# numtel/ntru-circom

Measured on NVIDIA B200. Metric: ciphertexts/sec (encrypt+decrypt) N=509 q=2048, higher is better.
Workload: dtype int8 x int8 -> int32

## Files before the change

### include/ntru_b200.h

```cpp
#ifndef NTRU_B200_H
#define NTRU_B200_H

#include <stddef.h>
#include <stdint.h>

#ifdef __cplusplus
extern "C" {
#endif

typedef struct ntru_ctx ntru_ctx;

enum {
  NTRU_OK = 0,
  NTRU_E_PARAM = -1,
  NTRU_E_LENGTH = -2,
  NTRU_E_NOKEY = -3,
  NTRU_E_CUDA = -4,
  NTRU_E_NCCL = -5,
  NTRU_E_NOMEM = -6,
  NTRU_E_UNSUPPORTED = -7
};

enum {
  NTRU_OPT_PATH = 1,
  NTRU_OPT_CHUNK_ROWS = 2,
  NTRU_OPT_TIMING = 3,
  NTRU_OPT_DR = 5,
  NTRU_OPT_DEC1_FORM = 6,
  NTRU_OPT_SCHEDULE = 7,
  NTRU_OPT_EPILOGUE = 8,
  NTRU_OPT_IMMA_FORM = 9
};

enum {
  NTRU_K_ENC_TENSOR = 0,
  NTRU_K_DEC1_TENSOR = 1,
  NTRU_K_DEC2_TENSOR = 2,
  NTRU_K_ENC_CORE = 3,
  NTRU_K_DEC_CORE = 4,
  NTRU_K_SUM = 5,
  NTRU_K_OTHER = 6,
  NTRU_K_ENC_IMMA = 7,
  NTRU_K_DEC_IMMA = 8,
  NTRU_K_MULDIV = 9,
  NTRU_K_PACK = 10,
  NTRU_K_COUNT = 11
};

int ntru_create(ntru_ctx **ctx, int N, int p, int q, int device);
void ntru_destroy(ntru_ctx *ctx);
const char *ntru_last_error(const ntru_ctx *ctx);
const char *ntru_strerror(int code);
int ntru_set_option(ntru_ctx *ctx, int key, long value);
int ntru_get_params(const ntru_ctx *ctx, int *N, int *p, int *q);
int ntru_pitch(const ntru_ctx *ctx);
uint64_t ntru_launch_count(const ntru_ctx *ctx);
int ntru_last_path(const ntru_ctx *ctx);
int ntru_timing_read(ntru_ctx *ctx, int kind, double *total_ms, uint64_t *launches);
int ntru_timing_reset(ntru_ctx *ctx);

int ntru_set_public_key(ntru_ctx *ctx, const uint16_t *h);
int ntru_set_private_key(ntru_ctx *ctx, const int8_t *f, const uint8_t *fp);

int ntru_encrypt_batch(ntru_ctx *ctx, size_t B, const uint8_t *r, const uint8_t *m,
                       uint16_t *value, uint16_t *quotientE, uint16_t *remainderE, uint8_t *r_out);
int ntru_encrypt_batch_wide(ntru_ctx *ctx, size_t B, const uint8_t *r, const uint16_t *m,
                            uint16_t *value, uint16_t *quotientE, uint16_t *remainderE, uint8_t *r_out);
int ntru_encrypt_batch_keys(ntru_ctx *ctx, size_t B, const uint16_t *h, const uint8_t *r, const uint8_t *m,
                            uint16_t *value, uint16_t *quotientE, uint16_t *remainderE, uint8_t *r_out);

#define NTRU_RNG_KEY_BYTES 32
int ntru_set_rng_key(ntru_ctx *ctx, const uint8_t key[NTRU_RNG_KEY_BYTES], uint64_t first_row);
uint64_t ntru_rng_next_row(const ntru_ctx *ctx);

int ntru_decrypt_batch(ntru_ctx *ctx, size_t B, const uint16_t *e, uint8_t *value,
                       uint16_t *quotient1, uint16_t *remainder1, uint8_t *quotient2, uint8_t *remainder2);
int ntru_decrypt_batch_keys(ntru_ctx *ctx, size_t B, const int8_t *f, const uint8_t *fp, const uint16_t *e,
                            uint8_t *value, uint16_t *quotient1, uint16_t *remainder1,
                            uint8_t *quotient2, uint8_t *remainder2);

int ntru_verify_keys_batch(ntru_ctx *ctx, size_t B, const int8_t *f, const uint16_t *fq, const uint8_t *fp, const int8_t *g,
                           uint16_t *quotient_fq, uint16_t *remainder_fq, uint8_t *quotient_fp, uint8_t *remainder_fp,
                           uint16_t *quotient_h, uint16_t *remainder_h);
int ntru_muldiv_dev(ntru_ctx *ctx, size_t B, const int8_t *x, const void *y, int mod_p, void *quotient, void *remainder);

int ntru_keygen_batch(ntru_ctx *ctx, size_t B, const int8_t *f, const int8_t *g, uint16_t *fq, uint8_t *fp, uint16_t *h,
                      uint8_t *valid);

int ntru_pack_geometry(uint32_t max_val, int data_len, int *max_input_bits, int *inputs_per_output, int *arr_len,
                       int *output_size);
int ntru_pack_output_dev(ntru_ctx *ctx, size_t B, const void *data, int elem_bytes, int data_len, size_t pitch,
                         uint32_t max_val, void *out);
int ntru_unpack_input_dev(ntru_ctx *ctx, size_t B, const void *data, int n_elems, uint32_t max_val, int packed_bits,
                          void *out, int elem_bytes, size_t pitch);

int ntru_pack_output(ntru_ctx *ctx, size_t B, const void *data, int elem_bytes, int data_len, uint32_t max_val, void *out);
int ntru_unpack_input(ntru_ctx *ctx, size_t B, const void *data, int n_elems, uint32_t max_val, int packed_bits, void *out,
                      int elem_bytes);

int ntru_packed_elems(const ntru_ctx *ctx, int mod_q, int width);
int ntru_encrypt_batch_packed(ntru_ctx *ctx, size_t B, const void *r, const void *m, void *value, void *quotientE,
                              void *remainderE, void *r_out);
int ntru_decrypt_batch_packed(ntru_ctx *ctx, size_t B, const void *e, void *value, void *quotient1, void *remainder1,
                              void *quotient2, void *remainder2);

int ntru_sum(ntru_ctx *ctx, size_t B, const uint16_t *e, uint16_t *out);
int ntru_sum_allreduce(ntru_ctx *ctx, size_t B, const uint16_t *e, uint16_t *out);

int ntru_encrypt_dev(ntru_ctx *ctx, size_t B, const uint16_t *h_rows, const uint8_t *r, const uint8_t *m,
                     uint16_t *value, uint16_t *quotientE, uint16_t *remainderE);
int ntru_decrypt_dev(ntru_ctx *ctx, size_t B, const int8_t *f_rows, const uint8_t *fp_rows, const uint16_t *e,
                     uint8_t *value, uint16_t *quotient1, uint16_t *remainder1,
                     uint8_t *quotient2, uint8_t *remainder2);
int ntru_sum_partial_dev(ntru_ctx *ctx, size_t B, const uint16_t *e, uint32_t *partial);
int ntru_sum_finalize_dev(ntru_ctx *ctx, const uint32_t *partial, uint16_t *out);
int ntru_sample_r_dev(ntru_ctx *ctx, size_t B, int dr, uint64_t row0, uint8_t *r);

#define NTRU_XCHG_HANDLE_BYTES 64
int ntru_xchg_create(ntru_ctx *ctx, int world, int rank, unsigned char handle_out[NTRU_XCHG_HANDLE_BYTES]);
int ntru_xchg_connect(ntru_ctx *ctx, const unsigned char *handles);
int ntru_sum_allreduce_dev(ntru_ctx *ctx, size_t B, const uint16_t *e, uint16_t *out);
int ntru_xchg_destroy(ntru_ctx *ctx);

void *ntru_stream(ntru_ctx *ctx);
int ntru_set_stream(ntru_ctx *ctx, void *stream);
int ntru_sync(ntru_ctx *ctx);

void *ntru_host_alloc(size_t bytes);
void ntru_host_free(void *p);

#ifdef __cplusplus
}
#endif
#endif
```

### ntru-circom_b200/_lib.py

```python
from __future__ import annotations

import ctypes
import os
from ctypes import POINTER, c_char_p, c_int, c_int8, c_long, c_size_t, c_uint8, c_uint16, c_uint32, c_uint64, c_void_p

_HERE = os.path.dirname(os.path.abspath(__file__))
LIB_PATH = os.environ.get("NTRU_B200_LIB") or os.path.join(_HERE, "libntru_b200.so")

NTRU_OK = 0
NTRU_E_PARAM, NTRU_E_LENGTH, NTRU_E_NOKEY, NTRU_E_CUDA = -1, -2, -3, -4
NTRU_E_NCCL, NTRU_E_NOMEM, NTRU_E_UNSUPPORTED = -5, -6, -7
NTRU_OPT_PATH, NTRU_OPT_CHUNK_ROWS, NTRU_OPT_TIMING, NTRU_OPT_DR, NTRU_OPT_DEC1_FORM, NTRU_OPT_SCHEDULE, NTRU_OPT_EPILOGUE = 1, 2, 3, 5, 6, 7, 8
NTRU_OPT_IMMA_FORM = 9
KERNEL_KINDS = ["enc_tensor", "dec1_tensor", "dec2_tensor", "enc_core", "dec_core", "sum", "other", "enc_imma", "dec_imma",
                "muldiv", "pack"]
PATH_AUTO, PATH_CUDA_CORE, PATH_TENSOR, PATH_IMMA = 0, 1, 2, 3

_P = c_void_p
SYMBOLS = {
    "ntru_create": (c_int, [POINTER(c_void_p), c_int, c_int, c_int, c_int]),
    "ntru_destroy": (None, [_P]),
    "ntru_last_error": (c_char_p, [_P]),
    "ntru_strerror": (c_char_p, [c_int]),
    "ntru_set_option": (c_int, [_P, c_int, c_long]),
    "ntru_pitch": (c_int, [_P]),
    "ntru_launch_count": (c_uint64, [_P]),
    "ntru_last_path": (c_int, [_P]),
    "ntru_timing_read": (c_int, [_P, c_int, POINTER(ctypes.c_double), POINTER(c_uint64)]),
    "ntru_timing_reset": (c_int, [_P]),
    "ntru_set_public_key": (c_int, [_P, _P]),
    "ntru_set_private_key": (c_int, [_P, _P, _P]),
    "ntru_encrypt_batch": (c_int, [_P, c_size_t, _P, _P, _P, _P, _P, _P]),
    "ntru_encrypt_batch_wide": (c_int, [_P, c_size_t, _P, _P, _P, _P, _P, _P]),
    "ntru_encrypt_batch_keys": (c_int, [_P, c_size_t, _P, _P, _P, _P, _P, _P, _P]),
    "ntru_set_rng_key": (c_int, [_P, _P, c_uint64]),
    "ntru_rng_next_row": (c_uint64, [_P]),
    "ntru_decrypt_batch": (c_int, [_P, c_size_t, _P, _P, _P, _P, _P, _P]),
    "ntru_decrypt_batch_keys": (c_int, [_P, c_size_t, _P, _P, _P, _P, _P, _P, _P, _P]),
    "ntru_packed_elems": (c_int, [_P, c_int, c_int]),
    "ntru_encrypt_batch_packed": (c_int, [_P, c_size_t, _P, _P, _P, _P, _P, _P]),
    "ntru_decrypt_batch_packed": (c_int, [_P, c_size_t, _P, _P, _P, _P, _P, _P]),
    "ntru_sum": (c_int, [_P, c_size_t, _P, _P]),
    "ntru_sum_allreduce": (c_int, [_P, c_size_t, _P, _P]),
    "ntru_pack_output": (c_int, [_P, c_size_t, _P, c_int, c_int, ctypes.c_uint32, _P]),
    "ntru_unpack_input": (c_int, [_P, c_size_t, _P, c_int, ctypes.c_uint32, c_int, _P, c_int]),
    "ntru_get_params": (c_int, [_P, POINTER(c_int), POINTER(c_int), POINTER(c_int)]),
    "ntru_keygen_batch": (c_int, [_P, c_size_t, _P, _P, _P, _P, _P, _P]),
    "ntru_pack_geometry": (c_int, [ctypes.c_uint32, c_int, POINTER(c_int), POINTER(c_int), POINTER(c_int), POINTER(c_int)]),
    "ntru_pack_output_dev": (c_int, [_P, c_size_t, _P, c_int, c_int, c_size_t, ctypes.c_uint32, _P]),
    "ntru_unpack_input_dev": (c_int, [_P, c_size_t, _P, c_int, ctypes.c_uint32, c_int, _P, c_int, c_size_t]),
    "ntru_verify_keys_batch": (c_int, [_P, c_size_t, _P, _P, _P, _P, _P, _P, _P, _P, _P, _P]),
    "ntru_muldiv_dev": (c_int, [_P, c_size_t, _P, _P, c_int, _P, _P]),
    "ntru_encrypt_dev": (c_int, [_P, c_size_t, _P, _P, _P, _P, _P, _P]),
    "ntru_decrypt_dev": (c_int, [_P, c_size_t, _P, _P, _P, _P, _P, _P, _P, _P]),
    "ntru_sum_partial_dev": (c_int, [_P, c_size_t, _P, _P]),
    "ntru_sum_finalize_dev": (c_int, [_P, _P, _P]),
    "ntru_sample_r_dev": (c_int, [_P, c_size_t, c_int, c_uint64, _P]),
    "ntru_xchg_create": (c_int, [_P, c_int, c_int, _P]),
    "ntru_xchg_connect": (c_int, [_P, _P]),
    "ntru_sum_allreduce_dev": (c_int, [_P, c_size_t, _P, _P]),
    "ntru_xchg_destroy": (c_int, [_P]),
    "ntru_stream": (c_void_p, [_P]),
    "ntru_set_stream": (c_int, [_P, _P]),
    "ntru_sync": (c_int, [_P]),
    "ntru_host_alloc": (c_void_p, [c_size_t]),
    "ntru_host_free": (None, [_P]),
}

_lib = None


class NtruError(RuntimeError):
    def __init__(self, code: int, msg: str):
        super().__init__(f"libntru_b200: {msg} (code {code})")
        self.code = code


def load() -> ctypes.CDLL:
    global _lib
    if _lib is not None:
        return _lib
    if not os.path.exists(LIB_PATH):
        from . import build as _build
        _build.build()
    lib = ctypes.CDLL(LIB_PATH)
    for name, (res, args) in SYMBOLS.items():
        fn = getattr(lib, name)
        fn.restype = res
        fn.argtypes = args
    _lib = lib
    return lib
```

### ntru-circom_b200/csrc/api.cu

```cuda

#include <cuda_runtime.h>
#include <stdint.h>
#include <stdio.h>
#include <stdlib.h>
#include <string.h>

#include <sys/random.h>

#include <new>
#include <string>

#include "ntru_internal.cuh"

namespace ntru {

int fail(ntru_ctx *ctx, int code, const std::string &msg) {
  if (ctx) ctx->err = msg;
  return code;
}

int cuda_fail(ntru_ctx *ctx, cudaError_t e, const char *what) {
  if (ctx) ctx->err = std::string("CUDA error: ") + cudaGetErrorString(e) + " in " + what;
  return NTRU_E_CUDA;
}

static cudaEvent_t pool_get(ntru_ctx *ctx) {
  if (!ctx->event_pool.empty()) {
    cudaEvent_t e = ctx->event_pool.back();
    ctx->event_pool.pop_back();
    return e;
  }
  cudaEvent_t e = nullptr;
  cudaEventCreate(&e);
  return e;
}

LaunchTimer::LaunchTimer(ntru_ctx *c, int k) : ctx(c), kind(k) {
  ctx->launches++;
  if (!ctx->timing) return;
  a = pool_get(ctx);
  b = pool_get(ctx);
  cudaEventRecord(a, ctx->stream);
}

LaunchTimer::~LaunchTimer() {
  if (!a) return;
  cudaEventRecord(b, ctx->stream);
  ctx->timed.push_back({kind, a, b});
}

namespace {

struct HostArr {
  const void *in = nullptr;
  void *out = nullptr;
  size_t elem = 1;
  size_t width = 0;
  bool used = false;
  int fe_bits = 0, fe_n = 0, fe_elems = 0;
  size_t host_row_bytes() const { return fe_bits ? (size_t)fe_elems * 32 : width * elem; }
};

constexpr int kMaxArr = 10;

template <class Launch>
int run_pipeline(ntru_ctx *ctx, size_t B, HostArr (&arr)[kMaxArr], Launch launch) {
  const size_t chunk = ctx->chunk_rows;
  const size_t P = (size_t)ctx->P;
  const size_t rows_alloc = B < chunk ? B : chunk;
  for (int s = 0; s < kNumSlots; ++s)
    for (int a = 0; a < kMaxArr; ++a)
      if (arr[a].used) {
        NTRU_CUDA(ctx, ctx->slot_bufs[s][a].reserve(rows_alloc * P * arr[a].elem));
        NTRU_CUDA(ctx, ctx->slot_packed[s][a].reserve(rows_alloc * arr[a].host_row_bytes()));
      }
  size_t ci = 0;
  for (size_t row0 = 0; row0 < B; row0 += chunk, ++ci) {
    const size_t rows = (B - row0) < chunk ? (B - row0) : chunk;
    const int s = (int)(ci % kNumSlots);
    void *dev[kMaxArr];
    for (int a = 0; a < kMaxArr; ++a) dev[a] = arr[a].used ? ctx->slot_bufs[s][a].ptr : nullptr;
    if (ci >= (size_t)kNumSlots) NTRU_CUDA(ctx, cudaStreamWaitEvent(ctx->s_in, ctx->ev_comp[s], 0));
    for (int a = 0; a < kMaxArr; ++a) {
      if (!arr[a].used || !arr[a].in) continue;
      const size_t wb = arr[a].host_row_bytes();
      NTRU_CUDA(ctx, cudaMemcpyAsync(ctx->slot_packed[s][a].ptr, (const char *)arr[a].in + row0 * wb, rows * wb,
                                     cudaMemcpyHostToDevice, ctx->s_in));
    }
    NTRU_CUDA(ctx, cudaEventRecord(ctx->ev_in[s], ctx->s_in));
    NTRU_CUDA(ctx, cudaStreamWaitEvent(ctx->stream, ctx->ev_in[s], 0));
    if (ci >= (size_t)kNumSlots) NTRU_CUDA(ctx, cudaStreamWaitEvent(ctx->stream, ctx->ev_out[s], 0));
    for (int a = 0; a < kMaxArr; ++a) {
      if (!arr[a].used || !arr[a].in) continue;
      int rc = arr[a].fe_bits
                   ? launch_wire_unpack(ctx, rows, (const uint32_t *)ctx->slot_packed[s][a].ptr, arr[a].fe_elems, arr[a].fe_bits,
                                        arr[a].fe_n, (int)arr[a].width, dev[a], (int)arr[a].elem)
                   : launch_repitch(ctx, ctx->slot_packed[s][a].ptr, dev[a], rows, (int)arr[a].width, (int)arr[a].elem, true);
      if (rc != NTRU_OK) return rc;
    }
    int rc = launch(rows, dev);
    if (rc != NTRU_OK) return rc;
    for (int a = 0; a < kMaxArr; ++a) {
      if (!arr[a].used || !arr[a].out) continue;
      rc = arr[a].fe_bits
               ? launch_pack_fields(ctx, rows, dev[a], (int)arr[a].elem, (int)arr[a].width, (size_t)ctx->P, arr[a].fe_bits, arr[a].fe_n,
                                    arr[a].fe_elems, (uint32_t *)ctx->slot_packed[s][a].ptr)
               : launch_repitch(ctx, dev[a], ctx->slot_packed[s][a].ptr, rows, (int)arr[a].width, (int)arr[a].elem, false);
      if (rc != NTRU_OK) return rc;
    }
    NTRU_CUDA(ctx, cudaEventRecord(ctx->ev_comp[s], ctx->stream));
    NTRU_CUDA(ctx, cudaStreamWaitEvent(ctx->s_out, ctx->ev_comp[s], 0));
    for (int a = 0; a < kMaxArr; ++a) {
      if (!arr[a].used || !arr[a].out) continue;
      const size_t wb = arr[a].host_row_bytes();
      NTRU_CUDA(ctx, cudaMemcpyAsync((char *)arr[a].out + row0 * wb, ctx->slot_packed[s][a].ptr, rows * wb,
                                     cudaMemcpyDeviceToHost, ctx->s_out));
    }
    NTRU_CUDA(ctx, cudaEventRecord(ctx->ev_out[s], ctx->s_out));
  }
  NTRU_CUDA(ctx, cudaStreamSynchronize(ctx->s_out));
  NTRU_CUDA(ctx, cudaStreamSynchronize(ctx->stream));
  return NTRU_OK;
}

void set_in(HostArr &a, const void *p, size_t elem, size_t width) {
  a.in = p; a.elem = elem; a.width = width; a.used = p != nullptr;
}
void set_out(HostArr &a, void *p, size_t elem, size_t width) {
  a.out = p; a.elem = elem; a.width = width; a.used = p != nullptr;
}

int bit_length(uint32_t v) {
  int b = 0;
  while (v) { ++b; v >>= 1; }
  return b;
}
void set_fe(HostArr &a, uint32_t max_val) {
  if (!a.used) return;
  a.fe_bits = bit_length(max_val);
  a.fe_n = 252 / a.fe_bits;
  int outs = ((int)a.width + a.fe_n - 1) / a.fe_n;
  a.fe_elems = outs < 3 ? 3 : outs;
}

int packed_elems(uint32_t max_val, int width) {
  const int n = 252 / bit_length(max_val);
  const int outs = (width + n - 1) / n;
  return outs < 3 ? 3 : outs;
}

constexpr size_t kSmallBatchRows = 4096;

bool want_tensor(ntru_ctx *ctx, bool same_key, bool ready, size_t B, int *rc) {
  *rc = NTRU_OK;
  if (ctx->opt_path == 1 || ctx->opt_path == 3) return false;
  if (ctx->opt_path == 0 && B < kSmallBatchRows && ctx->tensor_ok && imma_supported(ctx)) return false;
  const bool ok = same_key && ctx->tensor_ok && ready;
  if (ctx->opt_path == 2 && !ok) {
    *rc = fail(ctx, NTRU_E_UNSUPPORTED, "tensor schedule forced but not available for this call");
    return false;
  }
  return ok;
}

bool want_imma(ntru_ctx *ctx, bool wide_message, int *rc) {
  *rc = NTRU_OK;
  if (ctx->opt_path == 1) return false;
  const bool ok = ctx->tensor_ok && imma_supported(ctx) && !wide_message;
  if (ctx->opt_path == 3 && !ok) {
    *rc = fail(ctx, NTRU_E_UNSUPPORTED, "register-fragment schedule forced but not available for this call");
    return false;
  }
  return ok;
}

int encrypt_dispatch(ntru_ctx *ctx, size_t B, const uint16_t *h_rows, const uint8_t *r, const void *m, int m_wide,
                     uint16_t *value, uint16_t *quo, uint16_t *rem) {
  int rc;
  const bool same_key = h_rows == nullptr;
  if (same_key && !ctx->has_pub) return fail(ctx, NTRU_E_NOKEY, "public key h is not set");
  if (want_tensor(ctx, same_key && !m_wide, ctx->km_h.ready, B, &rc)) {
    ctx->last_path = 2;
    return umma_encrypt(ctx, B, r, (const uint8_t *)m, value, quo, rem);
  }
  if (rc != NTRU_OK) return rc;
  if (want_imma(ctx, m_wide != 0, &rc)) {
    ctx->last_path = 3;
    return launch_encrypt_imma(ctx, B, same_key ? (const uint16_t *)ctx->d_h.ptr : h_rows, same_key ? 0 : (size_t)ctx->P, r,
                               (const uint8_t *)m, value, quo, rem);
  }
  if (rc != NTRU_OK) return rc;
  ctx->last_path = 1;
  return launch_encrypt_generic(ctx, B, same_key ? (const uint16_t *)ctx->d_h.ptr : h_rows,
                                same_key ? 0 : (size_t)ctx->P, r, m, m_wide, value, quo, rem);
}

int decrypt_dispatch(ntru_ctx *ctx, size_t B, const int8_t *f_rows, const uint8_t *fp_rows, const uint16_t *e,
                     uint8_t *value, uint16_t *q1, uint16_t *r1, uint8_t *q2, uint8_t *r2) {
  int rc;
  const bool same_key = f_rows == nullptr && fp_rows == nullptr;
  if ((f_rows == nullptr) != (fp_rows == nullptr)) return fail(ctx, NTRU_E_PARAM, "f_rows and fp_rows must be given together");
  if (same_key && !ctx->has_priv) return fail(ctx, NTRU_E_NOKEY, "private key f/fp is not set");
  if (want_tensor(ctx, same_key, ctx->km_f.ready && ctx->km_fp.ready, B, &rc)) {
    ctx->last_path = 2;
    return umma_decrypt(ctx, B, e, value, q1, r1, q2, r2);
  }
  if (rc != NTRU_OK) return rc;
  if (want_imma(ctx, false, &rc)) {
    ctx->last_path = 3;
    return launch_decrypt_imma(ctx, B, same_key ? (const int8_t *)ctx->d_f.ptr : f_rows,
                               same_key ? (const uint8_t *)ctx->d_fp.ptr : fp_rows, same_key ? 0 : (size_t)ctx->P, e, value, q1,
                               r1, q2, r2);
  }
  if (rc != NTRU_OK) return rc;
  ctx->last_path = 1;
  return launch_decrypt_generic(ctx, B, same_key ? (const int8_t *)ctx->d_f.ptr : f_rows,
                                same_key ? (const uint8_t *)ctx->d_fp.ptr : fp_rows,
                                same_key ? 0 : (size_t)ctx->P, e, value, q1, r1, q2, r2);
}

int check(ntru_ctx *ctx) {
  if (!ctx) return NTRU_E_PARAM;
  cudaError_t e = cudaSetDevice(ctx->device);
  if (e != cudaSuccess) return cuda_fail(ctx, e, "cudaSetDevice");
  return NTRU_OK;
}

}
}

using namespace ntru;

extern "C" {

const char *ntru_strerror(int code) {
  switch (code) {
    case NTRU_OK: return "ok";
    case NTRU_E_PARAM: return "bad parameter";
    case NTRU_E_LENGTH: return "bad length";
    case NTRU_E_NOKEY: return "key not set";
    case NTRU_E_CUDA: return "CUDA error";
    case NTRU_E_NCCL: return "NCCL error";
    case NTRU_E_NOMEM: return "out of memory";
    case NTRU_E_UNSUPPORTED: return "unsupported";
    default: return "unknown error";
  }
}

const char *ntru_last_error(const ntru_ctx *ctx) { return ctx ? ctx->err.c_str() : "null context"; }

int ntru_create(ntru_ctx **out, int N, int p, int q, int device) {
  if (!out) return NTRU_E_PARAM;
  *out = nullptr;
  if (p != 3) return NTRU_E_PARAM;
  if (N < 8 || N > kMaxN) return NTRU_E_PARAM;
  if (q < 4 || q > 8192 || (q & (q - 1)) != 0) return NTRU_E_PARAM;
  if ((long long)N * 2 * (q - 1) >= (1ll << 24)) return NTRU_E_PARAM;
  int ndev = 0;
  cudaError_t e = cudaGetDeviceCount(&ndev);
  if (e != cudaSuccess || ndev == 0 || device < 0 || device >= ndev) return NTRU_E_CUDA;
  if (cudaSetDevice(device) != cudaSuccess) return NTRU_E_CUDA;
  ntru_ctx *ctx = new (std::nothrow) ntru_ctx();
  if (!ctx) return NTRU_E_NOMEM;
  ctx->N = N; ctx->p = p; ctx->q = q; ctx->device = device;
  ctx->logq = 0;
  while ((1 << ctx->logq) < q) ctx->logq++;
  ctx->P = ((N + 1 + 15) / 16) * 16;
  cudaDeviceProp prop;
  if (cudaGetDeviceProperties(&prop, device) == cudaSuccess) ctx->sm_count = prop.multiProcessorCount;
  bool ok = cudaStreamCreateWithFlags(&ctx->stream, cudaStreamNonBlocking) == cudaSuccess;
  ctx->own_stream = ok;
  ok = ok && cudaStreamCreateWithFlags(&ctx->s_in, cudaStreamNonBlocking) == cudaSuccess;
  ok = ok && cudaStreamCreateWithFlags(&ctx->s_out, cudaStreamNonBlocking) == cudaSuccess;
  for (int s = 0; ok && s < kNumSlots; ++s) {
    ok = ok && cudaEventCreateWithFlags(&ctx->ev_in[s], cudaEventDisableTiming) == cudaSuccess;
    ok = ok && cudaEventCreateWithFlags(&ctx->ev_comp[s], cudaEventDisableTiming) == cudaSuccess;
    ok = ok && cudaEventCreateWithFlags(&ctx->ev_out[s], cudaEventDisableTiming) == cudaSuccess;
  }
  ok = ok && ctx->d_h.reserve((size_t)ctx->P * 2) == cudaSuccess;
  ok = ok && ctx->d_f.reserve((size_t)ctx->P) == cudaSuccess;
  ok = ok && ctx->d_fp.reserve((size_t)ctx->P) == cudaSuccess;
  ok = ok && ctx->d_partial.reserve((size_t)ctx->P * 4) == cudaSuccess;
  if (!ok) {
    ntru_destroy(ctx);
    return NTRU_E_CUDA;
  }
  {
    size_t got = 0;
    unsigned char *kb = reinterpret_cast<unsigned char *>(ctx->rng_key);
    while (got < sizeof ctx->rng_key) {
      ssize_t n = getrandom(kb + got, sizeof ctx->rng_key - got, 0);
      if (n <= 0) break;
      got += (size_t)n;
    }
    if (got < sizeof ctx->rng_key) {
      FILE *fh = fopen("/dev/urandom", "rb");
      if (fh) {
        got += fread(kb + got, 1, sizeof ctx->rng_key - got, fh);
        fclose(fh);
      }
    }
    ctx->rng_keyed = got == sizeof ctx->rng_key;
  }
  umma_init(ctx);
  *out = ctx;
  return NTRU_OK;
}

static int xchg_release(ntru_ctx *ctx);
static int xchg_check(ntru_ctx *ctx);

void ntru_destroy(ntru_ctx *ctx) {
  if (!ctx) return;
  cudaSetDevice(ctx->device);
  cudaDeviceSynchronize();
  for (int s = 0; s < kNumSlots; ++s) {
    if (ctx->ev_in[s]) cudaEventDestroy(ctx->ev_in[s]);
    if (ctx->ev_comp[s]) cudaEventDestroy(ctx->ev_comp[s]);
    if (ctx->ev_out[s]) cudaEventDestroy(ctx->ev_out[s]);
    for (auto &b : ctx->slot_bufs[s]) b.release();
    for (auto &b : ctx->slot_packed[s]) b.release();
  }
  xchg_release(ctx);
  ctx->d_h.release(); ctx->d_f.release(); ctx->d_fp.release(); ctx->d_b.release(); ctx->d_partial.release(); ctx->d_sum_scratch.release();
  ctx->km_h.mat.release(); ctx->km_f.mat.release(); ctx->km_fp.mat.release();
  for (auto &t : ctx->timed) {
    cudaEventDestroy(t.a);
    cudaEventDestroy(t.b);
  }
  for (auto e : ctx->event_pool) cudaEventDestroy(e);
  if (ctx->own_stream && ctx->stream) cudaStreamDestroy(ctx->stream);
  if (ctx->s_in) cudaStreamDestroy(ctx->s_in);
  if (ctx->s_out) cudaStreamDestroy(ctx->s_out);
  delete ctx;
}

int ntru_set_option(ntru_ctx *ctx, int key, long value) {
  if (!ctx) return NTRU_E_PARAM;
  switch (key) {
    case NTRU_OPT_PATH:
      if (value < 0 || value > 3) return fail(ctx, NTRU_E_PARAM, "NTRU_OPT_PATH must be 0, 1, 2 or 3");
      ctx->opt_path = (int)value;
      return NTRU_OK;
    case NTRU_OPT_CHUNK_ROWS:
      if (value < 128) return fail(ctx, NTRU_E_PARAM, "NTRU_OPT_CHUNK_ROWS must be >= 128");
      ctx->chunk_rows = (size_t)value;
      return NTRU_OK;
    case NTRU_OPT_TIMING:
      ctx->timing = value != 0;
      return NTRU_OK;
    case NTRU_OPT_SCHEDULE:
      if (value < 0 || value > 1) return fail(ctx, NTRU_E_PARAM, "NTRU_OPT_SCHEDULE must be 0 or 1");
      ctx->opt_lohi = (int)value;
      return NTRU_OK;
    case NTRU_OPT_EPILOGUE:
      if (value < 0 || value > 2) return fail(ctx, NTRU_E_PARAM, "NTRU_OPT_EPILOGUE must be 0, 1 or 2");
      ctx->opt_epilogue = (int)value;
      if (ctx->tensor_ok) {
        if (ctx->has_pub) { int rc = umma_prepare_public(ctx); if (rc) return rc; }
        if (ctx->has_priv) { int rc = umma_prepare_private(ctx); if (rc) return rc; }
      }
      return NTRU_OK;
    case NTRU_OPT_IMMA_FORM:
      if (value < 0 || value > 1) return fail(ctx, NTRU_E_PARAM, "NTRU_OPT_IMMA_FORM must be 0 or 1");
      ctx->opt_imma_form = (int)value;
      return NTRU_OK;
    case NTRU_OPT_DEC1_FORM:
      if (value < 0 || value > 2) return fail(ctx, NTRU_E_PARAM, "NTRU_OPT_DEC1_FORM must be 0, 1 or 2");
      ctx->opt_dec1_form = (int)value;
      if (ctx->has_priv && ctx->tensor_ok) return umma_prepare_private(ctx);
      return NTRU_OK;
    case NTRU_OPT_DR:
      if (value < 0 || 2 * value > ctx->N) return fail(ctx, NTRU_E_PARAM, "The total of 1s and -1s cannot exceed the array length.");
      ctx->opt_dr = (int)value;
      return NTRU_OK;
    default:
      return fail(ctx, NTRU_E_PARAM, "unknown option");
  }
}

int ntru_pitch(const ntru_ctx *ctx) { return ctx ? ctx->P : 0; }
uint64_t ntru_launch_count(const ntru_ctx *ctx) { return ctx ? ctx->launches : 0; }
int ntru_last_path(const ntru_ctx *ctx) { return ctx ? ctx->last_path : 0; }

int ntru_timing_reset(ntru_ctx *ctx) {
  int rc = check(ctx);
  if (rc) return rc;
  NTRU_CUDA(ctx, cudaStreamSynchronize(ctx->stream));
  for (auto &t : ctx->timed) {
    ctx->event_pool.push_back(t.a);
    ctx->event_pool.push_back(t.b);
  }
  ctx->timed.clear();
  return NTRU_OK;
}

int ntru_timing_read(ntru_ctx *ctx, int kind, double *total_ms, uint64_t *launches) {
  int rc = check(ctx);
  if (rc) return rc;
  if (kind < 0 || kind >= NTRU_K_COUNT || !total_ms || !launches) return fail(ctx, NTRU_E_PARAM, "bad timing query");
  NTRU_CUDA(ctx, cudaStreamSynchronize(ctx->stream));
  double sum = 0;
  uint64_t n = 0;
  for (auto &t : ctx->timed) {
    if (t.kind != kind) continue;
    float ms = 0;
    NTRU_CUDA(ctx, cudaEventElapsedTime(&ms, t.a, t.b));
    sum += ms;
    ++n;
  }
  *total_ms = sum;
  *launches = n;
  return NTRU_OK;
}

int ntru_set_public_key(ntru_ctx *ctx, const uint16_t *h) {
  int rc = check(ctx);
  if (rc) return rc;
  if (!h) return fail(ctx, NTRU_E_PARAM, "h is NULL");
  uint16_t tmp[kMaxN + 32];
  memset(tmp, 0, sizeof tmp);
  for (int i = 0; i < ctx->N; ++i) {
    if (h[i] >= ctx->q) return fail(ctx, NTRU_E_PARAM, "h coefficient outside [0,q)");
    tmp[i] = h[i];
  }
  NTRU_CUDA(ctx, cudaMemcpy(ctx->d_h.ptr, tmp, (size_t)ctx->P * 2, cudaMemcpyHostToDevice));
  ctx->has_pub = true;
  ctx->km_h.ready = false;
  if (ctx->tensor_ok) {
    rc = umma_prepare_public(ctx);
    if (rc) return rc;
  }
  return NTRU_OK;
}

int ntru_set_private_key(ntru_ctx *ctx, const int8_t *f, const uint8_t *fp) {
  int rc = check(ctx);
  if (rc) return rc;
  if (!f || !fp) return fail(ctx, NTRU_E_PARAM, "f or fp is NULL");
  int8_t tf[kMaxN + 32];
  uint8_t tp[kMaxN + 32];
  memset(tf, 0, sizeof tf);
  memset(tp, 0, sizeof tp);
  for (int i = 0; i < ctx->N; ++i) {
    if (f[i] < -1 || f[i] > 1) return fail(ctx, NTRU_E_PARAM, "f coefficient outside {-1,0,1}");
    if (fp[i] >= ctx->p) return fail(ctx, NTRU_E_PARAM, "fp coefficient outside [0,p)");
    tf[i] = f[i];
    tp[i] = fp[i];
  }
  NTRU_CUDA(ctx, cudaMemcpy(ctx->d_f.ptr, tf, (size_t)ctx->P, cudaMemcpyHostToDevice));
  NTRU_CUDA(ctx, cudaMemcpy(ctx->d_fp.ptr, tp, (size_t)ctx->P, cudaMemcpyHostToDevice));
  ctx->has_priv = true;
  ctx->km_f.ready = ctx->km_fp.ready = false;
  if (ctx->tensor_ok) {
    rc = umma_prepare_private(ctx);
    if (rc) return rc;
  }
  return NTRU_OK;
}


static int encrypt_host(ntru_ctx *ctx, size_t B, const uint16_t *h, const uint8_t *r, const void *m, int m_wide,
                        uint16_t *value, uint16_t *quo, uint16_t *rem, uint8_t *r_out, bool fe = false) {
  int rc = check(ctx);
  if (rc) return rc;
  if (!m) return fail(ctx, NTRU_E_PARAM, "m is required");
  if (!r) {
    if (ctx->opt_dr < 0) return fail(ctx, NTRU_E_PARAM, "r is NULL and NTRU_OPT_DR (the dr of the constructor options) is not set");
    if (!ctx->rng_keyed) return fail(ctx, NTRU_E_UNSUPPORTED, "r is NULL and the device generator has no key (no OS entropy; call ntru_set_rng_key)");
  }
  if (B == 0) return NTRU_OK;
  const size_t N = (size_t)ctx->N;
  HostArr arr[kMaxArr];
  set_in(arr[0], h, 2, N);
  if (r) {
    set_in(arr[1], r, 1, N);
    if (r_out && r_out != r)
      memcpy(r_out, r, fe ? B * (size_t)packed_elems(ctx->p - 1, (int)N) * 32 : B * N);
  } else {
    set_out(arr[1], r_out, 1, N);
    arr[1].used = true;
  }
  set_in(arr[2], m, m_wide ? 2 : 1, N);
  set_out(arr[3], value, 2, N);
  set_out(arr[4], quo, 2, N + 1);
  set_out(arr[5], rem, 2, N + 1);
  if (fe) {
    set_fe(arr[1], (uint32_t)ctx->p - 1); set_fe(arr[2], (uint32_t)ctx->p - 1);
    for (int a = 3; a <= 5; ++a) set_fe(arr[a], (uint32_t)ctx->q - 1);
  }
  uint64_t next_row = ctx->rng_row;
  if (!r) ctx->rng_row += B;
  return run_pipeline(ctx, B, arr, [&](size_t rows, void **dev) {
    if (!r) {
      int rs = launch_sample_r(ctx, rows, ctx->opt_dr, next_row, (uint8_t *)dev[1]);
      if (rs) return rs;
      next_row += rows;
    }
    return encrypt_dispatch(ctx, rows, (const uint16_t *)dev[0], (const uint8_t *)dev[1], dev[2], m_wide,
                            (uint16_t *)dev[3], (uint16_t *)dev[4], (uint16_t *)dev[5]);
  });
}

int ntru_encrypt_batch(ntru_ctx *ctx, size_t B, const uint8_t *r, const uint8_t *m, uint16_t *value,
                       uint16_t *quotientE, uint16_t *remainderE, uint8_t *r_out) {
  return encrypt_host(ctx, B, nullptr, r, m, 0, value, quotientE, remainderE, r_out);
}

int ntru_encrypt_batch_wide(ntru_ctx *ctx, size_t B, const uint8_t *r, const uint16_t *m, uint16_t *value,
                            uint16_t *quotientE, uint16_t *remainderE, uint8_t *r_out) {
  return encrypt_host(ctx, B, nullptr, r, m, 1, value, quotientE, remainderE, r_out);
}

int ntru_encrypt_batch_keys(ntru_ctx *ctx, size_t B, const uint16_t *h, const uint8_t *r, const uint8_t *m,
                            uint16_t *value, uint16_t *quotientE, uint16_t *remainderE, uint8_t *r_out) {
  if (!h) return fail(ctx, NTRU_E_PARAM, "h is NULL");
  return encrypt_host(ctx, B, h, r, m, 0, value, quotientE, remainderE, r_out);
}

static int decrypt_host(ntru_ctx *ctx, size_t B, const int8_t *f, const uint8_t *fp, const uint16_t *e,
                        uint8_t *value, uint16_t *q1, uint16_t *r1, uint8_t *q2, uint8_t *r2, bool fe = false) {
  int rc = check(ctx);
  if (rc) return rc;
  if (!e) return fail(ctx, NTRU_E_PARAM, "e is required");
  if (B == 0) return NTRU_OK;
  const size_t N = (size_t)ctx->N;
  HostArr arr[kMaxArr];
  set_in(arr[0], f, 1, N);
  set_in(arr[1], fp, 1, N);
  set_in(arr[2], e, 2, N);
  set_out(arr[3], value, 1, N);
  set_out(arr[4], q1, 2, N + 1);
  set_out(arr[5], r1, 2, N + 1);
  set_out(arr[6], q2, 1, N + 1);
  set_out(arr[7], r2, 1, N + 1);
  if (fe) {
    set_fe(arr[2], (uint32_t)ctx->q - 1); set_fe(arr[4], (uint32_t)ctx->q - 1); set_fe(arr[5], (uint32_t)ctx->q - 1);
    set_fe(arr[3], (uint32_t)ctx->p - 1); set_fe(arr[6], (uint32_t)ctx->p - 1); set_fe(arr[7], (uint32_t)ctx->p - 1);
  }
  return run_pipeline(ctx, B, arr, [&](size_t rows, void **dev) {
    return decrypt_dispatch(ctx, rows, (const int8_t *)dev[0], (const uint8_t *)dev[1], (const uint16_t *)dev[2],
                            (uint8_t *)dev[3], (uint16_t *)dev[4], (uint16_t *)dev[5], (uint8_t *)dev[6],
                            (uint8_t *)dev[7]);
  });
}

int ntru_decrypt_batch(ntru_ctx *ctx, size_t B, const uint16_t *e, uint8_t *value, uint16_t *quotient1,
                       uint16_t *remainder1, uint8_t *quotient2, uint8_t *remainder2) {
  return decrypt_host(ctx, B, nullptr, nullptr, e, value, quotient1, remainder1, quotient2, remainder2);
}

int ntru_decrypt_batch_keys(ntru_ctx *ctx, size_t B, const int8_t *f, const uint8_t *fp, const uint16_t *e,
                            uint8_t *value, uint16_t *quotient1, uint16_t *remainder1, uint8_t *quotient2,
                            uint8_t *remainder2) {
  if (!f || !fp) return fail(ctx, NTRU_E_PARAM, "f or fp is NULL");
  return decrypt_host(ctx, B, f, fp, e, value, quotient1, remainder1, quotient2, remainder2);
}

int ntru_packed_elems(const ntru_ctx *ctx, int mod_q, int width) {
  if (!ctx || width < 0) return 0;
  return packed_elems(mod_q ? (uint32_t)ctx->q - 1 : (uint32_t)ctx->p - 1, width);
}

int ntru_encrypt_batch_packed(ntru_ctx *ctx, size_t B, const void *r, const void *m, void *value, void *quotientE,
                              void *remainderE, void *r_out) {
  return encrypt_host(ctx, B, nullptr, (const uint8_t *)r, m, 0, (uint16_t *)value, (uint16_t *)quotientE, (uint16_t *)remainderE,
                      (uint8_t *)r_out, true);
}

int ntru_decrypt_batch_packed(ntru_ctx *ctx, size_t B, const void *e, void *value, void *quotient1, void *remainder1,
                              void *quotient2, void *remainder2) {
  return decrypt_host(ctx, B, nullptr, nullptr, (const uint16_t *)e, (uint8_t *)value, (uint16_t *)quotient1, (uint16_t *)remainder1,
                      (uint8_t *)quotient2, (uint8_t *)remainder2, true);
}

__global__ void k_scale_u16(const uint16_t *__restrict__ src, uint16_t *__restrict__ dst, size_t n, uint32_t mul) {
  for (size_t i = (size_t)blockIdx.x * blockDim.x + threadIdx.x; i < n; i += (size_t)gridDim.x * blockDim.x)
    dst[i] = (uint16_t)(src[i] * mul);
}

int ntru_muldiv_dev(ntru_ctx *ctx, size_t B, const int8_t *x, const void *y, int mod_p, void *quotient, void *remainder) {
  int rc = check(ctx);
  if (rc) return rc;
  if (B > 0 && (!x || !y)) return fail(ctx, NTRU_E_PARAM, "x and y are required");
  if (!ctx->tensor_ok) return fail(ctx, NTRU_E_UNSUPPORTED, "multiply + divide needs the sm_100 tensor path");
  return launch_muldiv_imma(ctx, B, x, y, mod_p, quotient, remainder);
}

int ntru_verify_keys_batch(ntru_ctx *ctx, size_t B, const int8_t *f, const uint16_t *fq, const uint8_t *fp, const int8_t *g,
                           uint16_t *quotient_fq, uint16_t *remainder_fq, uint8_t *quotient_fp, uint8_t *remainder_fp,
                           uint16_t *quotient_h, uint16_t *remainder_h) {
  int rc = check(ctx);
  if (rc) return rc;
  if (!f || !fq || !fp || !g) return fail(ctx, NTRU_E_PARAM, "f, fq, fp and g are required");
  if (!ctx->tensor_ok) return fail(ctx, NTRU_E_UNSUPPORTED, "verify_keys needs the sm_100 tensor path");
  if (B == 0) return NTRU_OK;
  const size_t N = (size_t)ctx->N;
  HostArr arr[kMaxArr];
  set_in(arr[0], f, 1, N);
  set_in(arr[1], fq, 2, N);
  set_in(arr[2], fp, 1, N);
  set_in(arr[3], g, 1, N);
  set_out(arr[4], quotient_fq, 2, N + 1);
  set_out(arr[5], remainder_fq, 2, N + 1);
  set_out(arr[6], quotient_fp, 1, N + 1);
  set_out(arr[7], remainder_fp, 1, N + 1);
  set_out(arr[8], quotient_h, 2, N + 1);
  set_out(arr[9], remainder_h, 2, N + 1);
  return run_pipeline(ctx, B, arr, [&](size_t rows, void **dev) {
    int r2 = NTRU_OK;
    if (dev[4] || dev[5]) r2 = launch_muldiv_imma(ctx, rows, (const int8_t *)dev[0], dev[1], 0, dev[4], dev[5]);
    if (r2) return r2;
    if (dev[6] || dev[7]) r2 = launch_muldiv_imma(ctx, rows, (const int8_t *)dev[0], dev[2], 1, dev[6], dev[7]);
    if (r2) return r2;
    if (dev[8] || dev[9]) {
      NTRU_CUDA(ctx, ctx->d_b.reserve(rows * (size_t)ctx->P * 2));
      {
        LaunchTimer timer(ctx, NTRU_K_OTHER);
        k_scale_u16<<<ctx->sm_count * 4, 256, 0, ctx->stream>>>((const uint16_t *)dev[1], (uint16_t *)ctx->d_b.ptr,
                                                               rows * (size_t)ctx->P, (uint32_t)ctx->p);
      }
      NTRU_CUDA(ctx, cudaGetLastError());
      r2 = launch_muldiv_imma(ctx, rows, (const int8_t *)dev[3], ctx->d_b.ptr, 0, dev[8], dev[9]);
    }
    return r2;
  });
}

int ntru_keygen_batch(ntru_ctx *ctx, size_t B, const int8_t *f, const int8_t *g, uint16_t *fq, uint8_t *fp, uint16_t *h,
                      uint8_t *valid) {
  int rc = check(ctx);
  if (rc) return rc;
  if (B > 0 && (!f || !g || !fq || !fp || !h || !valid)) return fail(ctx, NTRU_E_PARAM, "f, g, fq, fp, h and valid are required");
  return keygen_batch(ctx, B, f, g, fq, fp, h, valid);
}


int ntru_pack_geometry(uint32_t max_val, int data_len, int *max_input_bits, int *inputs_per_output, int *arr_len,
                       int *output_size) {
  if (max_val == 0 || data_len < 0) return NTRU_E_PARAM;
  const int bits = bit_length(max_val);
  const int n = 252 / bits;
  int arr = ((data_len + n - 1) / n) * n;
  if (arr < 3 * n) arr = 3 * n;
  int outs = (arr + n - 1) / n;
  if (outs < 3) outs = 3;
  if (max_input_bits) *max_input_bits = bits;
  if (inputs_per_output) *inputs_per_output = n;
  if (arr_len) *arr_len = arr;
  if (output_size) *output_size = outs;
  return NTRU_OK;
}

int ntru_pack_output_dev(ntru_ctx *ctx, size_t B, const void *data, int elem_bytes, int data_len, size_t pitch,
                         uint32_t max_val, void *out) {
  int rc = check(ctx);
  if (rc) return rc;
  int bits, n, arr, outs;
  if (ntru_pack_geometry(max_val, data_len, &bits, &n, &arr, &outs) != NTRU_OK || (elem_bytes != 1 && elem_bytes != 2))
    return fail(ctx, NTRU_E_PARAM, "bad maxVal / dataLen / element size");
  if (bits > 8 * elem_bytes + 16) return fail(ctx, NTRU_E_PARAM, "maxVal does not fit the element type");
  if (B > 0 && (!data || !out)) return fail(ctx, NTRU_E_PARAM, "data and out are required");
  return launch_pack_fields(ctx, B, data, elem_bytes, data_len, pitch, bits, n, outs, (uint32_t *)out);
}

int ntru_unpack_input_dev(ntru_ctx *ctx, size_t B, const void *data, int n_elems, uint32_t max_val, int packed_bits,
                          void *out, int elem_bytes, size_t pitch) {
  int rc = check(ctx);
  if (rc) return rc;
  if (max_val == 0 || n_elems < 0 || packed_bits < 1 || packed_bits > 256 || (elem_bytes != 1 && elem_bytes != 2))
    return fail(ctx, NTRU_E_PARAM, "bad maxVal / packedBits / element size");
  const int bits = bit_length(max_val);
  const int n = packed_bits / bits;
  if (n < 1) return fail(ctx, NTRU_E_PARAM, "packedBits is smaller than one coefficient");
  if (bits > 8 * elem_bytes) return fail(ctx, NTRU_E_PARAM, "maxVal does not fit the element type");
  if (B > 0 && (!data || !out)) return fail(ctx, NTRU_E_PARAM, "data and out are required");
  return launch_unpack_fields(ctx, B, (const uint32_t *)data, n_elems, bits, n, pitch, out, elem_bytes);
}

int ntru_sum(ntru_ctx *ctx, size_t B, const uint16_t *e, uint16_t *out) {
  int rc = check(ctx);
  if (rc) return rc;
  if (!e || !out) return fail(ctx, NTRU_E_PARAM, "e and out are required");
  NTRU_CUDA(ctx, cudaMemsetAsync(ctx->d_partial.ptr, 0, (size_t)ctx->P * 4, ctx->stream));
  if (B > 0) {
    HostArr arr[kMaxArr];
    set_in(arr[0], e, 2, (size_t)ctx->N);
    rc = run_pipeline(ctx, B, arr, [&](size_t rows, void **dev) {
      return launch_sum_partial(ctx, rows, (const uint16_t *)dev[0], (uint32_t *)ctx->d_partial.ptr);
    });
    if (rc) return rc;
  }
  NTRU_CUDA(ctx, ctx->slot_bufs[0][9].reserve((size_t)ctx->P * 2));
  rc = launch_sum_finalize(ctx, (const uint32_t *)ctx->d_partial.ptr, (uint16_t *)ctx->slot_bufs[0][9].ptr);
  if (rc) return rc;
  NTRU_CUDA(ctx, cudaMemcpyAsync(out, ctx->slot_bufs[0][9].ptr, (size_t)ctx->N * 2, cudaMemcpyDeviceToHost,
                                 ctx->stream));
  NTRU_CUDA(ctx, cudaStreamSynchronize(ctx->stream));
  return NTRU_OK;
}


int ntru_encrypt_dev(ntru_ctx *ctx, size_t B, const uint16_t *h_rows, const uint8_t *r, const uint8_t *m,
                     uint16_t *value, uint16_t *quotientE, uint16_t *remainderE) {
  int rc = check(ctx);
  if (rc) return rc;
  if (!r || !m) return fail(ctx, NTRU_E_PARAM, "r and m are required");
  return encrypt_dispatch(ctx, B, h_rows, r, m, 0, value, quotientE, remainderE);
}

int ntru_decrypt_dev(ntru_ctx *ctx, size_t B, const int8_t *f_rows, const uint8_t *fp_rows, const uint16_t *e,
                     uint8_t *value, uint16_t *quotient1, uint16_t *remainder1, uint8_t *quotient2,
                     uint8_t *remainder2) {
  int rc = check(ctx);
  if (rc) return rc;
  if (!e) return fail(ctx, NTRU_E_PARAM, "e is required");
  return decrypt_dispatch(ctx, B, f_rows, fp_rows, e, value, quotient1, remainder1, quotient2, remainder2);
}

int ntru_sum_partial_dev(ntru_ctx *ctx, size_t B, const uint16_t *e, uint32_t *partial) {
  int rc = check(ctx);
  if (rc) return rc;
  if (!e || !partial) return fail(ctx, NTRU_E_PARAM, "e and partial are required");
  return launch_sum_partial(ctx, B, e, partial);
}

int ntru_sum_finalize_dev(ntru_ctx *ctx, const uint32_t *partial, uint16_t *out) {
  int rc = check(ctx);
  if (rc) return rc;
  if (!partial || !out) return fail(ctx, NTRU_E_PARAM, "partial and out are required");
  return launch_sum_finalize(ctx, partial, out);
}

static int xchg_release(ntru_ctx *ctx) {
  for (int r = 0; r < ntru_ctx::kMaxRanks; ++r) {
    if (ctx->peer_opened[r] && ctx->peer_window[r]) cudaIpcCloseMemHandle(ctx->peer_window[r]);
    ctx->peer_opened[r] = false;
    ctx->peer_window[r] = nullptr;
  }
  ctx->d_window.release();
  ctx->xchg_connected = false;
  ctx->xchg_world = 1;
  ctx->xchg_rank = 0;
  ctx->xchg_epoch = 0;
  return NTRU_OK;
}

static int xchg_alloc(ntru_ctx *ctx, int world, int rank) {
  xchg_release(ctx);
  const size_t bytes = xchg_window_bytes(ctx, world);
  NTRU_CUDA(ctx, ctx->d_window.reserve(bytes));
  NTRU_CUDA(ctx, cudaMemset(ctx->d_window.ptr, 0, bytes));
  ctx->xchg_world = world;
  ctx->xchg_rank = rank;
  ctx->peer_window[rank] = ctx->d_window.ptr;
  return NTRU_OK;
}

int ntru_xchg_create(ntru_ctx *ctx, int world, int rank, unsigned char handle_out[NTRU_XCHG_HANDLE_BYTES]) {
  int rc = check(ctx);
  if (rc) return rc;
  if (world < 1 || world > ntru_ctx::kMaxRanks || rank < 0 || rank >= world || !handle_out)
    return fail(ctx, NTRU_E_PARAM, "bad world / rank / handle buffer");
  static_assert(sizeof(cudaIpcMemHandle_t) == NTRU_XCHG_HANDLE_BYTES, "IPC handle size");
  rc = xchg_alloc(ctx, world, rank);
  if (rc) return rc;
  cudaIpcMemHandle_t h;
  NTRU_CUDA(ctx, cudaIpcGetMemHandle(&h, ctx->d_window.ptr));
  memcpy(handle_out, &h, sizeof h);
  ctx->xchg_connected = world == 1;
  return NTRU_OK;
}

int ntru_xchg_connect(ntru_ctx *ctx, const unsigned char *handles) {
  int rc = check(ctx);
  if (rc) return rc;
  if (!handles) return fail(ctx, NTRU_E_PARAM, "handles is NULL");
  if (!ctx->d_window.ptr) return fail(ctx, NTRU_E_PARAM, "ntru_xchg_create has not been called");
  for (int r = 0; r < ctx->xchg_world; ++r) {
    if (r == ctx->xchg_rank) continue;
    cudaIpcMemHandle_t h;
    memcpy(&h, handles + (size_t)r * NTRU_XCHG_HANDLE_BYTES, sizeof h);
    void *p = nullptr;
    NTRU_CUDA(ctx, cudaIpcOpenMemHandle(&p, h, cudaIpcMemLazyEnablePeerAccess));
    ctx->peer_window[r] = p;
    ctx->peer_opened[r] = true;
  }
  ctx->xchg_connected = true;
  return NTRU_OK;
}

int ntru_sum_allreduce_dev(ntru_ctx *ctx, size_t B, const uint16_t *e, uint16_t *out) {
  int rc = check(ctx);
  if (rc) return rc;
  if ((B > 0 && !e) || !out) return fail(ctx, NTRU_E_PARAM, "e and out are required");
  if (!ctx->d_window.ptr) {
    rc = xchg_alloc(ctx, 1, 0);
    if (rc) return rc;
    ctx->xchg_connected = true;
  }
  if (!ctx->xchg_connected) return fail(ctx, NTRU_E_PARAM, "ntru_xchg_connect has not been called");
  return launch_sum_allreduce(ctx, B, e, out);
}

int ntru_sum_allreduce(ntru_ctx *ctx, size_t B, const uint16_t *e, uint16_t *out) {
  int rc = check(ctx);
  if (rc) return rc;
  if ((B > 0 && !e) || !out) return fail(ctx, NTRU_E_PARAM, "e and out are required");
  if (!ctx->d_window.ptr) {
    rc = xchg_alloc(ctx, 1, 0);
    if (rc) return rc;
    ctx->xchg_connected = true;
  }
  if (!ctx->xchg_connected) return fail(ctx, NTRU_E_PARAM, "ntru_xchg_connect has not been called");
  NTRU_CUDA(ctx, cudaMemsetAsync(ctx->d_partial.ptr, 0, (size_t)ctx->P * 4, ctx->stream));
  if (B > 0) {
    HostArr arr[kMaxArr];
    set_in(arr[0], e, 2, (size_t)ctx->N);
    rc = run_pipeline(ctx, B, arr, [&](size_t rows, void **dev) {
      return launch_sum_partial(ctx, rows, (const uint16_t *)dev[0], (uint32_t *)ctx->d_partial.ptr);
    });
    if (rc) return rc;
  }
  NTRU_CUDA(ctx, ctx->slot_bufs[0][9].reserve((size_t)ctx->P * 2));
  rc = launch_xchg_partial(ctx, (uint32_t *)ctx->d_partial.ptr, (uint16_t *)ctx->slot_bufs[0][9].ptr);
  if (rc) return rc;
  NTRU_CUDA(ctx, cudaMemcpyAsync(out, ctx->slot_bufs[0][9].ptr, (size_t)ctx->N * 2, cudaMemcpyDeviceToHost, ctx->stream));
  NTRU_CUDA(ctx, cudaStreamSynchronize(ctx->stream));
  return xchg_check(ctx);
}

int ntru_pack_output(ntru_ctx *ctx, size_t B, const void *data, int elem_bytes, int data_len, uint32_t max_val, void *out) {
  int rc = check(ctx);
  if (rc) return rc;
  int bits, n, arr, outs;
  if (ntru_pack_geometry(max_val, data_len, &bits, &n, &arr, &outs) != NTRU_OK || (elem_bytes != 1 && elem_bytes != 2))
    return fail(ctx, NTRU_E_PARAM, "bad maxVal / dataLen / element size");
  if (B == 0) return NTRU_OK;
  if (!data || !out) return fail(ctx, NTRU_E_PARAM, "data and out are required");
  const size_t in_bytes = B * (size_t)data_len * elem_bytes, out_bytes = B * (size_t)outs * 32;
  NTRU_CUDA(ctx, ctx->slot_packed[0][8].reserve(in_bytes));
  NTRU_CUDA(ctx, ctx->slot_packed[0][9].reserve(out_bytes));
  NTRU_CUDA(ctx, cudaMemcpyAsync(ctx->slot_packed[0][8].ptr, data, in_bytes, cudaMemcpyHostToDevice, ctx->stream));
  rc = ntru_pack_output_dev(ctx, B, ctx->slot_packed[0][8].ptr, elem_bytes, data_len, (size_t)data_len, max_val, ctx->slot_packed[0][9].ptr);
  if (rc) return rc;
  NTRU_CUDA(ctx, cudaMemcpyAsync(out, ctx->slot_packed[0][9].ptr, out_bytes, cudaMemcpyDeviceToHost, ctx->stream));
  NTRU_CUDA(ctx, cudaStreamSynchronize(ctx->stream));
  return NTRU_OK;
}

int ntru_unpack_input(ntru_ctx *ctx, size_t B, const void *data, int n_elems, uint32_t max_val, int packed_bits, void *out,
                      int elem_bytes) {
  int rc = check(ctx);
  if (rc) return rc;
  if (max_val == 0 || n_elems < 0 || packed_bits < 1 || packed_bits > 256 || (elem_bytes != 1 && elem_bytes != 2))
    return fail(ctx, NTRU_E_PARAM, "bad maxVal / packedBits / element size");
  const int bits = bit_length(max_val);
  const int n = packed_bits / bits;
  if (n < 1) return fail(ctx, NTRU_E_PARAM, "packedBits is smaller than one coefficient");
  if (B == 0 || n_elems == 0) return NTRU_OK;
  if (!data || !out) return fail(ctx, NTRU_E_PARAM, "data and out are required");
  const size_t width = (size_t)n * n_elems;
  const size_t in_bytes = B * (size_t)n_elems * 32, out_bytes = B * width * elem_bytes;
  NTRU_CUDA(ctx, ctx->slot_packed[0][8].reserve(in_bytes));
  NTRU_CUDA(ctx, ctx->slot_packed[0][9].reserve(out_bytes));
  NTRU_CUDA(ctx, cudaMemcpyAsync(ctx->slot_packed[0][8].ptr, data, in_bytes, cudaMemcpyHostToDevice, ctx->stream));
  rc = ntru_unpack_input_dev(ctx, B, ctx->slot_packed[0][8].ptr, n_elems, max_val, packed_bits, ctx->slot_packed[0][9].ptr, elem_bytes, width);
  if (rc) return rc;
  NTRU_CUDA(ctx, cudaMemcpyAsync(out, ctx->slot_packed[0][9].ptr, out_bytes, cudaMemcpyDeviceToHost, ctx->stream));
  NTRU_CUDA(ctx, cudaStreamSynchronize(ctx->stream));
  return NTRU_OK;
}

int ntru_get_params(const ntru_ctx *ctx, int *N, int *p, int *q) {
  if (!ctx) return NTRU_E_PARAM;
  if (N) *N = ctx->N;
  if (p) *p = ctx->p;
  if (q) *q = ctx->q;
  return NTRU_OK;
}

int ntru_sample_r_dev(ntru_ctx *ctx, size_t B, int dr, uint64_t row0, uint8_t *r) {
  int rc = check(ctx);
  if (rc) return rc;
  if (!r) return fail(ctx, NTRU_E_PARAM, "r is NULL");
  if (dr < 0 || 2 * dr > ctx->N) return fail(ctx, NTRU_E_PARAM, "The total of 1s and -1s cannot exceed the array length.");
  if (!ctx->rng_keyed) return fail(ctx, NTRU_E_UNSUPPORTED, "the device generator has no key (no OS entropy; call ntru_set_rng_key)");
  return launch_sample_r(ctx, B, dr, row0, r);
}

int ntru_set_rng_key(ntru_ctx *ctx, const uint8_t key[NTRU_RNG_KEY_BYTES], uint64_t first_row) {
  if (!ctx || !key) return NTRU_E_PARAM;
  for (int i = 0; i < 8; ++i)
    ctx->rng_key[i] = (uint32_t)key[4 * i] | ((uint32_t)key[4 * i + 1] << 8) | ((uint32_t)key[4 * i + 2] << 16) |
                      ((uint32_t)key[4 * i + 3] << 24);
  ctx->rng_row = first_row;
  ctx->rng_keyed = true;
  return NTRU_OK;
}

uint64_t ntru_rng_next_row(const ntru_ctx *ctx) { return ctx ? ctx->rng_row : 0; }

void *ntru_stream(ntru_ctx *ctx) { return ctx ? (void *)ctx->stream : nullptr; }

int ntru_set_stream(ntru_ctx *ctx, void *stream) {
  if (!ctx) return NTRU_E_PARAM;
  if (ctx->own_stream && ctx->stream) {
    cudaStreamSynchronize(ctx->stream);
    cudaStreamDestroy(ctx->stream);
  }
  ctx->stream = (cudaStream_t)stream;
  ctx->own_stream = false;
  return NTRU_OK;
}

static int xchg_check(ntru_ctx *ctx) {
  if (!ctx->d_window.ptr) return NTRU_OK;
  uint32_t err = 0;
  const uint32_t *word = (const uint32_t *)ctx->d_window.ptr + (size_t)2 * ctx->xchg_world * ctx->P + ctx->xchg_world;
  NTRU_CUDA(ctx, cudaMemcpy(&err, word, sizeof err, cudaMemcpyDeviceToHost));
  if (err) return fail(ctx, NTRU_E_CUDA, "cross-GPU sum: a peer rank did not arrive within the timeout; the result is invalid");
  return NTRU_OK;
}

int ntru_sync(ntru_ctx *ctx) {
  int rc = check(ctx);
  if (rc) return rc;
  NTRU_CUDA(ctx, cudaStreamSynchronize(ctx->stream));
  return xchg_check(ctx);
}

int ntru_xchg_destroy(ntru_ctx *ctx) {
  int rc = check(ctx);
  if (rc) return rc;
  NTRU_CUDA(ctx, cudaStreamSynchronize(ctx->stream));
  rc = xchg_check(ctx);
  xchg_release(ctx);
  return rc;
}

void *ntru_host_alloc(size_t bytes) {
  void *p = nullptr;
  if (cudaMallocHost(&p, bytes) != cudaSuccess) return nullptr;
  return p;
}

void ntru_host_free(void *p) {
  if (p) cudaFreeHost(p);
}

}
```

### ntru-circom_b200/csrc/ntru_internal.cuh

```cuda
#pragma once

#include <cuda_runtime.h>
#include <stdint.h>

#include <string>
#include <vector>

#include "../../include/ntru_b200.h"

namespace ntru {

constexpr int kMaxN = 1024;
constexpr int kNumSlots = 2;

struct DevBuf {
  void *ptr = nullptr;
  size_t bytes = 0;
  cudaError_t reserve(size_t need) {
    if (need <= bytes) return cudaSuccess;
    if (ptr) cudaFree(ptr);
    ptr = nullptr;
    bytes = 0;
    cudaError_t e = cudaMalloc(&ptr, need);
    if (e == cudaSuccess) bytes = need;
    return e;
  }
  void release() {
    if (ptr) cudaFree(ptr);
    ptr = nullptr;
    bytes = 0;
  }
};

constexpr int kMaxChunks = 8;

struct KeyMatrix {
  DevBuf mat;
  alignas(64) unsigned char tmap_half[2][128];
  bool ready = false;
  bool f16 = false;
  int limbs = 0, nlimbs = 0, klen = 0, nchunks = 0;
  int col0[kMaxChunks + 1] = {};
  int w[2] = {0, 0};
};

}

struct ntru_ctx {
  int N = 0, p = 0, q = 0, logq = 0, device = 0;
  int P = 0;
  cudaStream_t stream = nullptr;
  bool own_stream = false;
  cudaStream_t s_in = nullptr, s_out = nullptr;
  cudaEvent_t ev_in[ntru::kNumSlots] = {}, ev_comp[ntru::kNumSlots] = {}, ev_out[ntru::kNumSlots] = {};
  bool has_pub = false, has_priv = false;
  ntru::DevBuf d_h, d_f, d_fp;
  ntru::KeyMatrix km_h, km_f, km_fp;
  ntru::DevBuf d_b;
  ntru::DevBuf slot_bufs[ntru::kNumSlots][10];
  ntru::DevBuf slot_packed[ntru::kNumSlots][10];
  ntru::DevBuf d_partial;
  ntru::DevBuf d_sum_scratch;
  static constexpr int kMaxRanks = 16;
  int xchg_world = 1, xchg_rank = 0;
  bool xchg_connected = false;
  ntru::DevBuf d_window;
  void *peer_window[kMaxRanks] = {};
  bool peer_opened[kMaxRanks] = {};
  uint32_t xchg_epoch = 0;
  size_t chunk_rows = 32768;
  int opt_path = 0;
  int opt_imma_form = 0;
  int opt_epilogue = 0;
  int opt_lohi = 0;
  int opt_dec1_form = 0;
  int umma_attr_set = 0;
  bool sampler_attr_set = false;
  uint32_t rng_key[8] = {};
  bool rng_keyed = false;
  uint64_t rng_row = 0;
  int opt_dr = -1;
  struct ImmaCfg { const void *fn; size_t smem; int per_sm; };
  std::vector<ImmaCfg> imma_cfg;
  struct TmapKey {
    const void *base; uint64_t inner, rows, stride; uint32_t box_inner, box_rows; int elem, swz;
    bool operator==(const TmapKey &o) const {
      return base == o.base && inner == o.inner && rows == o.rows && stride == o.stride && box_inner == o.box_inner &&
             box_rows == o.box_rows && elem == o.elem && swz == o.swz;
    }
  };
  struct TmapEntry { TmapKey key; alignas(64) unsigned char map[128]; };
  std::vector<TmapEntry> tmap_cache;
  size_t tmap_next = 0;
  static constexpr size_t kTmapCacheMax = 64;
  int last_path = 0;
  int sm_count = 148;
  bool tensor_ok = false;
  uint64_t launches = 0;
  std::string err;
  bool timing = false;
  struct TimedLaunch { int kind; cudaEvent_t a, b; };
  std::vector<TimedLaunch> timed;
  std::vector<cudaEvent_t> event_pool;
};

namespace ntru {

int fail(ntru_ctx *ctx, int code, const std::string &msg);
int cuda_fail(ntru_ctx *ctx, cudaError_t e, const char *what);

struct LaunchTimer {
  ntru_ctx *ctx;
  cudaEvent_t a = nullptr, b = nullptr;
  int kind;
  LaunchTimer(ntru_ctx *c, int k);
  ~LaunchTimer();
};

#define NTRU_CUDA(ctx, expr)                                        \
  do {                                                              \
    cudaError_t _e = (expr);                                        \
    if (_e != cudaSuccess) return ntru::cuda_fail(ctx, _e, #expr);  \
  } while (0)

int launch_encrypt_generic(ntru_ctx *ctx, size_t B, const uint16_t *h, size_t h_stride, const uint8_t *r,
                           const void *m, int m_wide, uint16_t *value, uint16_t *quo, uint16_t *rem);
int launch_decrypt_generic(ntru_ctx *ctx, size_t B, const int8_t *f, const uint8_t *fp, size_t key_stride,
                           const uint16_t *e, uint8_t *value, uint16_t *q1, uint16_t *r1, uint8_t *q2,
                           uint8_t *r2);
int launch_sum_partial(ntru_ctx *ctx, size_t B, const uint16_t *e, uint32_t *partial);
int launch_sum_finalize(ntru_ctx *ctx, const uint32_t *partial, uint16_t *out);
size_t xchg_window_bytes(const ntru_ctx *ctx, int world);
int launch_sum_allreduce(ntru_ctx *ctx, size_t B, const uint16_t *e, uint16_t *out);
int launch_xchg_partial(ntru_ctx *ctx, uint32_t *partial, uint16_t *out);
int launch_sample_r(ntru_ctx *ctx, size_t B, int dr, uint64_t row0, uint8_t *r);
int launch_wire_unpack(ntru_ctx *ctx, size_t B, const uint32_t *data, int in_elems, int bits, int n, int width, void *out,
                       int elem_bytes);
int launch_pack_fields(ntru_ctx *ctx, size_t B, const void *data, int elem_bytes, int data_len, size_t pitch, int bits, int n,
                       int out_elems, uint32_t *out);
int launch_unpack_fields(ntru_ctx *ctx, size_t B, const uint32_t *data, int in_elems, int bits, int n, size_t pitch, void *out,
                         int elem_bytes);
int launch_repitch(ntru_ctx *ctx, const void *src, void *dst, size_t rows, int width, int elem, bool to_pitched);

bool imma_supported(const ntru_ctx *ctx);
int launch_encrypt_imma(ntru_ctx *ctx, size_t B, const uint16_t *h, size_t h_stride, const uint8_t *r, const uint8_t *m,
                        uint16_t *value, uint16_t *quo, uint16_t *rem);
int launch_decrypt_imma(ntru_ctx *ctx, size_t B, const int8_t *f, const uint8_t *fp, size_t key_stride, const uint16_t *e,
                        uint8_t *value, uint16_t *q1, uint16_t *r1, uint8_t *q2, uint8_t *r2);

int launch_muldiv_imma(ntru_ctx *ctx, size_t B, const int8_t *x, const void *y, int mod_p, void *quo, void *rem);

int keygen_batch(ntru_ctx *ctx, size_t B, const int8_t *f, const int8_t *g, uint16_t *fq, uint8_t *fp, uint16_t *h,
                 uint8_t *valid);

int umma_init(ntru_ctx *ctx);
int umma_prepare_public(ntru_ctx *ctx);
int umma_prepare_private(ntru_ctx *ctx);
int umma_encrypt(ntru_ctx *ctx, size_t B, const uint8_t *r, const uint8_t *m, uint16_t *value, uint16_t *quo,
                 uint16_t *rem);
int umma_decrypt(ntru_ctx *ctx, size_t B, const uint16_t *e, uint8_t *value, uint16_t *q1, uint16_t *r1,
                 uint8_t *q2, uint8_t *r2);

}
```

### ntru-circom_b200/csrc/umma_kernels.cu

```cuda

#include <cuda.h>
#include <cuda_runtime.h>
#include <stdint.h>
#include <stdlib.h>
#include <string.h>

#include "ntru_internal.cuh"

namespace ntru {

namespace {

enum Mode { ENC = 0, DEC1 = 1, DEC2 = 2, DEC1F = 3 };

constexpr int kTileRows = 128;
constexpr int kAtomK = 128;
constexpr int kABytes = kTileRows * kAtomK;
constexpr int kAccCols = 256;

constexpr int kMaxPhases = 2 * kMaxChunks;
enum PhaseKind { PH_CYC = 0, PH_HI = 1, PH_LO = 2 };
struct Phase {
  int8_t c, kind, a0, a1;
  uint16_t first, rel;
};

struct UmmaArgs {
  int nph;
  Phase ph[kMaxPhases];
  int8_t a_order[16];
  int N, P, Kp, atoms;
  int ea, ea_shift;
  int k_last;
  int kl;
  int nl;
  int nchunks;
  int col0[kMaxChunks + 1];
  int w0;
  int with_hi, q;
  uint32_t qmask;
  size_t B;
  int npairs;
  int nA, nB;
  int a_resident;
  int a_tma;
  int nM, nS;
  int a_rel;
  int two_issuers;
  int one_group;
  int debug_flags;
  int mat_rows;
  int out_mask;
  const void *a_src;
  const uint8_t *m;
  uint16_t *o16_cyc;
  uint16_t *o16_cyc2;
  uint16_t *o16_hi;
  uint8_t *o8_cyc;
  uint8_t *o8_cyc2;
  uint8_t *o8_hi;
};

__device__ __forceinline__ uint32_t smem_u32(const void *p) { return (uint32_t)__cvta_generic_to_shared(p); }

__device__ __forceinline__ void mbar_init(uint32_t bar, uint32_t count) {
  asm volatile("mbarrier.init.shared::cta.b64 [%0], %1;" ::"r"(bar), "r"(count));
}
__device__ __forceinline__ void mbar_arrive(uint32_t bar) {
  asm volatile("mbarrier.arrive.shared::cta.b64 _, [%0];" ::"r"(bar) : "memory");
}
__device__ __forceinline__ void mbar_arrive_expect_tx(uint32_t bar, uint32_t bytes) {
  asm volatile("mbarrier.arrive.expect_tx.shared::cta.b64 _, [%0], %1;" ::"r"(bar), "r"(bytes) : "memory");
}
__device__ __forceinline__ void mbar_wait(uint32_t bar, uint32_t parity) {
  asm volatile(
      "{\n\t"
      ".reg .pred p;\n\t"
      "WAIT_LOOP:\n\t"
      "mbarrier.try_wait.parity.shared::cta.b64 p, [%0], %1;\n\t"
      "@p bra WAIT_DONE;\n\t"
      "bra WAIT_LOOP;\n\t"
      "WAIT_DONE:\n\t"
      "}" ::"r"(bar), "r"(parity) : "memory");
}
__device__ __forceinline__ void fence_barrier_init() {
  asm volatile("fence.mbarrier_init.release.cluster;" ::: "memory");
}
__device__ __forceinline__ void fence_proxy_async() { asm volatile("fence.proxy.async.shared::cta;" ::: "memory"); }
__device__ __forceinline__ void tc_fence_before() { asm volatile("tcgen05.fence::before_thread_sync;" ::: "memory"); }
__device__ __forceinline__ void tc_fence_after() { asm volatile("tcgen05.fence::after_thread_sync;" ::: "memory"); }

__device__ __forceinline__ void tma_load_2d(uint32_t dst, const CUtensorMap *map, int c0, int c1, uint32_t bar) {
  asm volatile(
      "cp.async.bulk.tensor.2d.shared::cluster.global.mbarrier::complete_tx::bytes [%0], [%1, {%2, %3}], [%4];" ::"r"(dst),
      "l"(map), "r"(c0), "r"(c1), "r"(bar)
      : "memory");
}

__device__ __forceinline__ void tmem_ld16(uint32_t taddr, uint32_t (&v)[32]) {
  asm volatile(
      "tcgen05.ld.sync.aligned.32x32b.x16.b32 "
      "{%0, %1, %2, %3, %4, %5, %6, %7, %8, %9, %10, %11, %12, %13, %14, %15}, [%16];"
      : "=r"(v[0]), "=r"(v[1]), "=r"(v[2]), "=r"(v[3]), "=r"(v[4]), "=r"(v[5]), "=r"(v[6]), "=r"(v[7]), "=r"(v[8]),
        "=r"(v[9]), "=r"(v[10]), "=r"(v[11]), "=r"(v[12]), "=r"(v[13]), "=r"(v[14]), "=r"(v[15])
      : "r"(taddr));
}
__device__ __forceinline__ void tmem_ld_wait() { asm volatile("tcgen05.wait::ld.sync.aligned;" ::: "memory"); }

__device__ __forceinline__ uint64_t make_smem_desc(uint32_t saddr) {
  return (uint64_t)((saddr >> 4) & 0x3FFF) | (1ull << 16) | ((uint64_t)(1024 >> 4) << 32) | (1ull << 46) | (2ull << 61);
}

#include "umma_pair.cuh"

struct ChunkTable {
  int nchunks;
  int col0[kMaxChunks + 1];
};

__global__ void k_build_keymat(int mode, int N, int Kp, int kl, int nl, const ChunkTable ct, const void *poly, uint8_t *mat) {
  const int klen = kl * Kp;
  const int T = ct.col0[ct.nchunks];
  const size_t rows_total = (size_t)3 * nl * T;
  const size_t total = rows_total * klen;
  for (size_t idx = (size_t)blockIdx.x * blockDim.x + threadIdx.x; idx < total; idx += (size_t)gridDim.x * blockDim.x) {
    const int kb = (int)(idx % klen);
    const int row = (int)(idx / klen);
    const int part = row / (nl * T);
    const int rin = row % (nl * T);
    int c = 0;
    while (c + 1 < ct.nchunks && rin >= nl * ct.col0[c + 1]) ++c;
    const int w = ct.col0[c + 1] - ct.col0[c];
    const int off = rin - nl * ct.col0[c];
    const int ln = off / w, j = off % w;
    const int k = ct.col0[c] + j;
    const int lk = kb / Kp, i = mode == DEC1F ? (kb % Kp) >> 1 : kb % Kp;
    int coef = 0;
    bool nz = k < N && i < N;
    int src = 0;
    if (nz) {
      if (part == PH_HI) {
        nz = i > k;
        src = k + N - i;
      } else {
        nz = part == PH_CYC || i <= k;
        src = k - i;
        if (src < 0) src += N;
      }
    }
    if (nz) {
      if (mode == ENC) coef = reinterpret_cast<const uint16_t *>(poly)[src];
      else if (mode == DEC1 || mode == DEC1F) coef = reinterpret_cast<const int8_t *>(poly)[src];
      else coef = reinterpret_cast<const uint8_t *>(poly)[src];
    }
    uint8_t out;
    if (mode == ENC) out = ln == 0 ? (uint8_t)(coef & 0xff) : (uint8_t)(coef >> 8);
    else if (mode == DEC1) out = (uint8_t)(int8_t)(lk == 0 ? coef : coef * 64);
    else if (mode == DEC1F) out = (kb & 1) ? (coef > 0 ? 0x3C : (coef < 0 ? 0xBC : 0)) : 0;
    else out = (uint8_t)coef;
    mat[((size_t)(kb / kAtomK) * rows_total + (size_t)row) * kAtomK + (kb % kAtomK)] = out;
  }
}

typedef CUresult (*EncodeTiledFn)(CUtensorMap *, CUtensorMapDataType, cuuint32_t, void *, const cuuint64_t *,
                                  const cuuint64_t *, const cuuint32_t *, const cuuint32_t *, CUtensorMapInterleave,
                                  CUtensorMapSwizzle, CUtensorMapL2promotion, CUtensorMapFloatOOBfill);

EncodeTiledFn get_encode_fn() {
  static EncodeTiledFn fn = nullptr;
  if (!fn) {
    void *p = nullptr;
    cudaDriverEntryPointQueryResult qres;
    if (cudaGetDriverEntryPoint("cuTensorMapEncodeTiled", &p, cudaEnableDefault, &qres) == cudaSuccess &&
        qres == cudaDriverEntryPointSuccess)
      fn = (EncodeTiledFn)p;
  }
  return fn;
}

bool one_group_mode(const ntru_ctx *ctx, int mode) {
  if (ctx->opt_epilogue == 1) return false;
  if (ctx->opt_epilogue == 2) return true;
  const int N = ctx->N;
  if (mode == DEC1) return N <= 768;
  if (mode == DEC1F) return N <= 512;
  if (mode == DEC2) return N <= 512 && (N + 255) / 256 * 256 == (N + 127) / 128 * 128;
  return false;
}

void geometry(const ntru_ctx *ctx, int mode, int kl, int nl, KeyMatrix &km) {
  const int N = ctx->N;
  km.limbs = kl;
  km.nlimbs = nl;
  const int Kp = (((mode == DEC1F ? 2 * N : N) + kAtomK - 1) / kAtomK) * kAtomK;
  km.klen = kl * Kp;
  const int max_out = mode == ENC ? 128 : 256 / nl;
  const bool pu1 = mode == ENC && Kp / kAtomK >= 5;
  const int g = (mode == ENC ? (pu1 ? 32 : 64) : (mode == DEC1 ? 32 : (mode == DEC1F ? 64 : 128))) * (one_group_mode(ctx, mode) ? 2 : 1);
  const int T = ((N + g - 1) / g) * g;
  km.nchunks = (T + max_out - 1) / max_out;
  const int base = (T / km.nchunks / g) * g;
  const int wide = (T - base * km.nchunks) / g;
  km.col0[0] = 0;
  for (int c = 0; c < km.nchunks; ++c) km.col0[c + 1] = km.col0[c] + base + (c < wide ? g : 0);
  km.w[0] = km.col0[1] - km.col0[0];
  km.w[1] = km.col0[km.nchunks] - km.col0[km.nchunks - 1];
}

int encode_2d_ex(ntru_ctx *ctx, void *out, void *base, int elem_bytes, uint64_t inner, uint64_t rows, uint64_t stride_bytes,
                 uint32_t box_inner, uint32_t box_rows, CUtensorMapSwizzle swz) {
  EncodeTiledFn enc = get_encode_fn();
  if (!enc) return fail(ctx, NTRU_E_CUDA, "cuTensorMapEncodeTiled entry point not available");
  if (((uintptr_t)base & 15) != 0) return fail(ctx, NTRU_E_PARAM, "device arrays must be 16-byte aligned");
  const ntru_ctx::TmapKey key = {base, inner, rows, stride_bytes, box_inner, box_rows, elem_bytes, (int)swz};
  for (const auto &e : ctx->tmap_cache)
    if (e.key == key) {
      memcpy(out, e.map, 128);
      return NTRU_OK;
    }
  cuuint64_t gdim[2] = {(cuuint64_t)inner, (cuuint64_t)rows};
  cuuint64_t gstride[1] = {(cuuint64_t)stride_bytes};
  cuuint32_t box[2] = {box_inner, box_rows};
  cuuint32_t estr[2] = {1, 1};
  CUresult r = enc(reinterpret_cast<CUtensorMap *>(out), elem_bytes == 2 ? CU_TENSOR_MAP_DATA_TYPE_UINT16 : CU_TENSOR_MAP_DATA_TYPE_UINT8,
                   2, base, gdim, gstride, box, estr, CU_TENSOR_MAP_INTERLEAVE_NONE, swz, CU_TENSOR_MAP_L2_PROMOTION_L2_256B,
                   CU_TENSOR_MAP_FLOAT_OOB_FILL_NONE);
  if (r != CUDA_SUCCESS) return fail(ctx, NTRU_E_CUDA, "cuTensorMapEncodeTiled failed with code " + std::to_string((int)r));
  if (ctx->tmap_cache.size() < ntru_ctx::kTmapCacheMax) {
    ctx->tmap_cache.emplace_back();
    ctx->tmap_cache.back().key = key;
    memcpy(ctx->tmap_cache.back().map, out, 128);
  } else {
    auto &e = ctx->tmap_cache[ctx->tmap_next++ % ntru_ctx::kTmapCacheMax];
    e.key = key;
    memcpy(e.map, out, 128);
  }
  return NTRU_OK;
}

int encode_2d(ntru_ctx *ctx, void *out, void *base, uint64_t inner, uint64_t rows, uint64_t stride_bytes, uint32_t box_inner,
              uint32_t box_rows) {
  return encode_2d_ex(ctx, out, base, 1, inner, rows, stride_bytes, box_inner, box_rows, CU_TENSOR_MAP_SWIZZLE_128B);
}

int build_keymat(ntru_ctx *ctx, int mode, int kl, int nl, const void *poly, KeyMatrix &km) {
  geometry(ctx, mode, kl, nl, km);
  const int T = km.col0[km.nchunks];
  const int rows = 3 * nl * T;
  const int Kp = km.klen / kl;
  const size_t bytes = (size_t)rows * km.klen;
  NTRU_CUDA(ctx, km.mat.reserve(bytes));
  ChunkTable ct;
  ct.nchunks = km.nchunks;
  for (int c = 0; c <= kMaxChunks; ++c) ct.col0[c] = c <= km.nchunks ? km.col0[c] : 0;
  {
    LaunchTimer timer(ctx, NTRU_K_OTHER);
    k_build_keymat<<<ctx->sm_count * 4, 256, 0, ctx->stream>>>(mode, ctx->N, Kp, kl, nl, ct, poly, (uint8_t *)km.mat.ptr);
  }
  NTRU_CUDA(ctx, cudaGetLastError());
  const uint64_t tiled_rows = (uint64_t)rows * (km.klen / kAtomK);
  for (int i = 0; i < 2; ++i) {
    int rc = encode_2d(ctx, km.tmap_half[i], km.mat.ptr, kAtomK, tiled_rows, kAtomK, kAtomK, (uint32_t)(nl * km.w[i]) / 2);
    if (rc) return rc;
  }
  NTRU_CUDA(ctx, cudaStreamSynchronize(ctx->stream));
  km.ready = true;
  return NTRU_OK;
}

void build_schedule(UmmaArgs &a, bool lohi) {
  auto hi_a0 = [&](int c) {
    const int v = (a.col0[c] + 1) >> a.ea_shift;
    return v < a.atoms ? v : a.atoms - 1;
  };
  auto lo_a1 = [&](int c) {
    const int last = (a.col0[c + 1] < a.N ? a.col0[c + 1] : a.N) - 1;
    return (last >> a.ea_shift) + 1;
  };
  a.nph = 0;
  auto push = [&](int c, int kind) {
    Phase &p = a.ph[a.nph++];
    p.c = (int8_t)c; p.kind = (int8_t)kind;
    p.a0 = (int8_t)(kind == PH_HI ? hi_a0(c) : 0);
    p.a1 = (int8_t)(kind == PH_LO ? lo_a1(c) : a.atoms);
    p.first = p.rel = 0;
  };
  if (!a.with_hi) {
    for (int c = 0; c < a.nchunks; ++c) push(c, PH_CYC);
  } else if (!lohi) {
    for (int c = 0; c < a.nchunks; ++c) push(c, PH_CYC);
    for (int c = 0; c < a.nchunks; ++c) push(c, PH_HI);
  } else {
    int c = a.nchunks - 1;
    if (a.nchunks & 1) { push(c, PH_CYC); push(c, PH_HI); --c; }
    for (; c >= 1; c -= 2) { push(c, PH_HI); push(c - 1, PH_HI); push(c, PH_LO); push(c - 1, PH_LO); }
  }
  uint32_t seen = 0;
  int no = 0;
  for (int j = 0; j < a.nph; ++j)
    for (int at = a.ph[j].a0; at < a.ph[j].a1; ++at)
      if (!(seen >> at & 1u)) { seen |= 1u << at; a.ph[j].first |= (uint16_t)(1u << at); if (no < 16) a.a_order[no++] = (int8_t)at; }
  seen = 0;
  for (int j = a.nph - 1; j >= 0; --j)
    for (int at = a.ph[j].a0; at < a.ph[j].a1; ++at)
      if (!(seen >> at & 1u)) { seen |= 1u << at; a.ph[j].rel |= (uint16_t)(1u << at); }
}

template <int MODE>
int launch_product(ntru_ctx *ctx, const KeyMatrix &km, UmmaArgs &a, const void *a_bytes) {
  if (!(ctx->umma_attr_set & (1 << MODE))) {
    NTRU_CUDA(ctx, cudaFuncSetAttribute(k_umma_pair<MODE>, cudaFuncAttributeMaxDynamicSharedMemorySize, (int)kPairSmemBytes));
    ctx->umma_attr_set |= 1 << MODE;
  }
  a.N = ctx->N; a.P = ctx->P; a.kl = km.limbs; a.nl = km.nlimbs; a.Kp = km.klen / km.limbs; a.atoms = a.Kp / kAtomK;
  a.ea = MODE == DEC1F ? kAtomK / 2 : kAtomK;
  a.ea_shift = MODE == DEC1F ? 6 : 7;
  a.k_last = (ctx->N - (a.atoms - 1) * a.ea + a.ea / 4 - 1) / (a.ea / 4);
  a.nchunks = km.nchunks; a.q = ctx->q; a.qmask = (uint32_t)ctx->q - 1;
  for (int c = 0; c <= kMaxChunks; ++c) a.col0[c] = c <= km.nchunks ? km.col0[c] : km.col0[km.nchunks];
  a.w0 = km.w[0];
  a.mat_rows = 3 * a.nl * a.col0[a.nchunks];
  build_schedule(a, ctx->opt_lohi == 0);
  a.npairs = (int)((a.B + 2 * kTileRows - 1) / (2 * kTileRows));
  a.nS = 2;
  a.nM = MODE == ENC ? 2 : 0;
  const int a_slots = a.atoms * a.kl;
  const bool pu1 = MODE == ENC && a.atoms >= 5;
  if (pu1) { a.nS = 1; a.nM = 0; }
  const int avail = kPairSlots - a.nS - a.nM;
  if (a_slots + 4 <= avail) {
    a.a_resident = 1; a.nA = a_slots; a.nB = avail - a_slots;
  } else {
    a.a_resident = 0; a.nA = 6; a.nB = avail - 6;
  }
  a.a_tma = MODE == DEC1 && !a.a_resident && a.kl == 2 && avail >= 11;
  if (a.a_tma) { a.nA = 8; a.nB = avail - 8; }
  a.two_issuers = 0;
  a.a_rel = (a.a_resident && a.two_issuers) ? 2 : 1;
  a.one_group = one_group_mode(ctx, MODE) ? 1 : 0;
  CUtensorMap tmB, tmB2, tmA, tmM, tmO[3];
  memcpy(&tmB, km.tmap_half[0], sizeof tmB);
  memcpy(&tmB2, km.tmap_half[1], sizeof tmB2);
  memset(&tmA, 0, sizeof tmA);
  memset(&tmM, 0, sizeof tmM);
  memset(tmO, 0, sizeof tmO);
  const uint64_t N = (uint64_t)ctx->N, P = (uint64_t)ctx->P;
  int rc;
  if (MODE == DEC1F) {
    rc = encode_2d_ex(ctx, &tmA, const_cast<void *>(a.a_src), 2, N, (uint64_t)a.B, P * 2, kAtomK / 2, kTileRows, CU_TENSOR_MAP_SWIZZLE_128B);
    if (rc) return rc;
  } else if (MODE != DEC1) {
    rc = encode_2d(ctx, &tmA, const_cast<void *>(a_bytes), N, (uint64_t)a.B, P, kAtomK, kTileRows);
    if (rc) return rc;
  } else if (a.a_tma) {
    rc = encode_2d_ex(ctx, &tmA, const_cast<void *>(a.a_src), 2, P, (uint64_t)a.B, P * 2, kAtomK, kTileRows, CU_TENSOR_MAP_SWIZZLE_NONE);
    if (rc) return rc;
  }
  if (MODE == ENC && !pu1) {
    rc = encode_2d(ctx, &tmM, const_cast<uint8_t *>(a.m), N, (uint64_t)a.B, P, kAtomK, kTileRows);
    if (rc) return rc;
  }
  {
    void *optr[3];
    int oelem[3], obox[3];
    CUtensorMapSwizzle oswz[3];
    if (MODE == ENC || MODE == DEC1 || MODE == DEC1F) {
      const int ob = pu1 ? 16 : 32;
      const CUtensorMapSwizzle osw = pu1 ? CU_TENSOR_MAP_SWIZZLE_32B : CU_TENSOR_MAP_SWIZZLE_64B;
      optr[0] = a.o16_cyc; oelem[0] = 2; obox[0] = ob; oswz[0] = osw;
      optr[2] = a.o16_hi; oelem[2] = 2; obox[2] = ob; oswz[2] = osw;
      if (MODE == ENC) { optr[1] = a.o16_cyc2; oelem[1] = 2; obox[1] = ob; oswz[1] = osw; }
      else if (MODE == DEC1) { optr[1] = a.o8_cyc; oelem[1] = 1; obox[1] = 32; oswz[1] = CU_TENSOR_MAP_SWIZZLE_NONE; }
      else optr[1] = nullptr;
    } else {
      optr[0] = a.o8_cyc; optr[1] = a.o8_cyc2; optr[2] = a.o8_hi;
      for (int i = 0; i < 3; ++i) { oelem[i] = 1; obox[i] = 64; oswz[i] = CU_TENSOR_MAP_SWIZZLE_64B; }
    }
    a.out_mask = 0;
    for (int i = 0; i < 3; ++i) {
      if (!optr[i]) continue;
      a.out_mask |= 1 << i;
      rc = encode_2d_ex(ctx, &tmO[i], optr[i], oelem[i], P, (uint64_t)a.B, P * oelem[i], (uint32_t)obox[i], 32, oswz[i]);
      if (rc) return rc;
    }
#ifdef NTRU_TRACE
    if (getenv("NTRU_DEBUG_NOSTORE")) a.out_mask = 0;
    if (getenv("NTRU_DEBUG_NOB")) a.debug_flags |= 1;
    if (getenv("NTRU_DEBUG_ONE_MMA")) a.debug_flags |= 2;
    if (getenv("NTRU_TRACE_SLICES")) a.debug_flags |= 4;
    if (getenv("NTRU_TRACE_LIGHT")) a.debug_flags |= 16;
    if (getenv("NTRU_DEBUG_DOUBLE_MMA")) a.debug_flags |= 32;
#endif
  }
  {
    const size_t cov = (size_t)a.col0[a.nchunks];
    if (cov < P) {
      void *o16[3] = {a.o16_cyc, a.o16_cyc2, a.o16_hi};
      void *o8[3] = {MODE == DEC2 ? a.o8_cyc : nullptr, a.o8_cyc2, a.o8_hi};
      for (int i = 0; i < 3; ++i) {
        if (o16[i]) NTRU_CUDA(ctx, cudaMemset2DAsync((uint16_t *)o16[i] + cov, P * 2, 0, (P - cov) * 2, a.B, ctx->stream));
        if (o8[i]) NTRU_CUDA(ctx, cudaMemset2DAsync((uint8_t *)o8[i] + cov, P, 0, P - cov, a.B, ctx->stream));
      }
    }
  }
  {
    LaunchTimer timer(ctx, MODE == ENC ? NTRU_K_ENC_TENSOR : (MODE == DEC2 ? NTRU_K_DEC2_TENSOR : NTRU_K_DEC1_TENSOR));
    const int clusters = a.npairs < ctx->sm_count / 2 ? a.npairs : ctx->sm_count / 2;
#ifdef NTRU_TRACE
    const int dbg = getenv("NTRU_DEBUG_EPI") ? atoi(getenv("NTRU_DEBUG_EPI")) : 0;
#define NTRU_DBG_LAUNCH(D)                                                                                                  \
  case D:                                                                                                                  \
    cudaFuncSetAttribute(k_umma_pair<MODE, D>, cudaFuncAttributeMaxDynamicSharedMemorySize, (int)kPairSmemBytes);          \
    k_umma_pair<MODE, D><<<2 * clusters, kPairThreads, kPairSmemBytes, ctx->stream>>>(a, tmB, tmB2, tmA, tmM, tmO[0], tmO[1], tmO[2]); \
    break;
    switch (pu1 ? 0 : dbg) {
      NTRU_DBG_LAUNCH(1) NTRU_DBG_LAUNCH(2) NTRU_DBG_LAUNCH(4) NTRU_DBG_LAUNCH(8) NTRU_DBG_LAUNCH(12) NTRU_DBG_LAUNCH(16)
      default:
        if (pu1) {
          cudaFuncSetAttribute(k_umma_pair<ENC, 0, 1>, cudaFuncAttributeMaxDynamicSharedMemorySize, (int)kPairSmemBytes);
          k_umma_pair<ENC, 0, 1><<<2 * clusters, kPairThreads, kPairSmemBytes, ctx->stream>>>(a, tmB, tmB2, tmA, tmM, tmO[0], tmO[1], tmO[2]);
        } else {
          k_umma_pair<MODE><<<2 * clusters, kPairThreads, kPairSmemBytes, ctx->stream>>>(a, tmB, tmB2, tmA, tmM, tmO[0], tmO[1], tmO[2]);
        }
    }
#else
    if (pu1) {
      if (!(ctx->umma_attr_set & 16)) {
        NTRU_CUDA(ctx, cudaFuncSetAttribute(k_umma_pair<ENC, 0, 1>, cudaFuncAttributeMaxDynamicSharedMemorySize, (int)kPairSmemBytes));
        ctx->umma_attr_set |= 16;
      }
      k_umma_pair<ENC, 0, 1><<<2 * clusters, kPairThreads, kPairSmemBytes, ctx->stream>>>(a, tmB, tmB2, tmA, tmM, tmO[0], tmO[1], tmO[2]);
    } else {
      k_umma_pair<MODE><<<2 * clusters, kPairThreads, kPairSmemBytes, ctx->stream>>>(a, tmB, tmB2, tmA, tmM, tmO[0], tmO[1], tmO[2]);
    }
#endif
  }
  NTRU_CUDA(ctx, cudaGetLastError());
  return NTRU_OK;
}

}

#ifdef NTRU_TRACE
extern "C" int ntru_debug_trace_dump(unsigned long long *out, unsigned int cap) {
  cudaDeviceSynchronize();
  const unsigned int n = kTraceLanes * kTraceCap;
  if (cap < n) return -1;
  cudaMemcpyFromSymbol(out, g_trace, sizeof(unsigned long long) * n);
  return (int)n;
}
#endif

int umma_init(ntru_ctx *ctx) {
  ctx->tensor_ok = false;
  cudaDeviceProp prop;
  if (cudaGetDeviceProperties(&prop, ctx->device) != cudaSuccess) return NTRU_OK;
  if (prop.major != 10) return NTRU_OK;
  if ((size_t)prop.sharedMemPerBlockOptin < kPairSmemBytes) return NTRU_OK;
  if (!get_encode_fn()) return NTRU_OK;
  ctx->tensor_ok = true;
  return NTRU_OK;
}

int umma_prepare_public(ntru_ctx *ctx) {
  return build_keymat(ctx, ENC, 1, ctx->q > 256 ? 2 : 1, ctx->d_h.ptr, ctx->km_h);
}

int umma_prepare_private(ntru_ctx *ctx) {
  const bool f16 = ctx->q > 256 && ctx->q <= 2048 && ctx->opt_dec1_form != 1;
  int rc = f16 ? build_keymat(ctx, DEC1F, 1, 1, ctx->d_f.ptr, ctx->km_f)
               : build_keymat(ctx, DEC1, ctx->q > 256 ? 2 : 1, 1, ctx->d_f.ptr, ctx->km_f);
  ctx->km_f.f16 = f16;
  if (rc) return rc;
  return build_keymat(ctx, DEC2, 1, 1, ctx->d_fp.ptr, ctx->km_fp);
}

int umma_encrypt(ntru_ctx *ctx, size_t B, const uint8_t *r, const uint8_t *m, uint16_t *value, uint16_t *quo,
                 uint16_t *rem) {
  if (B == 0) return NTRU_OK;
  UmmaArgs a = {};
  a.B = B; a.m = m;
  a.with_hi = quo != nullptr;
  a.o16_cyc = value ? value : rem;
  a.o16_cyc2 = value ? rem : nullptr;
  a.o16_hi = quo;
  return launch_product<ENC>(ctx, ctx->km_h, a, r);
}

int umma_decrypt(ntru_ctx *ctx, size_t B, const uint16_t *e, uint8_t *value, uint16_t *q1, uint16_t *r1, uint8_t *q2,
                 uint8_t *r2) {
  if (B == 0) return NTRU_OK;
  NTRU_CUDA(ctx, ctx->d_b.reserve(B * (size_t)ctx->P));
  UmmaArgs a = {};
  a.B = B; a.a_src = e;
  a.with_hi = q1 != nullptr;
  a.o16_cyc = r1; a.o16_hi = q1; a.o8_cyc = (uint8_t *)ctx->d_b.ptr;
  int rc = ctx->km_f.f16 ? launch_product<DEC1F>(ctx, ctx->km_f, a, nullptr) : launch_product<DEC1>(ctx, ctx->km_f, a, nullptr);
  if (rc) return rc;
#ifdef NTRU_TRACE
  if (getenv("NTRU_TRACE_DEC1_ONLY")) return NTRU_OK;
#endif
  UmmaArgs b = {};
  b.B = B;
  b.with_hi = q2 != nullptr;
  b.o8_cyc = value ? value : r2;
  b.o8_cyc2 = value ? r2 : nullptr;
  b.o8_hi = q2;
  return launch_product<DEC2>(ctx, ctx->km_fp, b, ctx->d_b.ptr);
}

}
```

### ntru-circom_b200/csrc/umma_pair.cuh

```cuda

#ifdef NTRU_TRACE
constexpr int kTraceLanes = 4, kTraceCap = 2048;
__device__ unsigned long long g_trace[kTraceLanes * kTraceCap];
#define TRACE(role, ev, idx)                                                                      \
  do {                                                                                            \
    if (blockIdx.x == 0 && !(a.debug_flags & 16) && trace_n[role - 1] < kTraceCap) {              \
      g_trace[(role - 1) * kTraceCap + trace_n[role - 1]++] =                                     \
          ((unsigned long long)(((ev) << 12) | ((idx) & 0xfff)) << 40) | (clock64() & 0xffffffffffull); \
    }                                                                                             \
  } while (0)
#define TRACE_NS(role, ev, idx)                                                                   \
  do {                                                                                            \
    if (blockIdx.x == 0 && !(a.debug_flags & 16) && trace_n[role - 1] < kTraceCap) {              \
      unsigned long long _ns;                                                                     \
      asm volatile("mov.u64 %0, %%globaltimer;" : "=l"(_ns));                                     \
      g_trace[(role - 1) * kTraceCap + trace_n[role - 1]++] =                                     \
          ((unsigned long long)(((ev) << 12) | ((idx) & 0xfff)) << 40) | (_ns & 0xffffffffffull); \
    }                                                                                             \
  } while (0)
#else
#define TRACE(role, ev, idx) do {} while (0)
#define TRACE_NS(role, ev, idx) do {} while (0)
#endif

constexpr int kSlotBytes = 16384;
constexpr int kPairSlots = 14;
constexpr int kPairBars = 4 * kPairSlots + 8;
constexpr int kPairProducerWarp = 16, kPairMmaWarp = 17, kPairAuxWarp = 18, kPairEpiWarp0Dec1 = 8;
constexpr int kPairThreads = 19 * 32;
constexpr size_t kPairSmemBytes = (size_t)kPairSlots * kSlotBytes + 1024  + 8 * kPairBars + 64;

__device__ __forceinline__ uint32_t cluster_ctarank() {
  uint32_t r;
  asm volatile("mov.u32 %0, %%cluster_ctarank;" : "=r"(r));
  return r;
}
__device__ __forceinline__ uint32_t mapa_u32(uint32_t addr, uint32_t rank) {
  uint32_t r;
  asm volatile("mapa.shared::cluster.u32 %0, %1, %2;" : "=r"(r) : "r"(addr), "r"(rank));
  return r;
}
__device__ __forceinline__ void cluster_sync_all() {
  asm volatile("barrier.cluster.arrive.release.aligned;" ::: "memory");
  asm volatile("barrier.cluster.wait.acquire.aligned;" ::: "memory");
}
__device__ __forceinline__ void mbar_arrive_cluster(uint32_t cluster_addr) {
  asm volatile("mbarrier.arrive.shared::cluster.b64 _, [%0];" ::"r"(cluster_addr) : "memory");
}
__device__ __forceinline__ void tma_load_2d_pair(uint32_t dst, const CUtensorMap *map, int c0, int c1, uint32_t bar_cluster) {
  asm volatile(
      "cp.async.bulk.tensor.2d.cta_group::2.shared::cluster.global.mbarrier::complete_tx::bytes [%0], [%1, {%2, %3}], [%4];" ::"r"(dst),
      "l"(map), "r"(c0), "r"(c1), "r"(bar_cluster)
      : "memory");
}
template <bool F16>
__device__ __forceinline__ void umma_pair(uint32_t tmem_d, uint64_t desc_a, uint64_t desc_b, uint32_t idesc,
                                          uint32_t accumulate) {
  if (F16) {
    asm volatile(
        "{\n\t"
        ".reg .pred p;\n\t"
        "setp.ne.b32 p, %4, 0;\n\t"
        "tcgen05.mma.cta_group::2.kind::f16 [%0], %1, %2, %3, p;\n\t"
        "}" ::"r"(tmem_d), "l"(desc_a), "l"(desc_b), "r"(idesc), "r"(accumulate)
        : "memory");
  } else {
    asm volatile(
        "{\n\t"
        ".reg .pred p;\n\t"
        "setp.ne.b32 p, %4, 0;\n\t"
        "tcgen05.mma.cta_group::2.kind::i8 [%0], %1, %2, %3, p;\n\t"
        "}" ::"r"(tmem_d), "l"(desc_a), "l"(desc_b), "r"(idesc), "r"(accumulate)
        : "memory");
  }
}
__device__ __forceinline__ void umma_commit_pair(uint32_t bar) {
  asm volatile(
      "tcgen05.commit.cta_group::2.mbarrier::arrive::one.shared::cluster.multicast::cluster.b64 [%0], %1;" ::"r"(bar),
      "h"((uint16_t)3)
      : "memory");
}
__device__ __forceinline__ void tma_store_2d(const CUtensorMap *map, uint32_t src, int c0, int c1) {
  asm volatile("cp.async.bulk.tensor.2d.global.shared::cta.bulk_group [%0, {%2, %3}], [%1];" ::"l"(map), "r"(src), "r"(c0),
               "r"(c1)
               : "memory");
}
__device__ __forceinline__ void sts128(uint32_t addr, uint4 v) {
  asm volatile("st.shared.v4.b32 [%0], {%1, %2, %3, %4};" ::"r"(addr), "r"(v.x), "r"(v.y), "r"(v.z), "r"(v.w) : "memory");
}
__device__ __forceinline__ uint4 lds128(uint32_t addr) {
  uint4 v;
  asm volatile("ld.shared.v4.b32 {%0, %1, %2, %3}, [%4];" : "=r"(v.x), "=r"(v.y), "=r"(v.z), "=r"(v.w) : "r"(addr) : "memory");
  return v;
}
__device__ __forceinline__ bool elect_one() {
  uint32_t pred;
  asm volatile(
      "{\n\t"
      ".reg .pred P;\n\t"
      ".reg .b32 r;\n\t"
      "elect.sync r|P, 0xffffffff;\n\t"
      "selp.b32 %0, 1, 0, P;\n\t"
      "}" : "=r"(pred));
  return pred != 0;
}
__host__ __device__ constexpr uint32_t make_idesc_pair(int a_signed, int b_signed, int n) {
  return (2u << 4) | ((uint32_t)a_signed << 7) | ((uint32_t)b_signed << 10) | ((uint32_t)(n >> 3) << 17) |
         ((uint32_t)(256 >> 4) << 24);
}
__host__ __device__ constexpr uint32_t make_idesc_pair_f16(int n) {
  return (1u << 4) | ((uint32_t)(n >> 3) << 17) | ((uint32_t)(256 >> 4) << 24);
}

template <int MODE, int DBG = 0, int PU = (MODE == 2 ? 4 : 2)>
__global__ void __cluster_dims__(2, 1, 1) __launch_bounds__(kPairThreads, 1)
k_umma_pair(const UmmaArgs a, const __grid_constant__ CUtensorMap tmapB, const __grid_constant__ CUtensorMap tmapB2,
            const __grid_constant__ CUtensorMap tmapA,
            const __grid_constant__ CUtensorMap tmapM, const __grid_constant__ CUtensorMap tmapO0,
            const __grid_constant__ CUtensorMap tmapO1, const __grid_constant__ CUtensorMap tmapO2) {
  extern __shared__ uint8_t smem_raw[];
  uint8_t *smem = reinterpret_cast<uint8_t *>((reinterpret_cast<uintptr_t>(smem_raw) + 1023) & ~(uintptr_t)1023);
  uint64_t *bars = reinterpret_cast<uint64_t *>(smem + (size_t)kPairSlots * kSlotBytes);
  uint32_t *tmem_slot = reinterpret_cast<uint32_t *>(bars + kPairBars);
  const uint32_t bar0 = smem_u32(bars);
  auto a_full = [&](uint32_t i) { return bar0 + 8u * i; };
  auto a_empty = [&](uint32_t i) { return bar0 + 8u * (kPairSlots + i); };
  auto b_full = [&](uint32_t i) { return bar0 + 8u * (2 * kPairSlots + i); };
  auto b_empty = [&](uint32_t i) { return bar0 + 8u * (3 * kPairSlots + i); };
  auto tfull_bar = [&](uint32_t b) { return bar0 + 8u * (4 * kPairSlots + b); };
  auto tempty_bar = [&](uint32_t b) { return bar0 + 8u * (4 * kPairSlots + 2 + b); };
  auto m_full = [&](uint32_t b) { return bar0 + 8u * (4 * kPairSlots + 4 + b); };
  auto m_empty = [&](uint32_t b) { return bar0 + 8u * (4 * kPairSlots + 6 + b); };
  const uint32_t smem_base = smem_u32(smem);
  auto a_slot = [&](uint32_t i) { return smem_base + i * kSlotBytes; };
  auto b_slot = [&](uint32_t j) { return smem_base + (a.nA + j) * kSlotBytes; };
  auto m_slot = [&](uint32_t j) { return smem_base + (a.nA + a.nB + j) * kSlotBytes; };
  const uint32_t stage_base = smem_base + (a.nA + a.nB + a.nM) * kSlotBytes;

#ifdef NTRU_TRACE
  int trace_n[kTraceLanes] = {0, 0, 0, 0};
#endif
  const int warp = threadIdx.x >> 5, lane = threadIdx.x & 31;
  const uint32_t rank = cluster_ctarank();
  const bool leader = rank == 0;
  constexpr int kEpiWarps = MODE == DEC1 ? 8 : 16;

  if (threadIdx.x == 0) {
    for (int i = 0; i < a.nA; ++i) {
      mbar_init(a_full(i), MODE == DEC1 ? 16 : 2);
      mbar_init(a_empty(i), a.a_rel);
    }
    if (MODE == DEC1 && a.a_tma) {
      for (int j = 0; j < (a.nA >> 1); ++j) mbar_init(a_full(a.nA + j), 1);
    }
    for (int j = 0; j < a.nB; ++j) {
      mbar_init(b_full(j), 2);
      mbar_init(b_empty(j), 1);
    }
    for (int b = 0; b < 2; ++b) {
      mbar_init(tfull_bar(b), 1);
      mbar_init(tempty_bar(b), a.one_group ? 2 * kEpiWarps : kEpiWarps);
      mbar_init(m_full(b), 1);
      mbar_init(m_empty(b), a.one_group ? kEpiWarps : kEpiWarps / 2);
    }
    fence_barrier_init();
  }
  if (warp == kPairMmaWarp) {
    asm volatile("tcgen05.alloc.cta_group::2.sync.aligned.shared::cta.b32 [%0], %1;" ::"r"(smem_u32(tmem_slot)), "n"(512));
    asm volatile("tcgen05.relinquish_alloc_permit.cta_group::2.sync.aligned;");
  }
  tc_fence_before();
  cluster_sync_all();
  tc_fence_after();
  const uint32_t tmem_base = *tmem_slot;
  auto lead = [&](uint32_t local_bar) { return mapa_u32(local_bar, 0); };

  if (warp == kPairProducerWarp) {
    const uint32_t lead_b_full = lead(b_full(0));
    const int part_rows = a.mat_rows / 3;
    uint32_t sb = 0, b_par = 0;
#ifdef NTRU_TRACE
    int gs = 0;
#endif
    if (lane == 0) { TRACE(3, 10, 0); TRACE_NS(3, 11, 0); }
    for (int T = blockIdx.x >> 1; T < a.npairs; T += gridDim.x >> 1) {
      for (int j = 0; j < a.nph; ++j) {
        const Phase ph = a.ph[j];
        const int c = ph.c;
        const int wc = a.col0[c + 1] - a.col0[c];
        const int half_rows = (a.nl * wc) >> 1;
        const uint32_t b_bytes = 2u * (uint32_t)half_rows * kAtomK;
        const CUtensorMap *bmap = wc == a.w0 ? &tmapB : &tmapB2;
        const int row0 = ph.kind * part_rows + a.nl * a.col0[c] + (int)rank * half_rows;
        for (int at = ph.a0; at < ph.a1; ++at) {
          for (int lk = 0; lk < a.kl; ++lk) {
#ifdef NTRU_TRACE
            if (lane == 0 && (a.debug_flags & 4)) TRACE(3, 0, gs);
#endif
            mbar_wait(b_empty(sb), b_par ^ 1);
#ifdef NTRU_TRACE
            if (lane == 0 && (a.debug_flags & 4)) TRACE(3, 1, gs);
            ++gs;
#endif
            if (elect_one()) {
#ifdef NTRU_TRACE
              if (a.debug_flags & 1) {
                if (leader) mbar_arrive(b_full(sb)); else mbar_arrive_cluster(lead_b_full + 8u * sb);
              } else
#endif
              {
                if (leader) mbar_arrive_expect_tx(b_full(sb), b_bytes);
                else mbar_arrive_cluster(lead_b_full + 8u * sb);
                tma_load_2d_pair(b_slot(sb), bmap, 0, (lk * a.atoms + at) * a.mat_rows + row0, lead_b_full + 8u * sb);
              }
            }
            __syncwarp();
            if (++sb == (uint32_t)a.nB) { sb = 0; b_par ^= 1; }
          }
        }
      }
    }
    if (lane == 0) { TRACE(3, 12, 0); TRACE_NS(3, 13, 0); }
  } else if (warp == kPairAuxWarp) {
    if (MODE == DEC1) {
      if (a.a_tma) {
        const uint32_t np = (uint32_t)a.nA >> 1;
        uint32_t pj = 0, par = 0;
        for (int T = blockIdx.x >> 1; T < a.npairs; T += gridDim.x >> 1) {
          const int a_row = T * 256 + (int)rank * kTileRows;
          for (int j = 0; j < a.nph; ++j) {
            const int at1 = a.ph[j].a1;
            for (int at = a.ph[j].a0; at < at1; ++at) {
              mbar_wait(a_empty(2 * pj), par ^ 1);
              mbar_wait(a_empty(2 * pj + 1), par ^ 1);
              if (elect_one()) {
                mbar_arrive_expect_tx(a_full(a.nA + pj), 2u * kABytes);
                tma_load_2d(a_slot(2 * pj), &tmapA, at * kAtomK, a_row, a_full(a.nA + pj));
              }
              __syncwarp();
              if (++pj == np) { pj = 0; par ^= 1; }
            }
          }
        }
      }
    } else {
      const uint32_t a_bytes = 2u * kABytes;
      const uint32_t lead_a_full = lead(a_full(0));
      const bool resident = a.a_resident != 0;
      uint32_t sas = 0, a_par_s = 0, t_par = 0, mc = 0;
      auto load_a = [&](uint32_t sa, uint32_t par, int at, int a_row) {
        mbar_wait(a_empty(sa), par ^ 1);
        if (elect_one()) {
          if (leader) mbar_arrive_expect_tx(a_full(sa), a_bytes);
          else mbar_arrive_cluster(lead_a_full + 8u * sa);
          tma_load_2d_pair(a_slot(sa), &tmapA, at * a.ea, a_row, lead_a_full + 8u * sa);
        }
        __syncwarp();
      };
      for (int T = blockIdx.x >> 1; T < a.npairs; T += gridDim.x >> 1, t_par ^= 1) {
        const int a_row = T * 256 + (int)rank * kTileRows;
        if (resident) {
          for (int k = 0; k < a.atoms; ++k) load_a((uint32_t)a.a_order[k], t_par, a.a_order[k], a_row);
        }
        for (int j = 0; j < a.nph; ++j) {
          const Phase ph = a.ph[j];
          if (!resident) {
            for (int at = ph.a0; at < ph.a1; ++at) {
              load_a(sas, a_par_s, at, a_row);
              if (++sas == (uint32_t)a.nA) { sas = 0; a_par_s ^= 1; }
            }
          }
          if (MODE == ENC && PU != 1 && ph.kind != PH_HI) {
            const uint32_t ms = mc & 1;
            mbar_wait(m_empty(ms), ((mc >> 1) & 1) ^ 1);
            if (elect_one()) {
              mbar_arrive_expect_tx(m_full(ms), kABytes);
              tma_load_2d(m_slot(ms), &tmapM, a.col0[ph.c], a_row, m_full(ms));
            }
            __syncwarp();
            ++mc;
          }
        }
      }
    }
  } else if (warp == kPairMmaWarp) {
    if (leader) {
      const uint64_t desc_hi = make_smem_desc(0) & ~0x3FFFull;
      const uint32_t a_lo0 = smem_base >> 4, b_lo0 = (smem_base + a.nA * kSlotBytes) >> 4;
      const bool resident = a.a_resident != 0;
      const uint32_t nB = (uint32_t)a.nB, nA = (uint32_t)a.nA;
      const uint32_t bfull0 = b_full(0), bempty0 = b_empty(0), afull0 = a_full(0), aempty0 = a_empty(0);
      const uint32_t klast = (uint32_t)a.k_last, kl_u = (uint32_t)a.kl;
      uint32_t sb = 0, b_par = 0;
      uint32_t sas = 0, a_par_s = 0;
      uint32_t cc = 0, t_par = 0;
#ifdef NTRU_TRACE
      int gs = 0;
      const bool light = (a.debug_flags & 16) != 0;
      unsigned long long lp_tmem = 0, lp_ops = 0, lp_issue = 0, lp_other = 0, lp_slices = 0, lp_phases = 0;
      uint32_t lp_t = light ? (uint32_t)clock() : 0u;
#define LP_ADD(acc) do { if (light) { const uint32_t now_ = (uint32_t)clock(); acc += now_ - lp_t; lp_t = now_; } } while (0)
      const long long lp_start = clock64();
#else
#define LP_ADD(acc) do {} while (0)
#endif
      for (int T = blockIdx.x >> 1; T < a.npairs; T += gridDim.x >> 1, t_par ^= 1) {
        for (int j = 0; j < a.nph; ++j, ++cc) {
          const Phase ph = a.ph[j];
          const uint32_t nsl = (uint32_t)(ph.a1 - ph.a0) * kl_u;
          const int wc = a.col0[ph.c + 1] - a.col0[ph.c];
          const uint32_t idesc = MODE == DEC1F ? make_idesc_pair_f16(wc) : make_idesc_pair(0, MODE == DEC1 ? 1 : 0, a.nl * wc);
          const uint32_t first = resident ? ph.first : 0xffffu, rel = resident ? ph.rel : 0xffffu;
          const uint32_t buf = cc & 1;
          if (lane == 0) TRACE(1, 0, cc);
          LP_ADD(lp_other);
          mbar_wait(tempty_bar(buf), ((cc >> 1) & 1) ^ 1);
          LP_ADD(lp_tmem);
#ifdef NTRU_TRACE
          ++lp_phases;
#endif
          if (lane == 0) TRACE(1, 1, cc);
          const uint32_t d_tmem = tmem_base + buf * kAccCols;
          const uint32_t tfull = tfull_bar(buf);
          uint32_t sa = resident ? (uint32_t)ph.a0 * kl_u : sas;
          uint32_t at = (uint32_t)ph.a0, lk = 0;
          uint32_t accumulate = ph.kind == PH_LO ? 1u : 0u;
          for (uint32_t i = 0; i < nsl; ++i) {
            LP_ADD(lp_other);
            if ((first >> at) & 1u) mbar_wait((lane & 1) ? afull0 + 8u * sa : bfull0 + 8u * sb, (lane & 1) ? (resident ? t_par : a_par_s) : b_par);
            else mbar_wait(bfull0 + 8u * sb, b_par);
            __syncwarp();
            LP_ADD(lp_ops);
#ifdef NTRU_TRACE
            if (lane == 0) TRACE(1, 3, (a.debug_flags & 4) ? gs : (int)cc);
#endif
            tc_fence_after();
            const uint64_t da = desc_hi | (uint64_t)(a_lo0 + sa * (kSlotBytes >> 4));
            const uint64_t db = desc_hi | (uint64_t)(b_lo0 + sb * (kSlotBytes >> 4));
#ifdef NTRU_TRACE
            const uint32_t nk = (a.debug_flags & 2) ? 1u : (at == (uint32_t)(a.atoms - 1) ? klast : 4u);
#else
            const uint32_t nk = at == (uint32_t)(a.atoms - 1) ? klast : 4u;
#endif
            if (elect_one()) {
              umma_pair<MODE == DEC1F>(d_tmem, da, db, idesc, accumulate);
              if (nk > 1) umma_pair<MODE == DEC1F>(d_tmem, da + 2, db + 2, idesc, 1u);
              if (nk > 2) umma_pair<MODE == DEC1F>(d_tmem, da + 4, db + 4, idesc, 1u);
              if (nk > 3) umma_pair<MODE == DEC1F>(d_tmem, da + 6, db + 6, idesc, 1u);
#ifdef NTRU_TRACE
              if (a.debug_flags & 32) {
                umma_pair<MODE == DEC1F>(d_tmem, da, db, idesc, 1u);
                umma_pair<MODE == DEC1F>(d_tmem, da + 2, db + 2, idesc, 1u);
                umma_pair<MODE == DEC1F>(d_tmem, da + 4, db + 4, idesc, 1u);
                umma_pair<MODE == DEC1F>(d_tmem, da + 6, db + 6, idesc, 1u);
              }
#endif
              umma_commit_pair(bempty0 + 8u * sb);
              if ((rel >> at) & 1u) umma_commit_pair(aempty0 + 8u * sa);
              if (i == nsl - 1) umma_commit_pair(tfull);
            }
            __syncwarp();
            LP_ADD(lp_issue);
#ifdef NTRU_TRACE
            if (lane == 0) TRACE(1, 5, (a.debug_flags & 4) ? gs : (int)cc);
            ++gs;
            ++lp_slices;
#endif
            accumulate = 1;
            if (++sb == nB) { sb = 0; b_par ^= 1; }
            if (++lk == kl_u) { lk = 0; ++at; }
            if (resident) {
              ++sa;
            } else {
              if (++sas == nA) { sas = 0; a_par_s ^= 1; }
              sa = sas;
            }
          }
        }
      }
#ifdef NTRU_TRACE
      if (light && blockIdx.x == 0 && lane == 0) {
        g_trace[0] = 0x4c50ull << 48;
        g_trace[1] = (unsigned long long)(clock64() - lp_start);
        g_trace[2] = lp_tmem; g_trace[3] = lp_ops; g_trace[4] = lp_issue; g_trace[5] = lp_other; g_trace[6] = lp_slices; g_trace[7] = lp_phases;
      }
#endif
  }
  } else if (MODE == DEC1 && warp < kPairEpiWarp0Dec1) {
    const int t = threadIdx.x;
    const int chunk = t & 7;
    const int r0 = t >> 3;
    if (a.a_tma) {
      const uint32_t np = (uint32_t)a.nA >> 1;
      const uint32_t lead_a_full = lead(a_full(0));
      const uint32_t sel = (uint32_t)(chunk >> 2) & 1u;
      uint32_t pj = 0, par = 0;
      int xn = 0;
      int per_tile = 0;
      for (int j = 0; j < a.nph; ++j) per_tile += a.ph[j].a1 - a.ph[j].a0;
      for (int T = blockIdx.x >> 1; T < a.npairs; T += gridDim.x >> 1) {
            for (int v = 0; v < per_tile; ++v, ++xn) {
              if (t == 0) TRACE(4, 0, xn);
              mbar_wait(a_full(a.nA + pj), par);
              if (t == 0) TRACE(4, 1, xn);
              const uint32_t raw0 = a_slot(2 * pj);
              uint4 w[8];
#pragma unroll
              for (int j = 0; j < 4; ++j) {
                const uint32_t base = raw0 + (uint32_t)(r0 + 32 * j) * 256u + (uint32_t)chunk * 32u;
                const uint4 x = lds128(base + sel * 16u), y = lds128(base + (sel ^ 1u) * 16u);
                w[2 * j] = sel ? y : x;
                w[2 * j + 1] = sel ? x : y;
              }
              asm volatile("bar.sync 1, 256;" ::: "memory");
#pragma unroll
              for (int j = 0; j < 4; ++j) {
                const int r_in = r0 + 32 * j;
                const uint32_t off = (uint32_t)((r_in >> 3) * 1024 + (r_in & 7) * 128 + ((chunk ^ (r_in & 7)) << 4));
                const uint4 w0 = w[2 * j], w1 = w[2 * j + 1];
                sts128(raw0 + off, make_uint4(__byte_perm(w0.x, w0.y, 0x6420), __byte_perm(w0.z, w0.w, 0x6420),
                                              __byte_perm(w1.x, w1.y, 0x6420), __byte_perm(w1.z, w1.w, 0x6420)));
                sts128(raw0 + kSlotBytes + off,
                       make_uint4(__byte_perm((w0.x >> 6) & 0x00FC00FCu, (w0.y >> 6) & 0x00FC00FCu, 0x6420),
                                  __byte_perm((w0.z >> 6) & 0x00FC00FCu, (w0.w >> 6) & 0x00FC00FCu, 0x6420),
                                  __byte_perm((w1.x >> 6) & 0x00FC00FCu, (w1.y >> 6) & 0x00FC00FCu, 0x6420),
                                  __byte_perm((w1.z >> 6) & 0x00FC00FCu, (w1.w >> 6) & 0x00FC00FCu, 0x6420)));
              }
              fence_proxy_async();
              __syncwarp();
              if (lane == 0) {
                mbar_arrive_cluster(lead_a_full + 16u * pj);
                mbar_arrive_cluster(lead_a_full + 16u * pj + 8u);
              }
              if (t == 0) TRACE(4, 5, xn);
              if (++pj == np) { pj = 0; par ^= 1; }
            }
      }
    } else {
    const uint16_t *src = reinterpret_cast<const uint16_t *>(a.a_src);
    struct Item { int T, j, k, at; uint32_t ia; int titer; bool valid; };
    auto advance = [&](Item &w) {
      if (a.a_resident) {
        if (++w.k < a.atoms) { w.at = a.a_order[w.k]; return; }
      } else {
        w.ia += a.kl;
        if (++w.at < a.ph[w.j].a1) return;
        if (++w.j < a.nph) { w.at = a.ph[w.j].a0; return; }
      }
      w.T += gridDim.x >> 1;
      ++w.titer;
      w.valid = w.T < a.npairs;
      w.j = 0; w.k = 0;
      w.at = a.a_resident ? a.a_order[0] : a.ph[0].a0;
    };
    auto load_atom = [&](const Item &w, uint4 (&raw)[8]) {
      const int col = w.at * kAtomK + chunk * 16;
#pragma unroll
      for (int j = 0; j < 4; ++j) {
        const size_t row = (size_t)w.T * 256 + rank * kTileRows + r0 + 32 * j;
        const bool ok = w.valid && row < a.B && col < a.P;
        const uint4 *ptr = reinterpret_cast<const uint4 *>(src + (ok ? row * (size_t)a.P + col : 0));
        uint4 x0 = __ldg(ptr), x1 = __ldg(ptr + 1);
        if (!ok) x0 = x1 = make_uint4(0, 0, 0, 0);
        raw[2 * j] = x0;
        raw[2 * j + 1] = x1;
      }
    };
    Item cur;
    cur.T = blockIdx.x >> 1; cur.j = 0; cur.k = 0; cur.ia = 0; cur.titer = 0;
    cur.valid = cur.T < a.npairs;
    cur.at = a.a_resident ? a.a_order[0] : a.ph[0].a0;
    uint4 raw[8], raw_next[8];
    int xn = 0;
    if (cur.valid) load_atom(cur, raw);
    while (cur.valid) {
      Item nxt = cur;
      advance(nxt);
      load_atom(nxt, raw_next);
      uint32_t sa0, sa1, par0, par1;
      if (a.a_resident) {
        sa0 = cur.at * a.kl; sa1 = sa0 + 1; par0 = par1 = cur.titer & 1;
      } else {
        sa0 = cur.ia % a.nA; par0 = (cur.ia / a.nA) & 1;
        sa1 = (cur.ia + 1) % a.nA; par1 = ((cur.ia + 1) / a.nA) & 1;
      }
      if (t == 0) TRACE(4, 0, xn);
      mbar_wait(a_empty(sa0), par0 ^ 1);
      if (a.kl == 2) mbar_wait(a_empty(sa1), par1 ^ 1);
      if (t == 0) TRACE(4, 1, xn);
      uint8_t *dst0 = smem + (size_t)sa0 * kSlotBytes;
      uint8_t *dst1 = smem + (size_t)sa1 * kSlotBytes;
#pragma unroll
      for (int j = 0; j < 4; ++j) {
        const int r_in = r0 + 32 * j;
        const int off = (r_in >> 3) * 1024 + (r_in & 7) * 128 + ((chunk ^ (r_in & 7)) << 4);
        const uint4 w0 = raw[2 * j], w1 = raw[2 * j + 1];
        uint4 lo;
        lo.x = __byte_perm(w0.x, w0.y, 0x6420);
        lo.y = __byte_perm(w0.z, w0.w, 0x6420);
        lo.z = __byte_perm(w1.x, w1.y, 0x6420);
        lo.w = __byte_perm(w1.z, w1.w, 0x6420);
        *reinterpret_cast<uint4 *>(dst0 + off) = lo;
        if (a.kl == 2) {
          uint4 hi4;
          hi4.x = __byte_perm((w0.x >> 6) & 0x00FC00FCu, (w0.y >> 6) & 0x00FC00FCu, 0x6420);
          hi4.y = __byte_perm((w0.z >> 6) & 0x00FC00FCu, (w0.w >> 6) & 0x00FC00FCu, 0x6420);
          hi4.z = __byte_perm((w1.x >> 6) & 0x00FC00FCu, (w1.y >> 6) & 0x00FC00FCu, 0x6420);
          hi4.w = __byte_perm((w1.z >> 6) & 0x00FC00FCu, (w1.w >> 6) & 0x00FC00FCu, 0x6420);
          *reinterpret_cast<uint4 *>(dst1 + off) = hi4;
        }
      }
      fence_proxy_async();
      __syncwarp();
      if (lane == 0) {
        mbar_arrive_cluster(lead(a_full(sa0)));
        if (a.kl == 2) mbar_arrive_cluster(lead(a_full(sa1)));
      }
      if (t == 0) TRACE(4, 5, xn);
      ++xn;
      cur = nxt;
#pragma unroll
      for (int j = 0; j < 8; ++j) raw[j] = raw_next[j];
    }
    }
  } else {
    const int kSub = (a.one_group ? kEpiWarps : kEpiWarps / 2) / 4;
    constexpr bool kMsgGlobal = MODE == ENC && PU == 1;
    constexpr int kPassUnits = PU;
    const int ew = warp - (MODE == DEC1 ? kPairEpiWarp0Dec1 : 0);
    const int quad = warp & 3;
    const uint32_t grp = (uint32_t)(ew >> 2) & 1u;
    const int sub = a.one_group ? ew >> 2 : ew >> 3;
    const uint32_t Q2 = a.qmask | (a.qmask << 16);
    const uint32_t LA2 = (((uint32_t)a.q >> 1) - 1u) * 0x00010001u;
    const int logq = 31 - __clz(a.q);
    constexpr uint32_t kRowBytes = (MODE == DEC2 ? 16u : 32u) * PU;
    static_assert(kRowBytes == 64 || kRowBytes == 32, "staging rows are one 64-byte or 32-byte swizzle span");
    const uint32_t stage = stage_base + (uint32_t)ew * (MODE == DEC1 ? 4096u : 32u * kRowBytes);
    const uint32_t st_row = stage + (uint32_t)lane * kRowBytes;
    const uint32_t st_x = kRowBytes == 64 ? (uint32_t)(lane >> 1) & 3u : (uint32_t)(lane >> 2) & 1u;
    const int row_in_tile = quad * 32 + lane;
    const uint32_t m_row = (uint32_t)((row_in_tile >> 3) * 1024 + (row_in_tile & 7) * 128), m_x = (uint32_t)row_in_tile & 7u;
    const uint32_t t_addr0 = tmem_base + ((uint32_t)(quad * 32) << 16);
    const uint32_t tfull0 = tfull_bar(0), lead_tempty0 = lead(tempty_bar(0));
    uint32_t cc = 0, mc = 0;
    bool store_pending = false;
    for (int T = blockIdx.x >> 1; T < a.npairs; T += gridDim.x >> 1) {
      const int out_row = T * 256 + (int)rank * kTileRows + quad * 32;
      {
        for (int jp = 0; jp < a.nph; ++jp, ++cc) {
          const int c = a.ph[jp].c;
          const int hi = a.ph[jp].kind == PH_HI;
          const uint32_t ms = mc & 1, m_par = (mc >> 1) & 1;
          if (MODE == ENC && !hi) ++mc;
          if (!a.one_group && (cc & 1u) != grp) continue;
          const uint32_t buf = cc & 1u;
          const uint32_t t_addr = t_addr0 + buf * kAccCols, my_tfull = tfull0 + 8u * buf, lead_tempty = lead_tempty0 + 8u * buf;
          const int col0c = a.col0[c], wc = a.col0[c + 1] - col0c;
          const int upw = (wc >> 4) / kSub;
          const int npass = upw / kPassUnits;
          if (lane == 0 && ew == 0) TRACE(2, 0, cc);
          uint4 mg[4];
          if (kMsgGlobal && !hi) {
            const size_t grow = (size_t)(out_row + lane);
#pragma unroll
            for (int j = 0; j < 4; ++j) {
              const int col = col0c + (sub * upw + j) * 16;
              mg[j] = (j < upw && grow < a.B && col < a.N) ? __ldg(reinterpret_cast<const uint4 *>(a.m + grow * (size_t)a.P + col))
                                                          : make_uint4(0, 0, 0, 0);
            }
          }
          mbar_wait(my_tfull, (cc >> 1) & 1);
          tc_fence_after();
          if (lane == 0 && ew == 0) TRACE(2, 1, cc);
          if (MODE == ENC && !kMsgGlobal && !hi) mbar_wait(m_full(ms), m_par);
          if (lane == 0 && ew == 0) TRACE(2, 3, cc);
          if (DBG & 1) {
            tc_fence_before();
            __syncwarp();
            if (lane == 0) {
              mbar_arrive_cluster(lead_tempty);
              if (MODE == ENC && !kMsgGlobal && !hi) mbar_arrive(m_empty(ms));
            }
            continue;
          }
          int npe = (a.P - (col0c + sub * upw * 16) + kPassUnits * 16 - 1) / (kPassUnits * 16);
          npe = npe < 0 ? 0 : (npe > npass ? npass : npe);
          if (npe == 0) {
            tc_fence_before();
            __syncwarp();
            if (lane == 0) {
              mbar_arrive_cluster(lead_tempty);
              if (MODE == ENC && !kMsgGlobal && !hi) mbar_arrive(m_empty(ms));
            }
            continue;
          }
          for (int ps = 0; ps < npe; ++ps) {
            const int u0 = sub * upw + ps * kPassUnits;
            const bool last_pass = ps == npe - 1;
            uint32_t res[kPassUnits * (MODE == DEC2 ? 4 : 8)];
            uint32_t bres[kPassUnits * 4];
            uint4 mm[kPassUnits];
            if (kMsgGlobal) {
              if (!hi) {
                mm[0] = ps == 0 ? mg[0] : (ps == 1 ? mg[1] : (ps == 2 ? mg[2] : mg[3]));
                const int keep = a.N - (col0c + u0 * 16);
                if (keep < 16) {
                  uint32_t w[4] = {mm[0].x, mm[0].y, mm[0].z, mm[0].w};
#pragma unroll
                  for (int t = 0; t < 4; ++t) {
                    const int kb = keep - 4 * t;
                    w[t] = kb >= 4 ? w[t] : (kb <= 0 ? 0u : (w[t] & ((1u << (8 * kb)) - 1u)));
                  }
                  mm[0] = make_uint4(w[0], w[1], w[2], w[3]);
                }
              }
            } else if (MODE == ENC && !hi) {
#pragma unroll
              for (int j = 0; j < kPassUnits; ++j) mm[j] = lds128(m_slot(ms) + m_row + ((((uint32_t)(u0 + j)) ^ m_x) << 4));
            }
            uint32_t acc[kPassUnits][32];
            {
              uint32_t acc1[kPassUnits][32];
#pragma unroll
              for (int j = 0; j < kPassUnits; ++j) {
                if (DBG & 4) {
#pragma unroll
                  for (int i = 0; i < 16; ++i) { acc[j][i] = (uint32_t)(i + lane + ps); acc1[j][i] = (uint32_t)(i ^ lane); }
                  continue;
                }
                tmem_ld16(t_addr + (u0 + j) * 16, acc[j]);
                if (MODE == ENC && a.nl == 2) tmem_ld16(t_addr + wc + (u0 + j) * 16, acc1[j]);
              }
              if (!(DBG & 4)) tmem_ld_wait();
              if (lane == 0 && ew == 0) TRACE(2, 4, cc);
              if (MODE == ENC && a.nl == 2) {
#pragma unroll
                for (int j = 0; j < kPassUnits; ++j)
#pragma unroll
                  for (int i = 0; i < 16; ++i) acc[j][i] += acc1[j][i] << 8;
              }
              if (MODE == DEC1F) {
#pragma unroll
                for (int j = 0; j < kPassUnits; ++j)
#pragma unroll
                  for (int i = 0; i < 16; ++i) acc[j][i] = __float_as_uint(__uint_as_float(acc[j][i]) + 0.75f);
              }
            }
            if (last_pass) {
              tc_fence_before();
              __syncwarp();
              if (lane == 0) {
                mbar_arrive_cluster(lead_tempty);
                if (MODE == ENC && !kMsgGlobal && !hi) mbar_arrive(m_empty(ms));
              }
            }
            if (DBG & 2) {
              uint32_t x = 0;
#pragma unroll
              for (int j = 0; j < kPassUnits; ++j) x ^= acc[j][0] ^ acc[j][15];
              if (x == 0x12345678u) sts128(st_row, make_uint4(x, x, x, x));
              continue;
            }
#pragma unroll
            for (int j = 0; j < kPassUnits; ++j) {
              uint32_t (&w)[32] = acc[j];
              if (MODE == ENC || MODE == DEC1 || MODE == DEC1F) {
                uint32_t *pk = res + 8 * j;
#pragma unroll
                for (int jj = 0; jj < 8; ++jj) pk[jj] = __byte_perm(w[2 * jj], w[2 * jj + 1], 0x5410);
                if (hi) {
#pragma unroll
                  for (int jj = 0; jj < 8; ++jj) pk[jj] = ((~pk[jj] & Q2) + 0x00010001u) & Q2;
                } else if (MODE == ENC) {
                  const uint32_t mw[4] = {mm[j].x, mm[j].y, mm[j].z, mm[j].w};
#pragma unroll
                  for (int jj = 0; jj < 8; ++jj) {
                    const uint32_t mp = __byte_perm(mw[jj >> 1], 0u, (jj & 1) ? 0x4342 : 0x4140);
                    pk[jj] = __vadd2(pk[jj], mp) & Q2;
                  }
                } else {
#pragma unroll
                  for (int jj = 0; jj < 8; ++jj) pk[jj] &= Q2;
                  if (a.o8_cyc) {
                    if (logq & 1) {
#pragma unroll
                      for (int wd = 0; wd < 4; ++wd) {
                        uint32_t y2[2];
#pragma unroll
                        for (int i = 0; i < 2; ++i) {
                          const uint32_t y = (pk[2 * wd + i] + LA2) & Q2;
                          y2[i] = y - 63u * ((y >> 6) & 0x00FF00FFu);
                        }
                        bres[4 * j + wd] = __byte_perm(y2[0], y2[1], 0x6420);
                      }
                    } else {
#pragma unroll
                      for (int wd = 0; wd < 4; ++wd) {
                        uint32_t y2[2];
#pragma unroll
                        for (int i = 0; i < 2; ++i) {
                          const uint32_t x = pk[2 * wd + i];
                          const uint32_t y = x + (((x + LA2) >> logq) & 0x00010001u);
                          y2[i] = y - 63u * ((y >> 6) & 0x00FF00FFu);
                        }
                        bres[4 * j + wd] = __byte_perm(y2[0], y2[1], 0x6420);
                      }
                    }
                  }
                }
              } else {
#pragma unroll
                for (int wd = 0; wd < 4; ++wd) {
                  uint32_t bb[4];
#pragma unroll
                  for (int i = 0; i < 4; ++i) {
                    const uint32_t y = hi ? 2u * w[4 * wd + i] : w[4 * wd + i];
                    bb[i] = y - 3u * __umulhi(y, 0x55555556u);
                  }
                  res[4 * j + wd] = __byte_perm(__byte_perm(bb[0], bb[1], 0x0040), __byte_perm(bb[2], bb[3], 0x0040), 0x5410);
                }
              }
            }
            if (lane == 0 && ew == 0) TRACE(2, 5, cc);
            if (DBG & 8) {
              uint32_t x = 0;
#pragma unroll
              for (int j = 0; j < kPassUnits * (MODE == DEC2 ? 4 : 8); ++j) x ^= res[j];
              if (x == 0x12345678u) sts128(st_row, make_uint4(x, x, x, x));
              continue;
            }
            if (store_pending) {
              if (lane == 0) asm volatile("cp.async.bulk.wait_group.read 0;" ::: "memory");
              __syncwarp();
            }
            if (MODE == DEC2) {
#pragma unroll
              for (int j = 0; j < kPassUnits; ++j)
                sts128(st_row + ((((uint32_t)j) ^ st_x) << 4), make_uint4(res[4 * j], res[4 * j + 1], res[4 * j + 2], res[4 * j + 3]));
            } else {
#pragma unroll
              for (int j = 0; j < kPassUnits; ++j) {
                sts128(st_row + ((((uint32_t)(2 * j)) ^ st_x) << 4), make_uint4(res[8 * j], res[8 * j + 1], res[8 * j + 2], res[8 * j + 3]));
                sts128(st_row + ((((uint32_t)(2 * j + 1)) ^ st_x) << 4), make_uint4(res[8 * j + 4], res[8 * j + 5], res[8 * j + 6], res[8 * j + 7]));
              }
              if (MODE == DEC1 && !hi && a.o8_cyc) {
#pragma unroll
                for (int j = 0; j < kPassUnits; ++j)
                  sts128(stage + 2048u + (uint32_t)lane * 32u + (uint32_t)j * 16u,
                         make_uint4(bres[4 * j], bres[4 * j + 1], bres[4 * j + 2], bres[4 * j + 3]));
              }
              if (MODE == DEC1F && !hi && a.o8_cyc) {
                const size_t grow = (size_t)(out_row + lane);
                const int col = col0c + u0 * 16;
                if (grow < a.B) {
#pragma unroll
                  for (int j = 0; j < kPassUnits; ++j)
                    if (col + 16 * j < a.P)
                      *reinterpret_cast<uint4 *>(a.o8_cyc + grow * (size_t)a.P + col + 16 * j) =
                          make_uint4(bres[4 * j], bres[4 * j + 1], bres[4 * j + 2], bres[4 * j + 3]);
                }
              }
            }
            if (lane == 0 && ew == 0) TRACE(2, 6, cc);
            fence_proxy_async();
            __syncwarp();
            if (lane == 0 && ew == 0) TRACE(2, 7, cc);
            if (DBG & 16) continue;
            if (lane == 0) {
              const int col = col0c + u0 * 16;
              if (hi) {
                if (a.out_mask & 4) tma_store_2d(&tmapO2, stage, col, out_row);
              } else {
                if (a.out_mask & 1) tma_store_2d(&tmapO0, stage, col, out_row);
                if (MODE == DEC1) {
                  if (a.out_mask & 2) tma_store_2d(&tmapO1, stage + 2048, col, out_row);
                } else {
                  if (a.out_mask & 2) tma_store_2d(&tmapO1, stage, col, out_row);
                }
              }
              asm volatile("cp.async.bulk.commit_group;" ::: "memory");
            }
            store_pending = true;
          }
          if (lane == 0 && ew == 0) TRACE(2, 2, cc);
        }
      }
    }
    if (lane == 0) asm volatile("cp.async.bulk.wait_group 0;" ::: "memory");
  }

#ifdef NTRU_TRACE
  if (blockIdx.x == 0 && lane == 0 && !(a.debug_flags & 16)) {
    const int role = warp == kPairProducerWarp ? 3 : (warp == kPairMmaWarp ? 1 : (warp == (MODE == DEC1 ? kPairEpiWarp0Dec1 : 0) ? 2 : (MODE == DEC1 && warp == 0 ? 4 : 0)));
    if (role && trace_n[role - 1] < kTraceCap) g_trace[(role - 1) * kTraceCap + trace_n[role - 1]] = 0ull;
  }
#endif
  tc_fence_before();
  cluster_sync_all();
  if (warp == kPairMmaWarp) {
    __syncwarp();
    asm volatile("tcgen05.dealloc.cta_group::2.sync.aligned.b32 %0, %1;" ::"r"(tmem_base), "n"(512));
  }
}
```

### ntru-circom_b200/engine.py

```python
from __future__ import annotations

import ctypes
from typing import Optional

import numpy as np

from . import _lib
from ._lib import NtruError


def _ptr(a) -> Optional[int]:
    if a is None:
        return None
    if isinstance(a, int):
        return a
    if isinstance(a, np.ndarray):
        return a.ctypes.data
    if hasattr(a, "data_ptr"):
        return a.data_ptr()
    raise TypeError(f"cannot take the address of {type(a)}")


def _host(a, dtype, shape) -> np.ndarray:
    if hasattr(a, "numpy") and not isinstance(a, np.ndarray):
        a = a.numpy()
    a = np.ascontiguousarray(a, dtype=dtype)
    if a.shape != tuple(shape):
        raise IndexError(f"RangeError: expected shape {tuple(shape)}, got {a.shape}")
    return a


class Engine:

    def __init__(self, N: int, p: int, q: int, device: int = 0):
        self.lib = _lib.load()
        self.N, self.p, self.q = int(N), int(p), int(q)
        h = ctypes.c_void_p()
        rc = self.lib.ntru_create(ctypes.byref(h), self.N, self.p, self.q, int(device))
        if rc != _lib.NTRU_OK:
            raise NtruError(rc, {_lib.NTRU_E_CUDA: "no usable CUDA device (this engine has no CPU fallback)",
                                 _lib.NTRU_E_PARAM: "unsupported parameters N/p/q"}.get(
                                     rc, self.lib.ntru_strerror(rc).decode()))
        self._h = h
        self.device = int(device)
        self.pitch = int(self.lib.ntru_pitch(h))

    def close(self):
        if getattr(self, "_h", None):
            self.lib.ntru_destroy(self._h)
            self._h = None

    def __del__(self):
        try:
            self.close()
        except Exception:
            pass

    def _check(self, rc: int):
        if rc != _lib.NTRU_OK:
            raise NtruError(rc, self.lib.ntru_last_error(self._h).decode() or self.lib.ntru_strerror(rc).decode())

    def set_option(self, key: int, value: int):
        self._check(self.lib.ntru_set_option(self._h, key, value))

    def set_path(self, path: int):
        self.set_option(_lib.NTRU_OPT_PATH, path)

    def set_dec1_form(self, form: int):
        self.set_option(_lib.NTRU_OPT_DEC1_FORM, int(form))

    def set_schedule(self, cyc_plus_hi: bool):
        self.set_option(_lib.NTRU_OPT_SCHEDULE, 1 if cyc_plus_hi else 0)

    def set_epilogue(self, mode: int):
        self.set_option(_lib.NTRU_OPT_EPILOGUE, int(mode))

    def set_imma_form(self, generic: bool):
        self.set_option(_lib.NTRU_OPT_IMMA_FORM, 1 if generic else 0)

    @property
    def launch_count(self) -> int:
        return int(self.lib.ntru_launch_count(self._h))

    @property
    def last_path(self) -> int:
        return int(self.lib.ntru_last_path(self._h))

    def set_timing(self, on: bool):
        self.set_option(_lib.NTRU_OPT_TIMING, 1 if on else 0)

    def timing_reset(self):
        self._check(self.lib.ntru_timing_reset(self._h))

    def timing_read(self) -> dict:
        out = {}
        for i, name in enumerate(_lib.KERNEL_KINDS):
            ms, n = ctypes.c_double(0), ctypes.c_uint64(0)
            self._check(self.lib.ntru_timing_read(self._h, i, ctypes.byref(ms), ctypes.byref(n)))
            if n.value:
                out[name] = (ms.value, int(n.value))
        return out

    def stream(self) -> int:
        return int(self.lib.ntru_stream(self._h) or 0)

    def set_stream(self, cuda_stream: int):
        self._check(self.lib.ntru_set_stream(self._h, cuda_stream))

    def sync(self):
        self._check(self.lib.ntru_sync(self._h))

    def set_public_key(self, h):
        h = _host(h, np.uint16, (self.N,))
        self._check(self.lib.ntru_set_public_key(self._h, _ptr(h)))

    def set_private_key(self, f, fp):
        f = _host(f, np.int8, (self.N,))
        fp = _host(fp, np.uint8, (self.N,))
        self._check(self.lib.ntru_set_private_key(self._h, _ptr(f), _ptr(fp)))

    def encrypt_batch(self, r, m, *, h=None, witness=True, out=None, dr=None, return_r=False):
        N = self.N
        m_arr = np.asarray(m)
        B = m_arr.shape[0]
        if r is not None:
            r = _host(np.ascontiguousarray(r, dtype=np.uint8), np.uint8, (B, N))
        elif dr is not None:
            self.set_dr(dr)
        wide = m_arr.dtype.itemsize > 1 and m_arr.size and int(m_arr.max(initial=0)) > 255
        m_arr = _host(m_arr, np.uint16 if wide else np.uint8, (B, N))
        out = out or {}
        value = out.get("value", np.empty((B, N), dtype=np.uint16))
        quo = out.get("quotientE", np.empty((B, N + 1), dtype=np.uint16)) if witness else None
        rem = out.get("remainderE", np.empty((B, N + 1), dtype=np.uint16)) if witness else None
        r_out = out.get("r", np.empty((B, N), dtype=np.uint8)) if (return_r or r is None) else None
        if h is not None:
            if wide:
                raise NtruError(_lib.NTRU_E_UNSUPPORTED, "wide messages with per-row keys")
            h = _host(h, np.uint16, (B, N))
            rc = self.lib.ntru_encrypt_batch_keys(self._h, B, _ptr(h), _ptr(r), _ptr(m_arr), _ptr(value),
                                                  _ptr(quo), _ptr(rem), _ptr(r_out))
        elif wide:
            rc = self.lib.ntru_encrypt_batch_wide(self._h, B, _ptr(r), _ptr(m_arr), _ptr(value), _ptr(quo),
                                                  _ptr(rem), _ptr(r_out))
        else:
            rc = self.lib.ntru_encrypt_batch(self._h, B, _ptr(r), _ptr(m_arr), _ptr(value), _ptr(quo), _ptr(rem),
                                             _ptr(r_out))
        self._check(rc)
        res = {"value": value, "quotientE": quo, "remainderE": rem}
        if r_out is not None:
            res["r"] = r_out
        return res

    def decrypt_batch(self, e, *, f=None, fp=None, witness=True, out=None):
        N = self.N
        e = np.ascontiguousarray(e, dtype=np.uint16)
        B = e.shape[0]
        e = _host(e, np.uint16, (B, N))
        out = out or {}
        value = out.get("value", np.empty((B, N), dtype=np.uint8))
        q1 = out.get("quotient1", np.empty((B, N + 1), dtype=np.uint16)) if witness else None
        r1 = out.get("remainder1", np.empty((B, N + 1), dtype=np.uint16)) if witness else None
        q2 = out.get("quotient2", np.empty((B, N + 1), dtype=np.uint8)) if witness else None
        r2 = out.get("remainder2", np.empty((B, N + 1), dtype=np.uint8)) if witness else None
        if f is not None or fp is not None:
            f = _host(f, np.int8, (B, N))
            fp = _host(fp, np.uint8, (B, N))
            rc = self.lib.ntru_decrypt_batch_keys(self._h, B, _ptr(f), _ptr(fp), _ptr(e), _ptr(value), _ptr(q1),
                                                  _ptr(r1), _ptr(q2), _ptr(r2))
        else:
            rc = self.lib.ntru_decrypt_batch(self._h, B, _ptr(e), _ptr(value), _ptr(q1), _ptr(r1), _ptr(q2),
                                             _ptr(r2))
        self._check(rc)
        return {"value": value, "quotient1": q1, "remainder1": r1, "quotient2": q2, "remainder2": r2}

    def packed_elems(self, mod_q: bool, width: int) -> int:
        return int(self.lib.ntru_packed_elems(self._h, 1 if mod_q else 0, int(width)))

    def _fe(self, arr, mod_q, width, B):
        return _host(np.ascontiguousarray(arr, dtype=np.uint32), np.uint32, (B, self.packed_elems(mod_q, width), 8))

    def encrypt_batch_packed(self, r, m, *, witness=True, out=None, dr=None, return_r=False):
        N = self.N
        m = np.ascontiguousarray(m, dtype=np.uint32)
        B = m.shape[0]
        m = self._fe(m, False, N, B)
        if r is not None:
            r = self._fe(r, False, N, B)
        elif dr is not None:
            self.set_dr(dr)
        out = out or {}
        value = out.get("value", np.empty((B, self.packed_elems(True, N), 8), dtype=np.uint32))
        quo = out.get("quotientE", np.empty((B, self.packed_elems(True, N + 1), 8), dtype=np.uint32)) if witness else None
        rem = out.get("remainderE", np.empty((B, self.packed_elems(True, N + 1), 8), dtype=np.uint32)) if witness else None
        r_out = out.get("r", np.empty((B, self.packed_elems(False, N), 8), dtype=np.uint32)) if (return_r or r is None) else None
        self._check(self.lib.ntru_encrypt_batch_packed(self._h, B, _ptr(r), _ptr(m), _ptr(value), _ptr(quo), _ptr(rem), _ptr(r_out)))
        res = {"value": value, "quotientE": quo, "remainderE": rem}
        if r_out is not None:
            res["r"] = r_out
        return res

    def decrypt_batch_packed(self, e, *, witness=True, out=None):
        N = self.N
        e = np.ascontiguousarray(e, dtype=np.uint32)
        B = e.shape[0]
        e = self._fe(e, True, N, B)
        out = out or {}
        value = out.get("value", np.empty((B, self.packed_elems(False, N), 8), dtype=np.uint32))
        q1 = out.get("quotient1", np.empty((B, self.packed_elems(True, N + 1), 8), dtype=np.uint32)) if witness else None
        r1 = out.get("remainder1", np.empty((B, self.packed_elems(True, N + 1), 8), dtype=np.uint32)) if witness else None
        q2 = out.get("quotient2", np.empty((B, self.packed_elems(False, N + 1), 8), dtype=np.uint32)) if witness else None
        r2 = out.get("remainder2", np.empty((B, self.packed_elems(False, N + 1), 8), dtype=np.uint32)) if witness else None
        self._check(self.lib.ntru_decrypt_batch_packed(self._h, B, _ptr(e), _ptr(value), _ptr(q1), _ptr(r1), _ptr(q2), _ptr(r2)))
        return {"value": value, "quotient1": q1, "remainder1": r1, "quotient2": q2, "remainder2": r2}

    def verify_keys_batch(self, f, fq, fp, g):
        N = self.N
        f = np.ascontiguousarray(f, dtype=np.int8)
        B = f.shape[0]
        f = _host(f, np.int8, (B, N))
        fq = _host(fq, np.uint16, (B, N))
        fp = _host(fp, np.uint8, (B, N))
        g = _host(g, np.int8, (B, N))
        out = {k: np.empty((B, N + 1), dtype=np.uint8 if k.endswith("_fp") else np.uint16)
               for k in ("quotient_fq", "remainder_fq", "quotient_fp", "remainder_fp", "quotient_h", "remainder_h")}
        self._check(self.lib.ntru_verify_keys_batch(self._h, B, _ptr(f), _ptr(fq), _ptr(fp), _ptr(g),
                                                    *[_ptr(out[k]) for k in ("quotient_fq", "remainder_fq", "quotient_fp",
                                                                             "remainder_fp", "quotient_h", "remainder_h")]))
        return out

    def keygen_batch(self, f, g):
        N = self.N
        f = np.ascontiguousarray(f, dtype=np.int8)
        B = f.shape[0]
        f = _host(f, np.int8, (B, N))
        g = _host(g, np.int8, (B, N))
        fq = np.empty((B, N), dtype=np.uint16)
        fp = np.empty((B, N), dtype=np.uint8)
        h = np.empty((B, N), dtype=np.uint16)
        valid = np.empty(B, dtype=np.uint8)
        self._check(self.lib.ntru_keygen_batch(self._h, B, _ptr(f), _ptr(g), _ptr(fq), _ptr(fp), _ptr(h), _ptr(valid)))
        return {"fq": fq, "fp": fp, "h": h, "valid": valid.astype(bool)}

    def muldiv_dev(self, B, x, y, mod_p, quotient=None, remainder=None):
        self._check(self.lib.ntru_muldiv_dev(self._h, B, _ptr(x), _ptr(y), int(bool(mod_p)), _ptr(quotient), _ptr(remainder)))

    def pack_geometry(self, max_val: int, data_len: int):
        v = [ctypes.c_int() for _ in range(4)]
        self._check(self.lib.ntru_pack_geometry(int(max_val), int(data_len), *[ctypes.byref(x) for x in v]))
        return tuple(x.value for x in v)

    def pack_output_dev(self, B, data, elem_bytes, data_len, pitch, max_val, out):
        self._check(self.lib.ntru_pack_output_dev(self._h, B, _ptr(data), int(elem_bytes), int(data_len), int(pitch), int(max_val),
                                                  _ptr(out)))

    def unpack_input_dev(self, B, data, n_elems, max_val, packed_bits, out, elem_bytes, pitch):
        self._check(self.lib.ntru_unpack_input_dev(self._h, B, _ptr(data), int(n_elems), int(max_val), int(packed_bits), _ptr(out),
                                                   int(elem_bytes), int(pitch)))

    def pack_output(self, max_val: int, data):
        data = np.ascontiguousarray(data)
        if data.dtype not in (np.uint8, np.uint16):
            raise TypeError("pack_output takes uint8 or uint16 rows")
        B, n = data.shape
        outs = self.pack_geometry(max_val, n)[3]
        out = np.empty((B, outs, 8), dtype=np.uint32)
        self._check(self.lib.ntru_pack_output(self._h, B, _ptr(data), data.dtype.itemsize, n, int(max_val), _ptr(out)))
        return out

    def unpack_input(self, max_val: int, packed_bits: int, packed, dtype=np.uint16):
        packed = np.ascontiguousarray(packed, dtype=np.uint32)
        B, n_elems = packed.shape[0], packed.shape[1]
        bits = max(1, int(max_val).bit_length())
        out = np.empty((B, (packed_bits // bits) * n_elems), dtype=dtype)
        self._check(self.lib.ntru_unpack_input(self._h, B, _ptr(packed), n_elems, int(max_val), int(packed_bits), _ptr(out),
                                               out.dtype.itemsize))
        return out

    def sum_allreduce(self, e):
        e = np.ascontiguousarray(e, dtype=np.uint16)
        B = e.shape[0]
        e = _host(e, np.uint16, (B, self.N))
        out = np.empty(self.N, dtype=np.uint16)
        self._check(self.lib.ntru_sum_allreduce(self._h, B, _ptr(e) if B else None, _ptr(out)))
        return out

    def sum(self, e):
        e = np.ascontiguousarray(e, dtype=np.uint16)
        B = e.shape[0]
        e = _host(e, np.uint16, (B, self.N))
        out = np.empty(self.N, dtype=np.uint16)
        self._check(self.lib.ntru_sum(self._h, B, _ptr(e), _ptr(out)))
        return out

    def encrypt_dev(self, B, r, m, value=None, quotientE=None, remainderE=None, h_rows=None):
        self._check(self.lib.ntru_encrypt_dev(self._h, B, _ptr(h_rows), _ptr(r), _ptr(m), _ptr(value),
                                              _ptr(quotientE), _ptr(remainderE)))

    def decrypt_dev(self, B, e, value=None, quotient1=None, remainder1=None, quotient2=None, remainder2=None,
                    f_rows=None, fp_rows=None):
        self._check(self.lib.ntru_decrypt_dev(self._h, B, _ptr(f_rows), _ptr(fp_rows), _ptr(e), _ptr(value),
                                              _ptr(quotient1), _ptr(remainder1), _ptr(quotient2),
                                              _ptr(remainder2)))

    def sum_partial_dev(self, B, e, partial):
        self._check(self.lib.ntru_sum_partial_dev(self._h, B, _ptr(e), _ptr(partial)))

    def sum_finalize_dev(self, partial, out):
        self._check(self.lib.ntru_sum_finalize_dev(self._h, _ptr(partial), _ptr(out)))

    def xchg_create(self, world: int, rank: int) -> bytes:
        buf = (ctypes.c_ubyte * 64)()
        self._check(self.lib.ntru_xchg_create(self._h, int(world), int(rank), buf))
        return bytes(buf)

    def xchg_connect(self, handles: bytes):
        buf = (ctypes.c_ubyte * len(handles)).from_buffer_copy(handles)
        self._check(self.lib.ntru_xchg_connect(self._h, buf))

    def sum_allreduce_dev(self, B, e, out):
        self._check(self.lib.ntru_sum_allreduce_dev(self._h, B, _ptr(e) if B else None, _ptr(out)))

    def sample_r_dev(self, B, dr, row0, r, seed=None):
        if seed is not None:
            self.set_rng_key(seed_key(seed), self.rng_next_row)
        self._check(self.lib.ntru_sample_r_dev(self._h, B, int(dr), int(row0), _ptr(r)))

    def set_dr(self, dr: int):
        self.set_option(_lib.NTRU_OPT_DR, int(dr))

    def set_rng_key(self, key: bytes, first_row: int = 0):
        if len(key) != 32:
            raise ValueError("the ChaCha20 key is 32 bytes")
        buf = (ctypes.c_ubyte * 32).from_buffer_copy(bytes(key))
        self._check(self.lib.ntru_set_rng_key(self._h, buf, int(first_row)))

    @property
    def rng_next_row(self) -> int:
        return int(self.lib.ntru_rng_next_row(self._h))

    def xchg_destroy(self):
        self._check(self.lib.ntru_xchg_destroy(self._h))


_M32 = 0xFFFFFFFF


def seed_key(seed: int) -> bytes:
    return int(seed).to_bytes(32, "little")


def chacha20_block(key: bytes, counter: int, nonce: int):
    k = [int.from_bytes(key[4 * i:4 * i + 4], "little") for i in range(8)]
    st = [0x61707865, 0x3320646E, 0x79622D32, 0x6B206574, *k,
          counter & _M32, (counter >> 32) & _M32, nonce & _M32, (nonce >> 32) & _M32]
    x = list(st)

    def rotl(v, n):
        return ((v << n) & _M32) | (v >> (32 - n))

    def qr(a, b, c, d):
        x[a] = (x[a] + x[b]) & _M32; x[d] = rotl(x[d] ^ x[a], 16)
        x[c] = (x[c] + x[d]) & _M32; x[b] = rotl(x[b] ^ x[c], 12)
        x[a] = (x[a] + x[b]) & _M32; x[d] = rotl(x[d] ^ x[a], 8)
        x[c] = (x[c] + x[d]) & _M32; x[b] = rotl(x[b] ^ x[c], 7)

    for _ in range(10):
        qr(0, 4, 8, 12); qr(1, 5, 9, 13); qr(2, 6, 10, 14); qr(3, 7, 11, 15)
        qr(0, 5, 10, 15); qr(1, 6, 11, 12); qr(2, 7, 8, 13); qr(3, 4, 9, 14)
    return [(a + b) & _M32 for a, b in zip(x, st)]


def sampler_draws(key: bytes, row: int, count: int):
    out = []
    blk = 0
    while len(out) < count:
        out.extend(chacha20_block(key, blk, row))
        blk += 1
    return out[:count]
```

Before: 614.6 million.

## Fuse both decrypt products into one pipelined tcgen05 kernel with smem-resident intermediate

Adds a fused DEC mode that runs the f*e product (DEC1F) and the fp*b product (DEC2) in a single persistent kernel. The intermediate mod-p result is written by the epilogue into resident shared-memory slots instead of global memory, and the second product for tile T-stride is interleaved with the first product for tile T. This removes a kernel launch and the global round trip of the intermediate buffer. The cost is a more complex phase schedule, fewer B-pipeline slots because resident slots are reserved, and extra barrier coupling between the epilogue and MMA warps. It is on by default whenever the key layout qualifies (opt_dec_fused=0).

Result: slower. 590.4 million, median of 6 (-3.9%).

```diff
diff --git a/include/ntru_b200.h b/include/ntru_b200.h
--- a/include/ntru_b200.h
+++ b/include/ntru_b200.h
@@ -29,7 +29,8 @@
   NTRU_OPT_DEC1_FORM = 6,
   NTRU_OPT_SCHEDULE = 7,
   NTRU_OPT_EPILOGUE = 8,
-  NTRU_OPT_IMMA_FORM = 9
+  NTRU_OPT_IMMA_FORM = 9,
+  NTRU_OPT_DEC_FUSED = 10
 };
 
 enum {
@@ -44,7 +45,8 @@
   NTRU_K_DEC_IMMA = 8,
   NTRU_K_MULDIV = 9,
   NTRU_K_PACK = 10,
-  NTRU_K_COUNT = 11
+  NTRU_K_DEC_TENSOR = 11,
+  NTRU_K_COUNT = 12
 };
 
 int ntru_create(ntru_ctx **ctx, int N, int p, int q, int device);
diff --git a/ntru-circom_b200/_lib.py b/ntru-circom_b200/_lib.py
--- a/ntru-circom_b200/_lib.py
+++ b/ntru-circom_b200/_lib.py
@@ -11,9 +11,9 @@
 NTRU_E_PARAM, NTRU_E_LENGTH, NTRU_E_NOKEY, NTRU_E_CUDA = -1, -2, -3, -4
 NTRU_E_NCCL, NTRU_E_NOMEM, NTRU_E_UNSUPPORTED = -5, -6, -7
 NTRU_OPT_PATH, NTRU_OPT_CHUNK_ROWS, NTRU_OPT_TIMING, NTRU_OPT_DR, NTRU_OPT_DEC1_FORM, NTRU_OPT_SCHEDULE, NTRU_OPT_EPILOGUE = 1, 2, 3, 5, 6, 7, 8
-NTRU_OPT_IMMA_FORM = 9
+NTRU_OPT_IMMA_FORM, NTRU_OPT_DEC_FUSED = 9, 10
 KERNEL_KINDS = ["enc_tensor", "dec1_tensor", "dec2_tensor", "enc_core", "dec_core", "sum", "other", "enc_imma", "dec_imma",
-                "muldiv", "pack"]
+                "muldiv", "pack", "dec_tensor"]
 PATH_AUTO, PATH_CUDA_CORE, PATH_TENSOR, PATH_IMMA = 0, 1, 2, 3
 
 _P = c_void_p
diff --git a/ntru-circom_b200/csrc/api.cu b/ntru-circom_b200/csrc/api.cu
--- a/ntru-circom_b200/csrc/api.cu
+++ b/ntru-circom_b200/csrc/api.cu
@@ -370,6 +370,10 @@
       ctx->opt_dec1_form = (int)value;
       if (ctx->has_priv && ctx->tensor_ok) return umma_prepare_private(ctx);
       return NTRU_OK;
+    case NTRU_OPT_DEC_FUSED:
+      if (value < 0 || value > 2) return fail(ctx, NTRU_E_PARAM, "NTRU_OPT_DEC_FUSED must be 0, 1 or 2");
+      ctx->opt_dec_fused = (int)value;
+      return NTRU_OK;
     case NTRU_OPT_DR:
       if (value < 0 || 2 * value > ctx->N) return fail(ctx, NTRU_E_PARAM, "The total of 1s and -1s cannot exceed the array length.");
       ctx->opt_dr = (int)value;
diff --git a/ntru-circom_b200/csrc/ntru_internal.cuh b/ntru-circom_b200/csrc/ntru_internal.cuh
--- a/ntru-circom_b200/csrc/ntru_internal.cuh
+++ b/ntru-circom_b200/csrc/ntru_internal.cuh
@@ -74,6 +74,7 @@
   int opt_epilogue = 0;
   int opt_lohi = 0;
   int opt_dec1_form = 0;
+  int opt_dec_fused = 0;
   int umma_attr_set = 0;
   bool sampler_attr_set = false;
   uint32_t rng_key[8] = {};
diff --git a/ntru-circom_b200/csrc/umma_kernels.cu b/ntru-circom_b200/csrc/umma_kernels.cu
--- a/ntru-circom_b200/csrc/umma_kernels.cu
+++ b/ntru-circom_b200/csrc/umma_kernels.cu
@@ -5,13 +5,15 @@
 #include <stdlib.h>
 #include <string.h>
 
+#include <type_traits>
+
 #include "ntru_internal.cuh"
 
 namespace ntru {
 
 namespace {
 
-enum Mode { ENC = 0, DEC1 = 1, DEC2 = 2, DEC1F = 3 };
+enum Mode { ENC = 0, DEC1 = 1, DEC2 = 2, DEC1F = 3, DEC = 4 };
 
 constexpr int kTileRows = 128;
 constexpr int kAtomK = 128;
@@ -22,6 +24,7 @@
 enum PhaseKind { PH_CYC = 0, PH_HI = 1, PH_LO = 2 };
 struct Phase {
   int8_t c, kind, a0, a1;
+  int8_t prod;
   uint16_t first, rel;
 };
 
@@ -42,6 +45,9 @@
   size_t B;
   int npairs;
   int nA, nB;
+  int nR;
+  int atoms2, k_last2;
+  int out_mask2;
   int a_resident;
   int a_tma;
   int nM, nS;
@@ -306,12 +312,18 @@
       if (!(seen >> at & 1u)) { seen |= 1u << at; a.ph[j].rel |= (uint16_t)(1u << at); }
 }
 
+struct ProductMaps {
+  CUtensorMap b, b2, a, m, o[3];
+};
+
+template <int MODE, int DBG = 0, int PU = (MODE == DEC2 ? 4 : 2)>
+void launch_pair(ntru_ctx *ctx, int clusters, const UmmaArgs &a, const ProductMaps &t, const ProductMaps &t2) {
+  k_umma_pair<MODE, DBG, PU><<<2 * clusters, kPairThreads, kPairSmemBytes, ctx->stream>>>(
+      a, t.b, t.b2, t.a, t.m, t.o[0], t.o[1], t.o[2], t2.b, t2.b2, t2.o[0], t2.o[1], t2.o[2]);
+}
+
 template <int MODE>
-int launch_product(ntru_ctx *ctx, const KeyMatrix &km, UmmaArgs &a, const void *a_bytes) {
-  if (!(ctx->umma_attr_set & (1 << MODE))) {
-    NTRU_CUDA(ctx, cudaFuncSetAttribute(k_umma_pair<MODE>, cudaFuncAttributeMaxDynamicSharedMemorySize, (int)kPairSmemBytes));
-    ctx->umma_attr_set |= 1 << MODE;
-  }
+int setup_product(ntru_ctx *ctx, const KeyMatrix &km, UmmaArgs &a, const void *a_bytes, ProductMaps &t, bool *pu1_out) {
   a.N = ctx->N; a.P = ctx->P; a.kl = km.limbs; a.nl = km.nlimbs; a.Kp = km.klen / km.limbs; a.atoms = a.Kp / kAtomK;
   a.ea = MODE == DEC1F ? kAtomK / 2 : kAtomK;
   a.ea_shift = MODE == DEC1F ? 6 : 7;
@@ -326,6 +338,7 @@
   a.nM = MODE == ENC ? 2 : 0;
   const int a_slots = a.atoms * a.kl;
   const bool pu1 = MODE == ENC && a.atoms >= 5;
+  *pu1_out = pu1;
   if (pu1) { a.nS = 1; a.nM = 0; }
   const int avail = kPairSlots - a.nS - a.nM;
   if (a_slots + 4 <= avail) {
@@ -338,18 +351,16 @@
   a.two_issuers = 0;
   a.a_rel = (a.a_resident && a.two_issuers) ? 2 : 1;
   a.one_group = one_group_mode(ctx, MODE) ? 1 : 0;
-  CUtensorMap tmB, tmB2, tmA, tmM, tmO[3];
-  memcpy(&tmB, km.tmap_half[0], sizeof tmB);
-  memcpy(&tmB2, km.tmap_half[1], sizeof tmB2);
-  memset(&tmA, 0, sizeof tmA);
-  memset(&tmM, 0, sizeof tmM);
-  memset(tmO, 0, sizeof tmO);
+  memset(&t, 0, sizeof t);
+  memcpy(&t.b, km.tmap_half[0], sizeof t.b);
+  memcpy(&t.b2, km.tmap_half[1], sizeof t.b2);
+  CUtensorMap &tmA = t.a, &tmM = t.m, *tmO = t.o;
   const uint64_t N = (uint64_t)ctx->N, P = (uint64_t)ctx->P;
   int rc;
   if (MODE == DEC1F) {
     rc = encode_2d_ex(ctx, &tmA, const_cast<void *>(a.a_src), 2, N, (uint64_t)a.B, P * 2, kAtomK / 2, kTileRows, CU_TENSOR_MAP_SWIZZLE_128B);
     if (rc) return rc;
-  } else if (MODE != DEC1) {
+  } else if (MODE == ENC || (MODE == DEC2 && a_bytes)) {
     rc = encode_2d(ctx, &tmA, const_cast<void *>(a_bytes), N, (uint64_t)a.B, P, kAtomK, kTileRows);
     if (rc) return rc;
   } else if (a.a_tma) {
@@ -403,6 +414,20 @@
       }
     }
   }
+  return NTRU_OK;
+}
+
+template <int MODE>
+int launch_product(ntru_ctx *ctx, const KeyMatrix &km, UmmaArgs &a, const void *a_bytes) {
+  if (!(ctx->umma_attr_set & (1 << MODE))) {
+    NTRU_CUDA(ctx, cudaFuncSetAttribute(k_umma_pair<MODE>, cudaFuncAttributeMaxDynamicSharedMemorySize, (int)kPairSmemBytes));
+    ctx->umma_attr_set |= 1 << MODE;
+  }
+  ProductMaps t, none;
+  memset(&none, 0, sizeof none);
+  bool pu1 = false;
+  int rc = setup_product<MODE>(ctx, km, a, a_bytes, t, &pu1);
+  if (rc) return rc;
   {
     LaunchTimer timer(ctx, MODE == ENC ? NTRU_K_ENC_TENSOR : (MODE == DEC2 ? NTRU_K_DEC2_TENSOR : NTRU_K_DEC1_TENSOR));
     const int clusters = a.npairs < ctx->sm_count / 2 ? a.npairs : ctx->sm_count / 2;
@@ -411,16 +436,16 @@
 #define NTRU_DBG_LAUNCH(D)                                                                                                  \
   case D:                                                                                                                  \
     cudaFuncSetAttribute(k_umma_pair<MODE, D>, cudaFuncAttributeMaxDynamicSharedMemorySize, (int)kPairSmemBytes);          \
-    k_umma_pair<MODE, D><<<2 * clusters, kPairThreads, kPairSmemBytes, ctx->stream>>>(a, tmB, tmB2, tmA, tmM, tmO[0], tmO[1], tmO[2]); \
+    launch_pair<MODE, D>(ctx, clusters, a, t, none);                                                                       \
     break;
     switch (pu1 ? 0 : dbg) {
       NTRU_DBG_LAUNCH(1) NTRU_DBG_LAUNCH(2) NTRU_DBG_LAUNCH(4) NTRU_DBG_LAUNCH(8) NTRU_DBG_LAUNCH(12) NTRU_DBG_LAUNCH(16)
       default:
         if (pu1) {
           cudaFuncSetAttribute(k_umma_pair<ENC, 0, 1>, cudaFuncAttributeMaxDynamicSharedMemorySize, (int)kPairSmemBytes);
-          k_umma_pair<ENC, 0, 1><<<2 * clusters, kPairThreads, kPairSmemBytes, ctx->stream>>>(a, tmB, tmB2, tmA, tmM, tmO[0], tmO[1], tmO[2]);
+          launch_pair<ENC, 0, 1>(ctx, clusters, a, t, none);
         } else {
-          k_umma_pair<MODE><<<2 * clusters, kPairThreads, kPairSmemBytes, ctx->stream>>>(a, tmB, tmB2, tmA, tmM, tmO[0], tmO[1], tmO[2]);
+          launch_pair<MODE>(ctx, clusters, a, t, none);
         }
     }
 #else
@@ -429,11 +454,53 @@
         NTRU_CUDA(ctx, cudaFuncSetAttribute(k_umma_pair<ENC, 0, 1>, cudaFuncAttributeMaxDynamicSharedMemorySize, (int)kPairSmemBytes));
         ctx->umma_attr_set |= 16;
       }
-      k_umma_pair<ENC, 0, 1><<<2 * clusters, kPairThreads, kPairSmemBytes, ctx->stream>>>(a, tmB, tmB2, tmA, tmM, tmO[0], tmO[1], tmO[2]);
+      launch_pair<ENC, 0, 1>(ctx, clusters, a, t, none);
     } else {
-      k_umma_pair<MODE><<<2 * clusters, kPairThreads, kPairSmemBytes, ctx->stream>>>(a, tmB, tmB2, tmA, tmM, tmO[0], tmO[1], tmO[2]);
+      launch_pair<MODE>(ctx, clusters, a, t, none);
     }
 #endif
+  }
+  NTRU_CUDA(ctx, cudaGetLastError());
+  return NTRU_OK;
+}
+
+bool decrypt_fused(const ntru_ctx *ctx) {
+  if (ctx->opt_dec_fused == 1 || !ctx->km_f.f16 || ctx->P > 4 * kAtomK) return false;
+  if (!one_group_mode(ctx, DEC1F) || !one_group_mode(ctx, DEC2)) return false;
+  const KeyMatrix &k1 = ctx->km_f, &k2 = ctx->km_fp;
+  if (k1.nchunks != k2.nchunks || 4 * k1.nchunks > kMaxPhases) return false;
+  for (int c = 0; c <= k1.nchunks; ++c)
+    if (k1.col0[c] != k2.col0[c] || (k1.col0[c] & (kAtomK - 1))) return false;
+  return true;
+}
+
+int launch_decrypt_fused(ntru_ctx *ctx, UmmaArgs &a, UmmaArgs &b) {
+  if (!(ctx->umma_attr_set & 64)) {
+    NTRU_CUDA(ctx, cudaFuncSetAttribute(k_umma_pair<DEC>, cudaFuncAttributeMaxDynamicSharedMemorySize, (int)kPairSmemBytes));
+    ctx->umma_attr_set |= 64;
+  }
+  ProductMaps t1, t2;
+  bool pu1 = false;
+  int rc = setup_product<DEC1F>(ctx, ctx->km_f, a, nullptr, t1, &pu1);
+  if (rc) return rc;
+  rc = setup_product<DEC2>(ctx, ctx->km_fp, b, nullptr, t2, &pu1);
+  if (rc) return rc;
+  Phase ph[kMaxPhases];
+  int n = 0;
+  for (int j = 0; j < b.nph; ++j) { ph[n] = b.ph[j]; ph[n++].prod = 1; }
+  for (int j = 0; j < a.nph; ++j) { ph[n] = a.ph[j]; ph[n++].prod = 0; }
+  memcpy(a.ph, ph, sizeof ph);
+  a.nph = n;
+  a.atoms2 = b.atoms; a.k_last2 = b.k_last; a.out_mask2 = b.out_mask;
+  a.nS = 2; a.nM = 0;
+  a.a_resident = 0; a.a_tma = 0; a.a_rel = 1; a.one_group = 1;
+  a.nA = 4;
+  a.nR = b.atoms;
+  a.nB = kPairSlots - a.nS - a.nA - a.nR;
+  {
+    LaunchTimer timer(ctx, NTRU_K_DEC_TENSOR);
+    const int clusters = a.npairs < ctx->sm_count / 2 ? a.npairs : ctx->sm_count / 2;
+    launch_pair<DEC>(ctx, clusters, a, t1, t2);
   }
   NTRU_CUDA(ctx, cudaGetLastError());
   return NTRU_OK;
@@ -490,22 +557,24 @@
 int umma_decrypt(ntru_ctx *ctx, size_t B, const uint16_t *e, uint8_t *value, uint16_t *q1, uint16_t *r1, uint8_t *q2,
                  uint8_t *r2) {
   if (B == 0) return NTRU_OK;
-  NTRU_CUDA(ctx, ctx->d_b.reserve(B * (size_t)ctx->P));
+  const bool fused = decrypt_fused(ctx);
+  if (!fused) NTRU_CUDA(ctx, ctx->d_b.reserve(B * (size_t)ctx->P));
   UmmaArgs a = {};
   a.B = B; a.a_src = e;
   a.with_hi = q1 != nullptr;
-  a.o16_cyc = r1; a.o16_hi = q1; a.o8_cyc = (uint8_t *)ctx->d_b.ptr;
-  int rc = ctx->km_f.f16 ? launch_product<DEC1F>(ctx, ctx->km_f, a, nullptr) : launch_product<DEC1>(ctx, ctx->km_f, a, nullptr);
-  if (rc) return rc;
-#ifdef NTRU_TRACE
-  if (getenv("NTRU_TRACE_DEC1_ONLY")) return NTRU_OK;
-#endif
+  a.o16_cyc = r1; a.o16_hi = q1; a.o8_cyc = fused ? nullptr : (uint8_t *)ctx->d_b.ptr;
   UmmaArgs b = {};
   b.B = B;
   b.with_hi = q2 != nullptr;
   b.o8_cyc = value ? value : r2;
   b.o8_cyc2 = value ? r2 : nullptr;
   b.o8_hi = q2;
+  if (fused) return launch_decrypt_fused(ctx, a, b);
+  int rc = ctx->km_f.f16 ? launch_product<DEC1F>(ctx, ctx->km_f, a, nullptr) : launch_product<DEC1>(ctx, ctx->km_f, a, nullptr);
+  if (rc) return rc;
+#ifdef NTRU_TRACE
+  if (getenv("NTRU_TRACE_DEC1_ONLY")) return NTRU_OK;
+#endif
   return launch_product<DEC2>(ctx, ctx->km_fp, b, ctx->d_b.ptr);
 }
 
diff --git a/ntru-circom_b200/csrc/umma_pair.cuh b/ntru-circom_b200/csrc/umma_pair.cuh
--- a/ntru-circom_b200/csrc/umma_pair.cuh
+++ b/ntru-circom_b200/csrc/umma_pair.cuh
@@ -117,7 +117,10 @@
 k_umma_pair(const UmmaArgs a, const __grid_constant__ CUtensorMap tmapB, const __grid_constant__ CUtensorMap tmapB2,
             const __grid_constant__ CUtensorMap tmapA,
             const __grid_constant__ CUtensorMap tmapM, const __grid_constant__ CUtensorMap tmapO0,
-            const __grid_constant__ CUtensorMap tmapO1, const __grid_constant__ CUtensorMap tmapO2) {
+            const __grid_constant__ CUtensorMap tmapO1, const __grid_constant__ CUtensorMap tmapO2,
+            const __grid_constant__ CUtensorMap tmapC, const __grid_constant__ CUtensorMap tmapC2,
+            const __grid_constant__ CUtensorMap tmapP0, const __grid_constant__ CUtensorMap tmapP1,
+            const __grid_constant__ CUtensorMap tmapP2) {
   extern __shared__ uint8_t smem_raw[];
   uint8_t *smem = reinterpret_cast<uint8_t *>((reinterpret_cast<uintptr_t>(smem_raw) + 1023) & ~(uintptr_t)1023);
   uint64_t *bars = reinterpret_cast<uint64_t *>(smem + (size_t)kPairSlots * kSlotBytes);
@@ -133,9 +136,12 @@
   auto m_empty = [&](uint32_t b) { return bar0 + 8u * (4 * kPairSlots + 6 + b); };
   const uint32_t smem_base = smem_u32(smem);
   auto a_slot = [&](uint32_t i) { return smem_base + i * kSlotBytes; };
-  auto b_slot = [&](uint32_t j) { return smem_base + (a.nA + j) * kSlotBytes; };
-  auto m_slot = [&](uint32_t j) { return smem_base + (a.nA + a.nB + j) * kSlotBytes; };
-  const uint32_t stage_base = smem_base + (a.nA + a.nB + a.nM) * kSlotBytes;
+  auto b_slot = [&](uint32_t j) { return smem_base + (a.nA + a.nR + j) * kSlotBytes; };
+  auto m_slot = [&](uint32_t j) { return smem_base + (a.nA + a.nR + a.nB + j) * kSlotBytes; };
+  const uint32_t stage_base = smem_base + (a.nA + a.nR + a.nB + a.nM) * kSlotBytes;
+  const int stride = gridDim.x >> 1;
+  const int t_end = MODE == DEC ? a.npairs + stride : a.npairs;
+  auto skip = [&](const Phase &ph, int T) { return MODE == DEC && (ph.prod ? T < stride : T >= a.npairs); };
 
 #ifdef NTRU_TRACE
   int trace_n[kTraceLanes] = {0, 0, 0, 0};
@@ -146,8 +152,8 @@
   constexpr int kEpiWarps = MODE == DEC1 ? 8 : 16;
 
   if (threadIdx.x == 0) {
-    for (int i = 0; i < a.nA; ++i) {
-      mbar_init(a_full(i), MODE == DEC1 ? 16 : 2);
+    for (int i = 0; i < a.nA + a.nR; ++i) {
+      mbar_init(a_full(i), MODE == DEC1 ? 16 : (i < a.nA ? 2 : 2 * kEpiWarps));
       mbar_init(a_empty(i), a.a_rel);
     }
     if (MODE == DEC1 && a.a_tma) {
@@ -183,14 +189,16 @@
     int gs = 0;
 #endif
     if (lane == 0) { TRACE(3, 10, 0); TRACE_NS(3, 11, 0); }
-    for (int T = blockIdx.x >> 1; T < a.npairs; T += gridDim.x >> 1) {
+    for (int T = blockIdx.x >> 1; T < t_end; T += stride) {
       for (int j = 0; j < a.nph; ++j) {
         const Phase ph = a.ph[j];
+        if (skip(ph, T)) continue;
         const int c = ph.c;
         const int wc = a.col0[c + 1] - a.col0[c];
         const int half_rows = (a.nl * wc) >> 1;
         const uint32_t b_bytes = 2u * (uint32_t)half_rows * kAtomK;
-        const CUtensorMap *bmap = wc == a.w0 ? &tmapB : &tmapB2;
+        const CUtensorMap *bmap = (MODE == DEC && ph.prod) ? (wc == a.w0 ? &tmapC : &tmapC2)
+                                                           : (wc == a.w0 ? &tmapB : &tmapB2);
         const int row0 = ph.kind * part_rows + a.nl * a.col0[c] + (int)rank * half_rows;
         for (int at = ph.a0; at < ph.a1; ++at) {
           for (int lk = 0; lk < a.kl; ++lk) {
@@ -257,14 +265,15 @@
         }
         __syncwarp();
       };
-      for (int T = blockIdx.x >> 1; T < a.npairs; T += gridDim.x >> 1, t_par ^= 1) {
+      for (int T = blockIdx.x >> 1; T < t_end; T += stride, t_par ^= 1) {
         const int a_row = T * 256 + (int)rank * kTileRows;
         if (resident) {
           for (int k = 0; k < a.atoms; ++k) load_a((uint32_t)a.a_order[k], t_par, a.a_order[k], a_row);
         }
         for (int j = 0; j < a.nph; ++j) {
           const Phase ph = a.ph[j];
-          if (!resident) {
+          if (skip(ph, T)) continue;
+          if (!resident && !(MODE == DEC && ph.prod)) {
             for (int at = ph.a0; at < ph.a1; ++at) {
               load_a(sas, a_par_s, at, a_row);
               if (++sas == (uint32_t)a.nA) { sas = 0; a_par_s ^= 1; }
@@ -286,7 +295,7 @@
   } else if (warp == kPairMmaWarp) {
     if (leader) {
       const uint64_t desc_hi = make_smem_desc(0) & ~0x3FFFull;
-      const uint32_t a_lo0 = smem_base >> 4, b_lo0 = (smem_base + a.nA * kSlotBytes) >> 4;
+      const uint32_t a_lo0 = smem_base >> 4, b_lo0 = (smem_base + (a.nA + a.nR) * kSlotBytes) >> 4;
       const bool resident = a.a_resident != 0;
       const uint32_t nB = (uint32_t)a.nB, nA = (uint32_t)a.nA;
       const uint32_t bfull0 = b_full(0), bempty0 = b_empty(0), afull0 = a_full(0), aempty0 = a_empty(0);
@@ -304,13 +313,19 @@
 #else
 #define LP_ADD(acc) do {} while (0)
 #endif
-      for (int T = blockIdx.x >> 1; T < a.npairs; T += gridDim.x >> 1, t_par ^= 1) {
-        for (int j = 0; j < a.nph; ++j, ++cc) {
+      for (int T = blockIdx.x >> 1; T < t_end; T += stride, t_par ^= 1) {
+        for (int j = 0; j < a.nph; ++j) {
           const Phase ph = a.ph[j];
+          if (skip(ph, T)) continue;
+          const bool p2 = MODE == DEC && ph.prod;
+          const bool res = MODE == DEC ? p2 : resident;
+          const bool f16 = MODE == DEC1F || (MODE == DEC && !p2);
+          const uint32_t r_par = MODE == DEC ? t_par ^ 1u : t_par;
+          const uint32_t last_at = (uint32_t)(p2 ? a.atoms2 : a.atoms) - 1, klast_ph = p2 ? (uint32_t)a.k_last2 : klast;
           const uint32_t nsl = (uint32_t)(ph.a1 - ph.a0) * kl_u;
           const int wc = a.col0[ph.c + 1] - a.col0[ph.c];
-          const uint32_t idesc = MODE == DEC1F ? make_idesc_pair_f16(wc) : make_idesc_pair(0, MODE == DEC1 ? 1 : 0, a.nl * wc);
-          const uint32_t first = resident ? ph.first : 0xffffu, rel = resident ? ph.rel : 0xffffu;
+          const uint32_t idesc = f16 ? make_idesc_pair_f16(wc) : make_idesc_pair(0, MODE == DEC1 ? 1 : 0, a.nl * wc);
+          const uint32_t first = res ? ph.first : 0xffffu, rel = res ? ph.rel : 0xffffu;
           const uint32_t buf = cc & 1;
           if (lane == 0) TRACE(1, 0, cc);
           LP_ADD(lp_other);
@@ -322,12 +337,12 @@
           if (lane == 0) TRACE(1, 1, cc);
           const uint32_t d_tmem = tmem_base + buf * kAccCols;
           const uint32_t tfull = tfull_bar(buf);
-          uint32_t sa = resident ? (uint32_t)ph.a0 * kl_u : sas;
+          uint32_t sa = res ? (MODE == DEC ? nA : 0u) + (uint32_t)ph.a0 * kl_u : sas;
           uint32_t at = (uint32_t)ph.a0, lk = 0;
           uint32_t accumulate = ph.kind == PH_LO ? 1u : 0u;
           for (uint32_t i = 0; i < nsl; ++i) {
             LP_ADD(lp_other);
-            if ((first >> at) & 1u) mbar_wait((lane & 1) ? afull0 + 8u * sa : bfull0 + 8u * sb, (lane & 1) ? (resident ? t_par : a_par_s) : b_par);
+            if ((first >> at) & 1u) mbar_wait((lane & 1) ? afull0 + 8u * sa : bfull0 + 8u * sb, (lane & 1) ? (res ? r_par : a_par_s) : b_par);
             else mbar_wait(bfull0 + 8u * sb, b_par);
             __syncwarp();
             LP_ADD(lp_ops);
@@ -338,23 +353,28 @@
             const uint64_t da = desc_hi | (uint64_t)(a_lo0 + sa * (kSlotBytes >> 4));
             const uint64_t db = desc_hi | (uint64_t)(b_lo0 + sb * (kSlotBytes >> 4));
 #ifdef NTRU_TRACE
-            const uint32_t nk = (a.debug_flags & 2) ? 1u : (at == (uint32_t)(a.atoms - 1) ? klast : 4u);
+            const uint32_t nk = (a.debug_flags & 2) ? 1u : (at == last_at ? klast_ph : 4u);
 #else
-            const uint32_t nk = at == (uint32_t)(a.atoms - 1) ? klast : 4u;
-#endif
+            const uint32_t nk = at == last_at ? klast_ph : 4u;
+#endif
+            auto mma_slice = [&](auto f16c) {
+              constexpr bool F = decltype(f16c)::value;
+              umma_pair<F>(d_tmem, da, db, idesc, accumulate);
+              if (nk > 1) umma_pair<F>(d_tmem, da + 2, db + 2, idesc, 1u);
+              if (nk > 2) umma_pair<F>(d_tmem, da + 4, db + 4, idesc, 1u);
+              if (nk > 3) umma_pair<F>(d_tmem, da + 6, db + 6, idesc, 1u);
+#ifdef NTRU_TRACE
+              if (a.debug_flags & 32) {
+                umma_pair<F>(d_tmem, da, db, idesc, 1u);
+                umma_pair<F>(d_tmem, da + 2, db + 2, idesc, 1u);
+                umma_pair<F>(d_tmem, da + 4, db + 4, idesc, 1u);
+                umma_pair<F>(d_tmem, da + 6, db + 6, idesc, 1u);
+              }
+#endif
+            };
             if (elect_one()) {
-              umma_pair<MODE == DEC1F>(d_tmem, da, db, idesc, accumulate);
-              if (nk > 1) umma_pair<MODE == DEC1F>(d_tmem, da + 2, db + 2, idesc, 1u);
-              if (nk > 2) umma_pair<MODE == DEC1F>(d_tmem, da + 4, db + 4, idesc, 1u);
-              if (nk > 3) umma_pair<MODE == DEC1F>(d_tmem, da + 6, db + 6, idesc, 1u);
-#ifdef NTRU_TRACE
-              if (a.debug_flags & 32) {
-                umma_pair<MODE == DEC1F>(d_tmem, da, db, idesc, 1u);
-                umma_pair<MODE == DEC1F>(d_tmem, da + 2, db + 2, idesc, 1u);
-                umma_pair<MODE == DEC1F>(d_tmem, da + 4, db + 4, idesc, 1u);
-                umma_pair<MODE == DEC1F>(d_tmem, da + 6, db + 6, idesc, 1u);
-              }
-#endif
+              if (f16) mma_slice(std::true_type{});
+              else mma_slice(std::false_type{});
               umma_commit_pair(bempty0 + 8u * sb);
               if ((rel >> at) & 1u) umma_commit_pair(aempty0 + 8u * sa);
               if (i == nsl - 1) umma_commit_pair(tfull);
@@ -369,13 +389,14 @@
             accumulate = 1;
             if (++sb == nB) { sb = 0; b_par ^= 1; }
             if (++lk == kl_u) { lk = 0; ++at; }
-            if (resident) {
+            if (res) {
               ++sa;
             } else {
               if (++sas == nA) { sas = 0; a_par_s ^= 1; }
               sa = sas;
             }
           }
+          ++cc;
         }
       }
 #ifdef NTRU_TRACE
@@ -525,8 +546,6 @@
     }
   } else {
     const int kSub = (a.one_group ? kEpiWarps : kEpiWarps / 2) / 4;
-    constexpr bool kMsgGlobal = MODE == ENC && PU == 1;
-    constexpr int kPassUnits = PU;
     const int ew = warp - (MODE == DEC1 ? kPairEpiWarp0Dec1 : 0);
     const int quad = warp & 3;
     const uint32_t grp = (uint32_t)(ew >> 2) & 1u;
@@ -534,26 +553,31 @@
     const uint32_t Q2 = a.qmask | (a.qmask << 16);
     const uint32_t LA2 = (((uint32_t)a.q >> 1) - 1u) * 0x00010001u;
     const int logq = 31 - __clz(a.q);
-    constexpr uint32_t kRowBytes = (MODE == DEC2 ? 16u : 32u) * PU;
-    static_assert(kRowBytes == 64 || kRowBytes == 32, "staging rows are one 64-byte or 32-byte swizzle span");
-    const uint32_t stage = stage_base + (uint32_t)ew * (MODE == DEC1 ? 4096u : 32u * kRowBytes);
-    const uint32_t st_row = stage + (uint32_t)lane * kRowBytes;
-    const uint32_t st_x = kRowBytes == 64 ? (uint32_t)(lane >> 1) & 3u : (uint32_t)(lane >> 2) & 1u;
     const int row_in_tile = quad * 32 + lane;
     const uint32_t m_row = (uint32_t)((row_in_tile >> 3) * 1024 + (row_in_tile & 7) * 128), m_x = (uint32_t)row_in_tile & 7u;
     const uint32_t t_addr0 = tmem_base + ((uint32_t)(quad * 32) << 16);
     const uint32_t tfull0 = tfull_bar(0), lead_tempty0 = lead(tempty_bar(0));
     uint32_t cc = 0, mc = 0;
+    uint32_t r_par = 0;
     bool store_pending = false;
-    for (int T = blockIdx.x >> 1; T < a.npairs; T += gridDim.x >> 1) {
-      const int out_row = T * 256 + (int)rank * kTileRows + quad * 32;
-      {
-        for (int jp = 0; jp < a.nph; ++jp, ++cc) {
-          const int c = a.ph[jp].c;
-          const int hi = a.ph[jp].kind == PH_HI;
+    auto drain = [&](auto pm_c, const Phase &ph, int tile, uint32_t cc) {
+          constexpr int PM = decltype(pm_c)::value;
+          constexpr bool kMsgGlobal = PM == ENC && PU == 1;
+          constexpr int kPassUnits = MODE == DEC ? (PM == DEC2 ? 4 : 2) : PU;
+          constexpr uint32_t kRowBytes = (PM == DEC2 ? 16u : 32u) * kPassUnits;
+          static_assert(kRowBytes == 64 || kRowBytes == 32, "staging rows are one 64-byte or 32-byte swizzle span");
+          const uint32_t stage = stage_base + (uint32_t)ew * (PM == DEC1 ? 4096u : 32u * kRowBytes);
+          const uint32_t st_row = stage + (uint32_t)lane * kRowBytes;
+          const uint32_t st_x = kRowBytes == 64 ? (uint32_t)(lane >> 1) & 3u : (uint32_t)(lane >> 2) & 1u;
+          constexpr bool kP2 = MODE == DEC && PM == DEC2;
+          const CUtensorMap *o0 = kP2 ? &tmapP0 : &tmapO0, *o1 = kP2 ? &tmapP1 : &tmapO1, *o2 = kP2 ? &tmapP2 : &tmapO2;
+          const int out_mask = kP2 ? a.out_mask2 : a.out_mask;
+          const int out_row = tile * 256 + (int)rank * kTileRows + quad * 32;
+          const int c = ph.c;
+          const int hi = ph.kind == PH_HI;
           const uint32_t ms = mc & 1, m_par = (mc >> 1) & 1;
-          if (MODE == ENC && !hi) ++mc;
-          if (!a.one_group && (cc & 1u) != grp) continue;
+          if (PM == ENC && !hi) ++mc;
+          if (!a.one_group && (cc & 1u) != grp) return;
           const uint32_t buf = cc & 1u;
           const uint32_t t_addr = t_addr0 + buf * kAccCols, my_tfull = tfull0 + 8u * buf, lead_tempty = lead_tempty0 + 8u * buf;
           const int col0c = a.col0[c], wc = a.col0[c + 1] - col0c;
@@ -573,16 +597,28 @@
           mbar_wait(my_tfull, (cc >> 1) & 1);
           tc_fence_after();
           if (lane == 0 && ew == 0) TRACE(2, 1, cc);
-          if (MODE == ENC && !kMsgGlobal && !hi) mbar_wait(m_full(ms), m_par);
+          if (PM == ENC && !kMsgGlobal && !hi) mbar_wait(m_full(ms), m_par);
           if (lane == 0 && ew == 0) TRACE(2, 3, cc);
+          constexpr bool kBSmem = MODE == DEC && PM == DEC1F;
+          const int ba0 = col0c >> 7, ba1 = (col0c + wc) >> 7;
+          auto b_done = [&]() {
+            if (kBSmem && !hi) {
+              __syncwarp();
+              if (lane == 0)
+                for (int at = ba0; at < ba1; ++at) mbar_arrive_cluster(lead(a_full((uint32_t)(a.nA + at))));
+            }
+          };
+          if (kBSmem && !hi)
+            for (int at = ba0; at < ba1; ++at) mbar_wait(a_empty((uint32_t)(a.nA + at)), r_par ^ 1u);
           if (DBG & 1) {
             tc_fence_before();
             __syncwarp();
             if (lane == 0) {
               mbar_arrive_cluster(lead_tempty);
-              if (MODE == ENC && !kMsgGlobal && !hi) mbar_arrive(m_empty(ms));
-            }
-            continue;
+              if (PM == ENC && !kMsgGlobal && !hi) mbar_arrive(m_empty(ms));
+            }
+            b_done();
+            return;
           }
           int npe = (a.P - (col0c + sub * upw * 16) + kPassUnits * 16 - 1) / (kPassUnits * 16);
           npe = npe < 0 ? 0 : (npe > npass ? npass : npe);
@@ -591,14 +627,15 @@
             __syncwarp();
             if (lane == 0) {
               mbar_arrive_cluster(lead_tempty);
-              if (MODE == ENC && !kMsgGlobal && !hi) mbar_arrive(m_empty(ms));
-            }
-            continue;
+              if (PM == ENC && !kMsgGlobal && !hi) mbar_arrive(m_empty(ms));
+            }
+            b_done();
+            return;
           }
           for (int ps = 0; ps < npe; ++ps) {
             const int u0 = sub * upw + ps * kPassUnits;
             const bool last_pass = ps == npe - 1;
-            uint32_t res[kPassUnits * (MODE == DEC2 ? 4 : 8)];
+            uint32_t res[kPassUnits * (PM == DEC2 ? 4 : 8)];
             uint32_t bres[kPassUnits * 4];
             uint4 mm[kPassUnits];
             if (kMsgGlobal) {
@@ -615,7 +652,7 @@
                   mm[0] = make_uint4(w[0], w[1], w[2], w[3]);
                 }
               }
-            } else if (MODE == ENC && !hi) {
+            } else if (PM == ENC && !hi) {
 #pragma unroll
               for (int j = 0; j < kPassUnits; ++j) mm[j] = lds128(m_slot(ms) + m_row + ((((uint32_t)(u0 + j)) ^ m_x) << 4));
             }
@@ -630,17 +667,17 @@
                   continue;
                 }
                 tmem_ld16(t_addr + (u0 + j) * 16, acc[j]);
-                if (MODE == ENC && a.nl == 2) tmem_ld16(t_addr + wc + (u0 + j) * 16, acc1[j]);
+                if (PM == ENC && a.nl == 2) tmem_ld16(t_addr + wc + (u0 + j) * 16, acc1[j]);
               }
               if (!(DBG & 4)) tmem_ld_wait();
               if (lane == 0 && ew == 0) TRACE(2, 4, cc);
-              if (MODE == ENC && a.nl == 2) {
+              if (PM == ENC && a.nl == 2) {
 #pragma unroll
                 for (int j = 0; j < kPassUnits; ++j)
 #pragma unroll
                   for (int i = 0; i < 16; ++i) acc[j][i] += acc1[j][i] << 8;
               }
-              if (MODE == DEC1F) {
+              if (PM == DEC1F) {
 #pragma unroll
                 for (int j = 0; j < kPassUnits; ++j)
 #pragma unroll
@@ -652,7 +689,7 @@
               __syncwarp();
               if (lane == 0) {
                 mbar_arrive_cluster(lead_tempty);
-                if (MODE == ENC && !kMsgGlobal && !hi) mbar_arrive(m_empty(ms));
+                if (PM == ENC && !kMsgGlobal && !hi) mbar_arrive(m_empty(ms));
               }
             }
             if (DBG & 2) {
@@ -665,14 +702,14 @@
 #pragma unroll
             for (int j = 0; j < kPassUnits; ++j) {
               uint32_t (&w)[32] = acc[j];
-              if (MODE == ENC || MODE == DEC1 || MODE == DEC1F) {
+              if (PM == ENC || PM == DEC1 || PM == DEC1F) {
                 uint32_t *pk = res + 8 * j;
 #pragma unroll
                 for (int jj = 0; jj < 8; ++jj) pk[jj] = __byte_perm(w[2 * jj], w[2 * jj + 1], 0x5410);
                 if (hi) {
 #pragma unroll
                   for (int jj = 0; jj < 8; ++jj) pk[jj] = ((~pk[jj] & Q2) + 0x00010001u) & Q2;
-                } else if (MODE == ENC) {
+                } else if (PM == ENC) {
                   const uint32_t mw[4] = {mm[j].x, mm[j].y, mm[j].z, mm[j].w};
 #pragma unroll
                   for (int jj = 0; jj < 8; ++jj) {
@@ -682,7 +719,7 @@
                 } else {
 #pragma unroll
                   for (int jj = 0; jj < 8; ++jj) pk[jj] &= Q2;
-                  if (a.o8_cyc) {
+                  if (MODE == DEC || a.o8_cyc) {
                     if (logq & 1) {
 #pragma unroll
                       for (int wd = 0; wd < 4; ++wd) {
@@ -726,7 +763,7 @@
             if (DBG & 8) {
               uint32_t x = 0;
 #pragma unroll
-              for (int j = 0; j < kPassUnits * (MODE == DEC2 ? 4 : 8); ++j) x ^= res[j];
+              for (int j = 0; j < kPassUnits * (PM == DEC2 ? 4 : 8); ++j) x ^= res[j];
               if (x == 0x12345678u) sts128(st_row, make_uint4(x, x, x, x));
               continue;
             }
@@ -734,7 +771,7 @@
               if (lane == 0) asm volatile("cp.async.bulk.wait_group.read 0;" ::: "memory");
               __syncwarp();
             }
-            if (MODE == DEC2) {
+            if (PM == DEC2) {
 #pragma unroll
               for (int j = 0; j < kPassUnits; ++j)
                 sts128(st_row + ((((uint32_t)j) ^ st_x) << 4), make_uint4(res[4 * j], res[4 * j + 1], res[4 * j + 2], res[4 * j + 3]));
@@ -744,13 +781,28 @@
                 sts128(st_row + ((((uint32_t)(2 * j)) ^ st_x) << 4), make_uint4(res[8 * j], res[8 * j + 1], res[8 * j + 2], res[8 * j + 3]));
                 sts128(st_row + ((((uint32_t)(2 * j + 1)) ^ st_x) << 4), make_uint4(res[8 * j + 4], res[8 * j + 5], res[8 * j + 6], res[8 * j + 7]));
               }
-              if (MODE == DEC1 && !hi && a.o8_cyc) {
+              if (PM == DEC1 && !hi && a.o8_cyc) {
 #pragma unroll
                 for (int j = 0; j < kPassUnits; ++j)
                   sts128(stage + 2048u + (uint32_t)lane * 32u + (uint32_t)j * 16u,
                          make_uint4(bres[4 * j], bres[4 * j + 1], bres[4 * j + 2], bres[4 * j + 3]));
               }
-              if (MODE == DEC1F && !hi && a.o8_cyc) {
+              if (kBSmem && !hi) {
+#pragma unroll
+                for (int j = 0; j < kPassUnits; ++j) {
+                  const int col = col0c + (u0 + j) * 16;
+                  const int keep = a.N - col;
+                  uint32_t w[4] = {bres[4 * j], bres[4 * j + 1], bres[4 * j + 2], bres[4 * j + 3]};
+#pragma unroll
+                  for (int t = 0; t < 4; ++t) {
+                    const int kb = keep - 4 * t;
+                    w[t] = kb >= 4 ? w[t] : (kb <= 0 ? 0u : (w[t] & ((1u << (8 * kb)) - 1u)));
+                  }
+                  sts128(a_slot((uint32_t)(a.nA + (col >> 7))) + m_row + (((uint32_t)((col >> 4) & 7) ^ m_x) << 4),
+                         make_uint4(w[0], w[1], w[2], w[3]));
+                }
+              }
+              if (PM == DEC1F && !kBSmem && !hi && a.o8_cyc) {
                 const size_t grow = (size_t)(out_row + lane);
                 const int col = col0c + u0 * 16;
                 if (grow < a.B) {
@@ -770,21 +822,33 @@
             if (lane == 0) {
               const int col = col0c + u0 * 16;
               if (hi) {
-                if (a.out_mask & 4) tma_store_2d(&tmapO2, stage, col, out_row);
+                if (out_mask & 4) tma_store_2d(o2, stage, col, out_row);
               } else {
-                if (a.out_mask & 1) tma_store_2d(&tmapO0, stage, col, out_row);
-                if (MODE == DEC1) {
-                  if (a.out_mask & 2) tma_store_2d(&tmapO1, stage + 2048, col, out_row);
+                if (out_mask & 1) tma_store_2d(o0, stage, col, out_row);
+                if (PM == DEC1) {
+                  if (out_mask & 2) tma_store_2d(o1, stage + 2048, col, out_row);
                 } else {
-                  if (a.out_mask & 2) tma_store_2d(&tmapO1, stage, col, out_row);
+                  if (out_mask & 2) tma_store_2d(o1, stage, col, out_row);
                 }
               }
               asm volatile("cp.async.bulk.commit_group;" ::: "memory");
             }
             store_pending = true;
           }
+          b_done();
           if (lane == 0 && ew == 0) TRACE(2, 2, cc);
+    };
+    for (int T = blockIdx.x >> 1; T < t_end; T += stride, r_par ^= 1u) {
+      for (int jp = 0; jp < a.nph; ++jp) {
+        const Phase ph = a.ph[jp];
+        if (skip(ph, T)) continue;
+        if constexpr (MODE == DEC) {
+          if (ph.prod) drain(std::integral_constant<int, DEC2>{}, ph, T - stride, cc);
+          else drain(std::integral_constant<int, DEC1F>{}, ph, T, cc);
+        } else {
+          drain(std::integral_constant<int, MODE>{}, ph, T, cc);
         }
+        ++cc;
       }
     }
     if (lane == 0) asm volatile("cp.async.bulk.wait_group 0;" ::: "memory");
diff --git a/ntru-circom_b200/engine.py b/ntru-circom_b200/engine.py
--- a/ntru-circom_b200/engine.py
+++ b/ntru-circom_b200/engine.py
@@ -74,6 +74,9 @@
 
     def set_epilogue(self, mode: int):
         self.set_option(_lib.NTRU_OPT_EPILOGUE, int(mode))
+
+    def set_dec_fused(self, mode: int):
+        self.set_option(_lib.NTRU_OPT_DEC_FUSED, int(mode))
 
     def set_imma_form(self, generic: bool):
         self.set_option(_lib.NTRU_OPT_IMMA_FORM, 1 if generic else 0)
```
